# Runki2018/litehandnet

Hardware: AMD Instinct MI355X
Metric: images/sec fwd+bwd @256x256 bs64 litehandnet (higher is better)
Workload: dtype f32; 1 GPU; litehandnet variant B (MSRB hourglass litehourglass.py) C=128, 256x256x3 -> 21x64x64, per-GPU batch 64, train-mode BN, fwd + TopdownHeatmapLoss + bwd + fused Adam; global_batch=64, parallelism=dp1

## Files before the change

litehandnet_amd/csrc/k_misc.hip:

```cpp
#include "lhn_common.h"

static inline int grid_cap(int64_t blocks, int cap_per_cu) {
  const int64_t cap = (int64_t)lhn_num_cus() * cap_per_cu;
  if (blocks > cap) blocks = cap;
  if (blocks < 1) blocks = 1;
  return (int)blocks;
}
static inline bool pow2i(int v) { return v > 0 && (v & (v - 1)) == 0; }

#define LHN_FIN_THREADS 1024
__global__ void __launch_bounds__(LHN_FIN_THREADS) k_bn_finalize(const double* __restrict__ stats, const float* __restrict__ gamma,
                              const float* __restrict__ beta, float* __restrict__ rmean, float* __restrict__ rvar,
                              int64_t* __restrict__ nbt, float* __restrict__ table, int cs, int coff, int C,
                              float* __restrict__ save, double count, float eps, float momentum, float slope, int training,
                              const float* __restrict__ cbias, int SC) {
  __shared__ double part[2 * LHN_FIN_THREADS];
  const int nt = blockDim.x;
  int G = nt / C;
  G = G < 1 ? 1 : (G > LHN_STAT_REPLICAS ? LHN_STAT_REPLICAS : G);
  for (int c0 = 0; c0 < C; c0 += nt) {
    const int g = threadIdx.x / C, c = c0 + (G > 1 ? threadIdx.x - g * C : threadIdx.x);
    if (c0) __syncthreads();
    if (training && g < G && c < C) {
      double s1 = 0, s2 = 0;
#pragma unroll 4
      for (int r = g; r < LHN_STAT_REPLICAS; r += G) {
        s1 += stats[(size_t)r * 2 * SC + c];
        s2 += stats[(size_t)r * 2 * SC + SC + c];
      }
      part[2 * threadIdx.x] = s1;
      part[2 * threadIdx.x + 1] = s2;
    }
    __syncthreads();
    if (g != 0 || c >= C) continue;
    double mean, var;
    const double cb = cbias ? (double)cbias[c] : 0.0;
    if (training) {
      double s1 = 0, s2 = 0;
      for (int k = 0; k < G; ++k) {
        s1 += part[2 * (k * C + threadIdx.x)];
        s2 += part[2 * (k * C + threadIdx.x) + 1];
      }
      mean = s1 / count;
      var = s2 / count - mean * mean;
      if (var < 0) var = 0;
      if (rmean) {
        rmean[c] = (float)((1.0 - (double)momentum) * (double)rmean[c] + (double)momentum * (mean + cb));
        const double unb = count > 1 ? var * count / (count - 1.0) : var;
        rvar[c] = (float)((1.0 - (double)momentum) * (double)rvar[c] + (double)momentum * unb);
      }
    } else {
      mean = (double)rmean[c] - cb;
      var = rvar[c];
    }
    const float invstd = (float)(1.0 / sqrt(var + (double)eps));
    const float gm = gamma ? gamma[c] : 1.f, b = beta ? beta[c] : 0.f;
    const float sc = gm * invstd;
    table[coff + c] = sc;
    table[cs + coff + c] = b - (float)mean * sc;
    table[2 * cs + coff + c] = slope;
    if (save) {
      save[c] = (float)mean;
      save[SC + c] = invstd;
    }
  }
  if (training && nbt && threadIdx.x == 0) nbt[0] += 1;
}

__global__ void k_table_fill(float* __restrict__ table, int cs, int coff, int C, float sc, float sh, float sl) {
  for (int c = threadIdx.x; c < C; c += blockDim.x) {
    table[coff + c] = sc;
    table[cs + coff + c] = sh;
    table[2 * cs + coff + c] = sl;
  }
}

__global__ void k_table_bias(float* __restrict__ table, int cs, int coff, int C, const float* __restrict__ bias, float sl) {
  for (int c = threadIdx.x; c < C; c += blockDim.x) {
    table[coff + c] = 1.f;
    table[cs + coff + c] = bias ? bias[c] : 0.f;
    table[2 * cs + coff + c] = sl;
  }
}

struct EwSrcs {
  lhn_view v[3];
  float coef[3];
  int mode;
};
__device__ __forceinline__ void bil_taps(int d, int in, int out, int& i0, int& i1, float& w1) {
  if (in == out || out == 1) {
    i0 = i1 = (in == out) ? d : 0;
    w1 = 0.f;
    return;
  }
  const float pos = (float)d * ((float)(in - 1) / (float)(out - 1));
  i0 = (int)floorf(pos);
  if (i0 > in - 1) i0 = in - 1;
  i1 = i0 + 1 < in ? i0 + 1 : in - 1;
  w1 = pos - (float)i0;
}
__device__ __forceinline__ float lhn_relu_sigmoid(float v) { return 1.f / (1.f + expf(-fmaxf(v, 0.f))); }
__device__ __forceinline__ float lhn_relu_sigmoid_grad(float v) {
  if (!(v > 0.f)) return 0.f;
  const float s = 1.f / (1.f + expf(-v));
  return s * (1.f - s);
}
__device__ __forceinline__ int nearest_src(int d, int in, int out) {
  if (in == out) return d;
  const float sc = (float)in / (float)out;
  const int s = (int)floorf((float)d * sc);
  return s < in - 1 ? s : in - 1;
}
template <bool BIL>
__global__ void __launch_bounds__(256, BIL ? 1 : 3) k_ew_fwd(EwSrcs S, int nsrc, lhn_view dst, float out_slope) {
  const int C4 = dst.C >> 2, c4 = threadIdx.x % C4, pl = threadIdx.x / C4, PL = 256 / C4;
  const int rows = dst.N * dst.H;
  Xf4 xf[3];
  int ca[3];
#pragma unroll
  for (int k = 0; k < 3; ++k)
    if (k < nsrc) {
      ca[k] = S.v[k].coff + 4 * c4;
      xf[k] = lhn_load_xf(S.v[k], ca[k]);
    }
  for (int row = blockIdx.x; row < rows; row += gridDim.x) {
    const int n = row / dst.H, h = row - n * dst.H;
    const float* base[3];
    f4 gate[3];
#pragma unroll
    for (int k = 0; k < 3; ++k)
      if (k < nsrc) {
        const lhn_view& v = S.v[k];
        const int hs = nearest_src(h, v.H, dst.H);
        base[k] = v.data + ((size_t)(n * v.H + hs) * v.W) * v.cstride + ca[k];
        gate[k] = v.gate ? *reinterpret_cast<const f4*>(v.gate + (size_t)n * v.cstride + ca[k]) : (f4){1.f, 1.f, 1.f, 1.f};
      }
    float* out = dst.data + (size_t)row * dst.W * dst.cstride + dst.coff + 4 * c4;
    const bool mul = (S.mode & 1) != 0;
    constexpr bool bil = BIL;
    if (!bil) {
      for (int w0 = LHN_LANE0(pl, PL); w0 < dst.W; w0 += 4 * PL) {
        f4 raw[3][4];
#pragma unroll
        for (int k = 0; k < 3; ++k)
          if (k < nsrc) {
            const lhn_view& v = S.v[k];
#pragma unroll
            for (int j = 0; j < 4; ++j) {
              const int w = min(w0 + j * PL, dst.W - 1);
              const int ws = (v.W == dst.W) ? w : nearest_src(w, v.W, dst.W);
              raw[k][j] = *reinterpret_cast<const f4*>(base[k] + (size_t)ws * v.cstride);
            }
          }
#pragma unroll
        for (int j = 0; j < 4; ++j) {
          const int w = w0 + j * PL;
          if (w < dst.W) {
            f4 acc = mul ? (f4){1.f, 1.f, 1.f, 1.f} : (f4){0.f, 0.f, 0.f, 0.f};
#pragma unroll
            for (int k = 0; k < 3; ++k)
              if (k < nsrc) {
                const f4 val = lhn_apply_xf(raw[k][j], xf[k]) * (gate[k] * S.coef[k]);
                if (mul) acc *= val; else acc += val;
              }
            if (out_slope == LHN_SLOPE_RELU_SIGMOID) {
              acc.x = lhn_relu_sigmoid(acc.x); acc.y = lhn_relu_sigmoid(acc.y); acc.z = lhn_relu_sigmoid(acc.z); acc.w = lhn_relu_sigmoid(acc.w);
            } else if (out_slope == LHN_SLOPE_SILU) {
              acc.x = lhn_silu(acc.x); acc.y = lhn_silu(acc.y); acc.z = lhn_silu(acc.z); acc.w = lhn_silu(acc.w);
            } else {
              acc.x = lhn_lrelu(acc.x, out_slope); acc.y = lhn_lrelu(acc.y, out_slope); acc.z = lhn_lrelu(acc.z, out_slope); acc.w = lhn_lrelu(acc.w, out_slope);
            }
            *reinterpret_cast<f4*>(out + (size_t)w * dst.cstride) = acc;
          }
        }
      }
      continue;
    }
    for (int w = LHN_LANE0(pl, PL); w < dst.W; w += PL) {
      f4 acc = mul ? (f4){1.f, 1.f, 1.f, 1.f} : (f4){0.f, 0.f, 0.f, 0.f};
#pragma unroll
      for (int k = 0; k < 3; ++k)
        if (k < nsrc) {
          const lhn_view& v = S.v[k];
          f4 val;
          if (bil && (v.H != dst.H || v.W != dst.W)) {
            int h0, h1, w0, w1;
            float ah, aw;
            bil_taps(h, v.H, dst.H, h0, h1, ah);
            bil_taps(w, v.W, dst.W, w0, w1, aw);
            const float* b0 = v.data + ((size_t)(n * v.H + h0) * v.W) * v.cstride + ca[k];
            const float* b1 = v.data + ((size_t)(n * v.H + h1) * v.W) * v.cstride + ca[k];
            const f4 v00 = lhn_apply_xf(*reinterpret_cast<const f4*>(b0 + (size_t)w0 * v.cstride), xf[k]);
            const f4 v01 = lhn_apply_xf(*reinterpret_cast<const f4*>(b0 + (size_t)w1 * v.cstride), xf[k]);
            const f4 v10 = lhn_apply_xf(*reinterpret_cast<const f4*>(b1 + (size_t)w0 * v.cstride), xf[k]);
            const f4 v11 = lhn_apply_xf(*reinterpret_cast<const f4*>(b1 + (size_t)w1 * v.cstride), xf[k]);
            val = ((v00 * (1.f - aw) + v01 * aw) * (1.f - ah) + (v10 * (1.f - aw) + v11 * aw) * ah) * (gate[k] * S.coef[k]);
          } else {
            const int ws = nearest_src(w, v.W, dst.W);
            val = lhn_apply_xf(*reinterpret_cast<const f4*>(base[k] + (size_t)ws * v.cstride), xf[k]) * (gate[k] * S.coef[k]);
          }
          if (mul) acc *= val; else acc += val;
        }
      if (out_slope == LHN_SLOPE_RELU_SIGMOID) {
        acc.x = lhn_relu_sigmoid(acc.x);
        acc.y = lhn_relu_sigmoid(acc.y);
        acc.z = lhn_relu_sigmoid(acc.z);
        acc.w = lhn_relu_sigmoid(acc.w);
      } else if (out_slope == LHN_SLOPE_SILU) {
        acc.x = lhn_silu(acc.x);
        acc.y = lhn_silu(acc.y);
        acc.z = lhn_silu(acc.z);
        acc.w = lhn_silu(acc.w);
      } else {
        acc.x = lhn_lrelu(acc.x, out_slope);
        acc.y = lhn_lrelu(acc.y, out_slope);
        acc.z = lhn_lrelu(acc.z, out_slope);
        acc.w = lhn_lrelu(acc.w, out_slope);
      }
      *reinterpret_cast<f4*>(out + (size_t)w * dst.cstride) = acc;
    }
  }
}

__global__ void __launch_bounds__(256) k_ew_bwd_src(lhn_view src, lhn_view dst, const float* __restrict__ ddst,
                                                    const float* __restrict__ dst_dpool, float out_slope,
                                                    float* __restrict__ dsrc, int accumulate, lhn_bnsum bs) {
  __shared__ f4 bred[512];
  const int C4 = src.C >> 2, c4 = threadIdx.x % C4, pl = threadIdx.x / C4, PL = 256 / C4;
  f4 bsum = (f4){0.f, 0.f, 0.f, 0.f}, bsq = bsum, bmean = bsum, binv = bsum;
  Xf4 bxf;
  if (bs.sums) {
    bxf = lhn_load_xf(src, src.coff + 4 * c4);
    bmean = *reinterpret_cast<const f4*>(bs.save + bs.coff + 4 * c4);
    binv = *reinterpret_cast<const f4*>(bs.save + bs.C + bs.coff + 4 * c4);
  }
  const int fh = dst.H / src.H, fw = dst.W / src.W;
  const int cd = dst.coff + 4 * c4;
  const int rows = src.N * src.H;
  for (int row = blockIdx.x; row < rows; row += gridDim.x) {
    const int n = row / src.H, h = row - n * src.H;
    const f4 gate = dst.gate ? *reinterpret_cast<const f4*>(dst.gate + (size_t)n * dst.cstride + cd) : (f4){1.f, 1.f, 1.f, 1.f};
    for (int w = LHN_LANE0(pl, PL); w < src.W; w += PL) {
      f4 g = (f4){0.f, 0.f, 0.f, 0.f};
      for (int a = 0; a < fh; ++a)
        for (int b = 0; b < fw; ++b) {
          const int hd = h * fh + a, wd = w * fw + b;
          const size_t pd = ((size_t)(n * dst.H + hd) * dst.W + wd) * dst.cstride + cd;
          f4 e = *reinterpret_cast<const f4*>(ddst + pd) * gate;
          if (dst_dpool) {
            lhn_gradview gv{nullptr, dst_dpool, nullptr};
            e += lhn_dpool_sum(gv, dst, n, hd, wd, cd);
          }
          if (out_slope == LHN_SLOPE_SILU || out_slope == LHN_SLOPE_RELU_SIGMOID) {
            const Xf4 sxf = lhn_load_xf(src, src.coff + 4 * c4);
            const f4 v = lhn_load_val(src, sxf, (int64_t)(n * src.H + h) * src.W + w, n, src.coff + 4 * c4);
            if (out_slope == LHN_SLOPE_SILU) {
              e.x *= lhn_silu_grad(v.x);
              e.y *= lhn_silu_grad(v.y);
              e.z *= lhn_silu_grad(v.z);
              e.w *= lhn_silu_grad(v.w);
            } else {
              e.x *= lhn_relu_sigmoid_grad(v.x);
              e.y *= lhn_relu_sigmoid_grad(v.y);
              e.z *= lhn_relu_sigmoid_grad(v.z);
              e.w *= lhn_relu_sigmoid_grad(v.w);
            }
          } else if (out_slope != 1.f) {
            const f4 o = *reinterpret_cast<const f4*>(dst.data + pd);
            e.x *= o.x > 0.f ? 1.f : out_slope;
            e.y *= o.y > 0.f ? 1.f : out_slope;
            e.z *= o.z > 0.f ? 1.f : out_slope;
            e.w *= o.w > 0.f ? 1.f : out_slope;
          }
          g += e;
        }
      float* o = dsrc + ((size_t)row * src.W + w) * src.cstride + src.coff + 4 * c4;
      if (bs.sums) {
        const f4 raw = *reinterpret_cast<const f4*>(src.data + ((size_t)row * src.W + w) * src.cstride + src.coff + 4 * c4);
        const f4 du = g * lhn_dact_xf(raw, bxf);
        bsum += du;
        bsq += du * ((raw - bmean) * binv);
      }
      if (accumulate) g += *reinterpret_cast<const f4*>(o);
      *reinterpret_cast<f4*>(o) = g;
    }
  }
  if (bs.sums) lhn_bns_flush(bs, bsum, bsq, C4, bred);
}

struct EwBwdMulti {
  int n;
  lhn_view src[3];
  float* dsrc[3];
  int acc[3];
  lhn_bnsum bs[3];
};
__global__ void __launch_bounds__(256) k_ew_bwd_multi(EwBwdMulti m, lhn_view dst, const float* __restrict__ ddst,
                                                      const float* __restrict__ dst_dpool, float out_slope) {
  __shared__ f4 bred[512];
  const int C4 = dst.C >> 2, c4 = threadIdx.x % C4, pl = threadIdx.x / C4, PL = 256 / C4;
  f4 bsum[3], bsq[3], bmean[3], binv[3];
  Xf4 bxf[3];
#pragma unroll
  for (int k = 0; k < 3; ++k) {
    bsum[k] = bsq[k] = bmean[k] = binv[k] = (f4){0.f, 0.f, 0.f, 0.f};
    if (k < m.n && m.bs[k].sums) {
      bxf[k] = lhn_load_xf(m.src[k], m.src[k].coff + 4 * c4);
      bmean[k] = *reinterpret_cast<const f4*>(m.bs[k].save + m.bs[k].coff + 4 * c4);
      binv[k] = *reinterpret_cast<const f4*>(m.bs[k].save + m.bs[k].C + m.bs[k].coff + 4 * c4);
    }
  }
  const int cd = dst.coff + 4 * c4;
  const int rows = dst.N * dst.H;
  for (int row = blockIdx.x; row < rows; row += gridDim.x) {
    const int n = row / dst.H, h = row - n * dst.H;
    const f4 gate = dst.gate ? *reinterpret_cast<const f4*>(dst.gate + (size_t)n * dst.cstride + cd) : (f4){1.f, 1.f, 1.f, 1.f};
    for (int w = LHN_LANE0(pl, PL); w < dst.W; w += PL) {
      const size_t pix = (size_t)row * dst.W + w, pd = pix * dst.cstride + cd;
      f4 e = *reinterpret_cast<const f4*>(ddst + pd) * gate;
      if (dst_dpool) {
        lhn_gradview gv{nullptr, dst_dpool, nullptr};
        e += lhn_dpool_sum(gv, dst, n, h, w, cd);
      }
      if (out_slope != 1.f) {
        const f4 o = *reinterpret_cast<const f4*>(dst.data + pd);
        e.x *= o.x > 0.f ? 1.f : out_slope;
        e.y *= o.y > 0.f ? 1.f : out_slope;
        e.z *= o.z > 0.f ? 1.f : out_slope;
        e.w *= o.w > 0.f ? 1.f : out_slope;
      }
#pragma unroll
      for (int k = 0; k < 3; ++k) {
        if (k < m.n) {
          const size_t ps = pix * m.src[k].cstride + m.src[k].coff + 4 * c4;
          f4 g = e;
          if (m.bs[k].sums) {
            const f4 raw = *reinterpret_cast<const f4*>(m.src[k].data + ps);
            const f4 du = g * lhn_dact_xf(raw, bxf[k]);
            bsum[k] += du;
            bsq[k] += du * ((raw - bmean[k]) * binv[k]);
          }
          float* o = m.dsrc[k] + ps;
          if (m.acc[k]) g += *reinterpret_cast<const f4*>(o);
          *reinterpret_cast<f4*>(o) = g;
        }
      }
    }
  }
#pragma unroll
  for (int k = 0; k < 3; ++k)
    if (k < m.n && m.bs[k].sums) {
      lhn_bns_flush(m.bs[k], bsum[k], bsq[k], C4, bred);
      __syncthreads();
    }
}

__global__ void __launch_bounds__(256) k_maxpool2_fwd(lhn_view x, lhn_view y) {
  const int C4 = y.C >> 2, c4 = threadIdx.x % C4, pl = threadIdx.x / C4, PL = 256 / C4;
  const int ca = x.coff + 4 * c4;
  const Xf4 xf = lhn_load_xf(x, ca);
  const int rows = y.N * y.H;
  for (int row = blockIdx.x; row < rows; row += gridDim.x) {
    const int n = row / y.H, ho = row - n * y.H;
    const f4 gate = x.gate ? *reinterpret_cast<const f4*>(x.gate + (size_t)n * x.cstride + ca) : (f4){1.f, 1.f, 1.f, 1.f};
    for (int wo = LHN_LANE0(pl, PL); wo < y.W; wo += PL) {
      f4 m = (f4){-INFINITY, -INFINITY, -INFINITY, -INFINITY};
#pragma unroll
      for (int o = 0; o < 4; ++o) {
        const int ih = 2 * ho + (o >> 1), iw = 2 * wo + (o & 1);
        if (ih < x.H && iw < x.W) {
          const f4 v = lhn_apply_xf(*reinterpret_cast<const f4*>(x.data + ((size_t)(n * x.H + ih) * x.W + iw) * x.cstride + ca), xf) * gate;
          m.x = v.x > m.x || v.x != v.x ? v.x : m.x;
          m.y = v.y > m.y || v.y != v.y ? v.y : m.y;
          m.z = v.z > m.z || v.z != v.z ? v.z : m.z;
          m.w = v.w > m.w || v.w != v.w ? v.w : m.w;
        }
      }
      *reinterpret_cast<f4*>(y.data + ((size_t)row * y.W + wo) * y.cstride + y.coff + 4 * c4) = m;
    }
  }
}
template <bool ADD>
__global__ void __launch_bounds__(256) k_maxpool2_bwd(lhn_view x, lhn_view y, const float* __restrict__ dy,
                                                      float* __restrict__ dx, int accumulate, lhn_bnsum bs, lhn_grad_adds ad) {
  __shared__ f4 bred[512];
  const int C4 = y.C >> 2, c4 = threadIdx.x % C4, pl = threadIdx.x / C4, PL = 256 / C4;
  const int ca = x.coff + 4 * c4;
  const Xf4 xf = lhn_load_xf(x, ca);
  f4 bsum = (f4){0.f, 0.f, 0.f, 0.f}, bsq = bsum, bmean = bsum, binv = bsum;
  if (bs.sums) {
    bmean = *reinterpret_cast<const f4*>(bs.save + bs.coff + 4 * c4);
    binv = *reinterpret_cast<const f4*>(bs.save + bs.C + bs.coff + 4 * c4);
  }
  const int rows = y.N * y.H;
  for (int row = blockIdx.x; row < rows; row += gridDim.x) {
    const int n = row / y.H, ho = row - n * y.H;
    const f4 gate = x.gate ? *reinterpret_cast<const f4*>(x.gate + (size_t)n * x.cstride + ca) : (f4){1.f, 1.f, 1.f, 1.f};
    for (int wo = LHN_LANE0(pl, PL); wo < y.W; wo += PL) {
      const f4 g = *reinterpret_cast<const f4*>(dy + ((size_t)row * y.W + wo) * y.cstride + y.coff + 4 * c4);
      f4 m = (f4){-INFINITY, -INFINITY, -INFINITY, -INFINITY};
      int arg[4] = {-1, -1, -1, -1};
      f4 raws[4];
#pragma unroll
      for (int o = 0; o < 4; ++o) {
        const int ih = 2 * ho + (o >> 1), iw = 2 * wo + (o & 1);
        if (ih < x.H && iw < x.W) {
          raws[o] = *reinterpret_cast<const f4*>(x.data + ((size_t)(n * x.H + ih) * x.W + iw) * x.cstride + ca);
          const f4 v = lhn_apply_xf(raws[o], xf) * gate;
          if (v.x > m.x || v.x != v.x || arg[0] < 0) { if (!(m.x != m.x)) { m.x = v.x; arg[0] = o; } }
          if (v.y > m.y || v.y != v.y || arg[1] < 0) { if (!(m.y != m.y)) { m.y = v.y; arg[1] = o; } }
          if (v.z > m.z || v.z != v.z || arg[2] < 0) { if (!(m.z != m.z)) { m.z = v.z; arg[2] = o; } }
          if (v.w > m.w || v.w != v.w || arg[3] < 0) { if (!(m.w != m.w)) { m.w = v.w; arg[3] = o; } }
        }
      }
#pragma unroll
      for (int o = 0; o < 4; ++o) {
        const int ih = 2 * ho + (o >> 1), iw = 2 * wo + (o & 1);
        if (ih < x.H && iw < x.W) {
          f4 r = (f4){arg[0] == o ? g.x : 0.f, arg[1] == o ? g.y : 0.f, arg[2] == o ? g.z : 0.f, arg[3] == o ? g.w : 0.f};
          if (ADD) {
            if (ad.same) r += *reinterpret_cast<const f4*>(ad.same + ((size_t)(n * x.H + ih) * x.W + iw) * ad.same_cstride + ad.same_coff + 4 * c4);
            if (ad.pooled) {
              const int OH = ad.OH, OW = ad.OW, ohc = (ih * OH) / x.H, owc = (iw * OW) / x.W;
              for (int oh = max(ohc - 1, 0); oh <= min(ohc + 1, OH - 1); ++oh) {
                const int h0 = (oh * x.H) / OH, h1 = ((oh + 1) * x.H + OH - 1) / OH;
                if (ih < h0 || ih >= h1) continue;
                for (int ow = max(owc - 1, 0); ow <= min(owc + 1, OW - 1); ++ow) {
                  const int w0 = (ow * x.W) / OW, w1 = ((ow + 1) * x.W + OW - 1) / OW;
                  if (iw < w0 || iw >= w1) continue;
                  const float inv = 1.f / (float)((h1 - h0) * (w1 - w0));
                  r += *reinterpret_cast<const f4*>(ad.pooled + ((size_t)(n * OH + oh) * OW + ow) * ad.pooled_cstride + ad.pooled_coff + 4 * c4) * inv;
                }
              }
            }
          }
          float* q = dx + ((size_t)(n * x.H + ih) * x.W + iw) * x.cstride + ca;
          if (bs.sums) {
            const f4 du = r * lhn_dact_xf(raws[o], xf);
            bsum += du;
            bsq += du * ((raws[o] - bmean) * binv);
          }
          if (accumulate) r += *reinterpret_cast<const f4*>(q);
          *reinterpret_cast<f4*>(q) = r;
        }
      }
    }
  }
  if (bs.sums) lhn_bns_flush(bs, bsum, bsq, C4, bred);
}

struct BnSlices {
  const float* save[2];
  double* sums[2];
  int lo[2], C[2], n;
};
__device__ __forceinline__ void lhn_slice_mi4(const BnSlices& sl, int c, f4& mean, f4& inv) {
  mean = (f4){0.f, 0.f, 0.f, 0.f};
  inv = (f4){1.f, 1.f, 1.f, 1.f};
#pragma unroll
  for (int k = 0; k < 2; ++k)
    if (k < sl.n && c >= sl.lo[k] && c < sl.lo[k] + sl.C[k]) {
      mean = *reinterpret_cast<const f4*>(sl.save[k] + (c - sl.lo[k]));
      inv = *reinterpret_cast<const f4*>(sl.save[k] + sl.C[k] + (c - sl.lo[k]));
    }
}
__device__ __forceinline__ f4 lhn_dact4(f4 raw, const Xf4& t) {
  const f4 u = raw * t.sc + t.sh;
  return (f4){u.x > 0.f ? 1.f : t.sl.x, u.y > 0.f ? 1.f : t.sl.y, u.z > 0.f ? 1.f : t.sl.z, u.w > 0.f ? 1.f : t.sl.w};
}

template <bool STAT, bool COPY>
__global__ void __launch_bounds__(256) k_avgpool_fwd(lhn_view x, float* __restrict__ out, int OH, int OW, int ostride,
                                                     int ocoff, float* __restrict__ pstat, BnSlices sl, lhn_view src) {
  __shared__ f4 red[STAT ? 768 : 256];
  const int C4 = x.C >> 2, PL = 256 / C4;
  const int b = blockIdx.x;
  const int ow = b % OW, oh = (b / OW) % OH, n = b / (OW * OH);
  const int h0 = (oh * x.H) / OH, h1 = ((oh + 1) * x.H + OH - 1) / OH;
  const int w0 = (ow * x.W) / OW, w1 = ((ow + 1) * x.W + OW - 1) / OW;
  const int bw = w1 - w0, cnt = (h1 - h0) * bw;
  const int c4 = threadIdx.x % C4, pl = threadIdx.x / C4;
  const int ca = x.coff + 4 * c4;
  const bool cp = COPY && 4 * c4 < src.C;
  const int sca = src.coff + 4 * c4;
  Xf4 xf = lhn_load_xf(x, ca);
  f4 sgate = (f4){1.f, 1.f, 1.f, 1.f};
  if (cp) {
    xf = lhn_load_xf(src, sca);
    if (src.gate) sgate = *reinterpret_cast<const f4*>(src.gate + (int64_t)n * src.cstride + sca);
  }
  f4 mean, inv;
  if (STAT) lhn_slice_mi4(sl, ca, mean, inv);
  const float* base = cp ? src.data + (int64_t)n * x.H * x.W * src.cstride + sca : x.data + (int64_t)n * x.H * x.W * x.cstride + ca;
  const int64_t pstr = cp ? src.cstride : x.cstride;
  auto at = [&](int p) { return *reinterpret_cast<const f4*>(base + (int64_t)((h0 + p / bw) * x.W + w0 + p % bw) * pstr); };
  const int hown = ((oh + 1) * x.H) / OH, wown = ((ow + 1) * x.W) / OW;
  float* xout = x.data + (int64_t)n * x.H * x.W * x.cstride + ca;
  auto put = [&](int p, f4 v) {
    const int h = h0 + p / bw, w = w0 + p % bw;
    if (h < hown && w < wown) *reinterpret_cast<f4*>(xout + (int64_t)(h * x.W + w) * x.cstride) = v;
  };
  f4 s0 = (f4){0.f, 0.f, 0.f, 0.f}, s1 = s0, s2 = s0, s3 = s0, m0 = s0, m1 = s0;
  int p = LHN_LANE0(pl, PL);
  for (; p + 3 * PL < cnt; p += 4 * PL) {
    const f4 a = at(p), b2 = at(p + PL), c2 = at(p + 2 * PL), d2 = at(p + 3 * PL);
    const f4 va = lhn_apply_xf(a, xf) * sgate, vb = lhn_apply_xf(b2, xf) * sgate, vc = lhn_apply_xf(c2, xf) * sgate, vd = lhn_apply_xf(d2, xf) * sgate;
    s0 += va;
    s1 += vb;
    s2 += vc;
    s3 += vd;
    if (cp) {
      put(p, va);
      put(p + PL, vb);
      put(p + 2 * PL, vc);
      put(p + 3 * PL, vd);
    }
    if (STAT) {
      const f4 da = lhn_dact4(a, xf), db = lhn_dact4(b2, xf), dc = lhn_dact4(c2, xf), dd = lhn_dact4(d2, xf);
      m0 += (da + db) + (dc + dd);
      m1 += (da * ((a - mean) * inv) + db * ((b2 - mean) * inv)) + (dc * ((c2 - mean) * inv) + dd * ((d2 - mean) * inv));
    }
  }
  for (; p < cnt; p += PL) {
    const f4 a = at(p);
    const f4 va = lhn_apply_xf(a, xf) * sgate;
    s0 += va;
    if (cp) put(p, va);
    if (STAT) {
      const f4 da = lhn_dact4(a, xf);
      m0 += da;
      m1 += da * ((a - mean) * inv);
    }
  }
  f4 s = (s0 + s1) + (s2 + s3);
  if (x.gate) s *= *reinterpret_cast<const f4*>(x.gate + (int64_t)n * x.cstride + ca);
  const bool shuf = C4 <= 64 && (C4 & (C4 - 1)) == 0;
  if (shuf)
    for (int o = C4; o < 64; o <<= 1) {
      s.x += __shfl_xor(s.x, o, 64); s.y += __shfl_xor(s.y, o, 64); s.z += __shfl_xor(s.z, o, 64); s.w += __shfl_xor(s.w, o, 64);
      if (STAT) {
        m0.x += __shfl_xor(m0.x, o, 64); m0.y += __shfl_xor(m0.y, o, 64); m0.z += __shfl_xor(m0.z, o, 64); m0.w += __shfl_xor(m0.w, o, 64);
        m1.x += __shfl_xor(m1.x, o, 64); m1.y += __shfl_xor(m1.y, o, 64); m1.z += __shfl_xor(m1.z, o, 64); m1.w += __shfl_xor(m1.w, o, 64);
      }
    }
  const int lane = threadIdx.x & 63, wave = threadIdx.x >> 6;
  if (shuf && lane < C4) {
    red[wave * C4 + lane] = s;
    if (STAT) {
      red[256 + wave * C4 + lane] = m0;
      red[512 + wave * C4 + lane] = m1;
    }
  }
  if (!shuf) {
    red[threadIdx.x] = s;
    if (STAT) {
      red[256 + threadIdx.x] = m0;
      red[512 + threadIdx.x] = m1;
    }
  }
  __syncthreads();
  if (threadIdx.x < C4) {
    const int nj = shuf ? 4 : PL;
    f4 t = (f4){0.f, 0.f, 0.f, 0.f}, t0 = t, t1 = t;
    for (int j = 0; j < nj; ++j) {
      t += red[j * C4 + threadIdx.x];
      if (STAT) {
        t0 += red[256 + j * C4 + threadIdx.x];
        t1 += red[512 + j * C4 + threadIdx.x];
      }
    }
    const float invc = 1.f / (float)cnt;
    *reinterpret_cast<f4*>(out + (int64_t)b * ostride + ocoff + 4 * threadIdx.x) = t * invc;
    if (STAT) {
      *reinterpret_cast<f4*>(pstat + ((int64_t)b * 2 + 0) * x.C + 4 * threadIdx.x) = t0;
      *reinterpret_cast<f4*>(pstat + ((int64_t)b * 2 + 1) * x.C + 4 * threadIdx.x) = t1;
    }
  }
}
__global__ void __launch_bounds__(256) k_avgpool_small(lhn_view x, float* __restrict__ out, int OH, int OW, int ostride, int ocoff) {
  const int C4 = x.C >> 2;
  const int64_t total = (int64_t)x.N * OH * OW * C4;
  for (int64_t i = (int64_t)blockIdx.x * 256 + threadIdx.x; i < total; i += (int64_t)gridDim.x * 256) {
    const int c4 = (int)(i % C4);
    const int64_t b = i / C4;
    const int ow = (int)(b % OW), oh = (int)((b / OW) % OH), n = (int)(b / ((int64_t)OW * OH));
    const int h0 = (oh * x.H) / OH, h1 = ((oh + 1) * x.H + OH - 1) / OH;
    const int w0 = (ow * x.W) / OW, w1 = ((ow + 1) * x.W + OW - 1) / OW;
    const int ca = x.coff + 4 * c4;
    const Xf4 xf = lhn_load_xf(x, ca);
    f4 s = (f4){0.f, 0.f, 0.f, 0.f};
    for (int h = h0; h < h1; ++h)
      for (int w = w0; w < w1; ++w)
        s += lhn_apply_xf(*reinterpret_cast<const f4*>(x.data + ((int64_t)(n * x.H + h) * x.W + w) * x.cstride + ca), xf);
    if (x.gate) s *= *reinterpret_cast<const f4*>(x.gate + (int64_t)n * x.cstride + ca);
    *reinterpret_cast<f4*>(out + b * ostride + ocoff + 4 * c4) = s * (1.f / (float)((h1 - h0) * (w1 - w0)));
  }
}
__global__ void __launch_bounds__(256) k_avgpool_bwd(lhn_view x, const float* __restrict__ dout, int OH, int OW,
                                                     float* __restrict__ dx, int accumulate, int ostride, int ocoff, lhn_bnsum bs) {
  __shared__ f4 bred[512];
  const int C4 = x.C >> 2, c4 = threadIdx.x % C4, pl = threadIdx.x / C4, PL = 256 / C4;
  f4 bsum = (f4){0.f, 0.f, 0.f, 0.f}, bsq = bsum, bmean = bsum, binv = bsum;
  Xf4 bxf;
  if (bs.sums) {
    bxf = lhn_load_xf(x, x.coff + 4 * c4);
    bmean = *reinterpret_cast<const f4*>(bs.save + bs.coff + 4 * c4);
    binv = *reinterpret_cast<const f4*>(bs.save + bs.C + bs.coff + 4 * c4);
  }
  const int rows = x.N * x.H;
  for (int row = blockIdx.x; row < rows; row += gridDim.x) {
    const int n = row / x.H, h = row - n * x.H;
    for (int w = LHN_LANE0(pl, PL); w < x.W; w += PL) {
      f4 g = (f4){0.f, 0.f, 0.f, 0.f};
      const int ohc = (h * OH) / x.H, owc = (w * OW) / x.W;
      for (int oh = max(ohc - 1, 0); oh <= min(ohc + 1, OH - 1); ++oh) {
        const int h0 = (oh * x.H) / OH, h1 = ((oh + 1) * x.H + OH - 1) / OH;
        if (h < h0 || h >= h1) continue;
        for (int ow = max(owc - 1, 0); ow <= min(owc + 1, OW - 1); ++ow) {
          const int w0 = (ow * x.W) / OW, w1 = ((ow + 1) * x.W + OW - 1) / OW;
          if (w < w0 || w >= w1) continue;
          const float inv = 1.f / (float)((h1 - h0) * (w1 - w0));
          g += *reinterpret_cast<const f4*>(dout + ((size_t)(n * OH + oh) * OW + ow) * ostride + ocoff + 4 * c4) * inv;
        }
      }
      float* o = dx + ((size_t)row * x.W + w) * x.cstride + x.coff + 4 * c4;
      if (bs.sums) {
        const f4 raw = *reinterpret_cast<const f4*>(x.data + ((size_t)row * x.W + w) * x.cstride + x.coff + 4 * c4);
        const f4 du = g * lhn_dact_xf(raw, bxf);
        bsum += du;
        bsq += du * ((raw - bmean) * binv);
      }
      if (accumulate) g += *reinterpret_cast<const f4*>(o);
      *reinterpret_cast<f4*>(o) = g;
    }
  }
  if (bs.sums) lhn_bns_flush(bs, bsum, bsq, C4, bred);
}

__global__ void __launch_bounds__(1024) k_ca1(const float* __restrict__ pooled, const float* __restrict__ w3,
                                             const float* __restrict__ gamma, const float* __restrict__ beta,
                                             float* __restrict__ rmean, float* __restrict__ rvar, int64_t* __restrict__ nbt,
                                             const float* __restrict__ mask, float* __restrict__ save, int N, int C,
                                             float eps, float momentum, int training, int stage, double* __restrict__ gsum,
                                             double count_scale) {
  __shared__ double rs[32][32], rq[32][32];
  const int NL = blockDim.x >> 5;
  __shared__ float s_sc[32], s_sh[32];
  float* a = save;
  float* ahat = save + (int64_t)N * C;
  float* smean = save + (int64_t)N * C * 3 + (int64_t)N * (C / 2);
  float* sinv = smean + C;
  const int cl = threadIdx.x & 31, nl = threadIdx.x >> 5, c = blockIdx.x * 32 + cl;
  const bool ok = c < C;
  float wt[9];
#pragma unroll
  for (int t = 0; t < 9; ++t) wt[t] = ok ? w3[c * 9 + t] : 0.f;
  double s = 0, q = 0;
  if (ok && stage != 2)
    for (int n = nl; n < N; n += NL) {
      float v = 0.f;
#pragma unroll
      for (int t = 0; t < 9; ++t) v += pooled[((int64_t)n * 9 + t) * C + c] * wt[t];
      a[(int64_t)n * C + c] = v;
      s += v;
      q += (double)v * v;
    }
  rs[nl][cl] = s;
  rq[nl][cl] = q;
  __syncthreads();
  if (nl == 0 && ok) {
    for (int j = 1; j < NL; ++j) {
      s += rs[j][cl];
      q += rq[j][cl];
    }
    if (stage == 1) {
      gsum[c] = s;
      gsum[C + c] = q;
    } else if (stage == 2) {
      s = gsum[c];
      q = gsum[C + c];
    }
  }
  if (stage == 1) return;
  const double NT = (double)N * count_scale;
  if (nl == 0 && ok) {
    double mean, var;
    if (!gamma) {
      smean[c] = 0.f;
      sinv[c] = 1.f;
      s_sc[cl] = 1.f;
      s_sh[cl] = beta ? beta[c] : 0.f;
    } else {
    if (training) {
      mean = s / NT;
      var = q / NT - mean * mean;
      if (var < 0) var = 0;
      rmean[c] = (float)((1.0 - (double)momentum) * rmean[c] + (double)momentum * mean);
      rvar[c] = (float)((1.0 - (double)momentum) * rvar[c] + (double)momentum * (NT > 1 ? var * NT / (NT - 1.0) : var));
    } else {
      mean = rmean[c];
      var = rvar[c];
    }
    const float invstd = (float)(1.0 / sqrt(var + (double)eps));
    smean[c] = (float)mean;
    sinv[c] = invstd;
    s_sc[cl] = gamma[c] * invstd;
    s_sh[cl] = beta[c] - (float)mean * (gamma[c] * invstd);
    }
  }
  __syncthreads();
  if (ok) {
    const float sc = s_sc[cl], sh = s_sh[cl];
    for (int n = nl; n < N; n += NL) {
      float v = a[(int64_t)n * C + c] * sc + sh;
      if (mask) v *= mask[(int64_t)n * C + c];
      ahat[(int64_t)n * C + c] = v;
    }
  }
  if (training && nbt && blockIdx.x == 0 && threadIdx.x == 0) nbt[0] += 1;
}
__global__ void __launch_bounds__(256) k_ca2(const float* __restrict__ w1, const float* __restrict__ b1,
                                             const float* __restrict__ w2, const float* __restrict__ b2,
                                             float* __restrict__ save, float* __restrict__ gate, int gs, int gcoff, int N,
                                             int C) {
  __shared__ float sa[256], shh[128];
  const int n = blockIdx.x, Ch = C / 2;
  const float* ahat = save + (int64_t)N * C + (int64_t)n * C;
  float* h = save + (int64_t)N * C * 2 + (int64_t)n * Ch;
  float* g = save + (int64_t)N * C * 2 + (int64_t)N * Ch + (int64_t)n * C;
  for (int c = threadIdx.x; c < C; c += blockDim.x) sa[c] = ahat[c];
  __syncthreads();
  for (int j = threadIdx.x; j < Ch; j += blockDim.x) {
    float v = b1[j];
    for (int c = 0; c < C; ++c) v += w1[j * C + c] * sa[c];
    v = lhn_lrelu(v, 0.01f);
    h[j] = v;
    shh[j] = v;
  }
  __syncthreads();
  for (int c = threadIdx.x; c < C; c += blockDim.x) {
    float v = b2[c];
    for (int j = 0; j < Ch; ++j) v += w2[c * Ch + j] * shh[j];
    const float sg = 1.f / (1.f + expf(-v));
    g[c] = sg;
    gate[(int64_t)n * gs + gcoff + c] = sg;
  }
}

__global__ void __launch_bounds__(256) k_gate_bwd_reduce(lhn_view y, const float* __restrict__ dz,
                                                         float* __restrict__ dgate, float* __restrict__ tsum, BnSlices sl) {
  __shared__ f4 red[768];
  const int C4 = y.C >> 2, PL = 256 / C4, n = blockIdx.x;
  const int c4 = threadIdx.x % C4, pl = threadIdx.x / C4;
  const int ca = y.coff + 4 * c4;
  const Xf4 xf = lhn_load_xf(y, ca);
  f4 mean, inv;
  lhn_slice_mi4(sl, ca, mean, inv);
  const int HW = y.H * y.W;
  const int chunk = (HW + gridDim.y - 1) / gridDim.y;
  const int p0 = blockIdx.y * chunk, p1 = min(HW, p0 + chunk);
  f4 s = (f4){0.f, 0.f, 0.f, 0.f}, t0 = s, t1 = s;
  for (int p = p0 + LHN_LANE0(pl, PL); p < p1; p += 2 * PL) {
    const int64_t pixa = (int64_t)n * HW + p, pixb = (int64_t)n * HW + min(p + PL, p1 - 1);
    const f4 rawa = *reinterpret_cast<const f4*>(y.data + pixa * y.cstride + ca);
    const f4 rawb = *reinterpret_cast<const f4*>(y.data + pixb * y.cstride + ca);
    const f4 dza = *reinterpret_cast<const f4*>(dz + pixa * y.cstride + ca);
    f4 dzb = *reinterpret_cast<const f4*>(dz + pixb * y.cstride + ca);
    if (p + PL >= p1) dzb = (f4){0.f, 0.f, 0.f, 0.f};
    s += lhn_apply_xf(rawa, xf) * dza + lhn_apply_xf(rawb, xf) * dzb;
    if (tsum) {
      const f4 da = lhn_dact4(rawa, xf) * dza, db = lhn_dact4(rawb, xf) * dzb;
      t0 += da + db;
      t1 += da * ((rawa - mean) * inv) + db * ((rawb - mean) * inv);
    }
  }
  red[threadIdx.x] = s;
  red[256 + threadIdx.x] = t0;
  red[512 + threadIdx.x] = t1;
  __syncthreads();
  if (threadIdx.x < C4) {
    f4 t = (f4){0.f, 0.f, 0.f, 0.f}, u0 = t, u1 = t;
    for (int j = 0; j < PL; ++j) {
      t += red[j * C4 + threadIdx.x];
      u0 += red[256 + j * C4 + threadIdx.x];
      u1 += red[512 + j * C4 + threadIdx.x];
    }
    float* o = dgate + (int64_t)n * y.C + 4 * threadIdx.x;
    atomicAdd(o + 0, t.x);
    atomicAdd(o + 1, t.y);
    atomicAdd(o + 2, t.z);
    atomicAdd(o + 3, t.w);
    if (tsum) {
      float* o0 = tsum + ((int64_t)n * 2 + 0) * y.C + 4 * threadIdx.x;
      float* o1 = tsum + ((int64_t)n * 2 + 1) * y.C + 4 * threadIdx.x;
      atomicAdd(o0 + 0, u0.x); atomicAdd(o0 + 1, u0.y); atomicAdd(o0 + 2, u0.z); atomicAdd(o0 + 3, u0.w);
      atomicAdd(o1 + 0, u1.x); atomicAdd(o1 + 1, u1.y); atomicAdd(o1 + 2, u1.z); atomicAdd(o1 + 3, u1.w);
    }
  }
}

__global__ void __launch_bounds__(256) k_ca_bwd2(const float* __restrict__ w1, const float* __restrict__ w2,
                                                 const float* __restrict__ save, const float* __restrict__ dgate,
                                                 float* __restrict__ dahat , float* __restrict__ dvbuf ,
                                                 float* __restrict__ dhbuf , int N, int C) {
  __shared__ float sdv[256], sdh[128], shh[128];
  const int Ch = C / 2, n = blockIdx.x;
  const float* h = save + (int64_t)N * C * 2 + (int64_t)n * Ch;
  const float* g = save + (int64_t)N * C * 2 + (int64_t)N * Ch + (int64_t)n * C;
  for (int c = threadIdx.x; c < C; c += blockDim.x) {
    const float gg = g[c];
    const float dv = dgate[(int64_t)n * C + c] * gg * (1.f - gg);
    sdv[c] = dv;
    dvbuf[(int64_t)n * C + c] = dv;
  }
  for (int j = threadIdx.x; j < Ch; j += blockDim.x) shh[j] = h[j];
  __syncthreads();
  for (int j = threadIdx.x; j < Ch; j += blockDim.x) {
    float d = 0.f;
#pragma unroll 8
    for (int c = 0; c < C; ++c) d += w2[c * Ch + j] * sdv[c];
    d *= shh[j] > 0.f ? 1.f : 0.01f;
    sdh[j] = d;
    dhbuf[(int64_t)n * Ch + j] = d;
  }
  __syncthreads();
  for (int c = threadIdx.x; c < C; c += blockDim.x) {
    float d = 0.f;
#pragma unroll 8
    for (int j = 0; j < Ch; ++j) d += w1[j * C + c] * sdh[j];
    dahat[(int64_t)n * C + c] = d;
  }
}
__global__ void __launch_bounds__(1024) k_ca_bwd1(const float* __restrict__ pooled, const float* __restrict__ w3,
                                                 const float* __restrict__ gamma, const float* __restrict__ mask,
                                                 const float* __restrict__ save, const float* __restrict__ dahat,
                                                 float* __restrict__ dpool, int cs, int coff, int H, int W,
                                                 float* __restrict__ dw3, float* __restrict__ dgamma,
                                                 float* __restrict__ dbeta, int N, int C, int training, int stage,
                                                 double* __restrict__ gsum, double count_scale, float pgrad_scale,
                                                 const float* __restrict__ tsum, const float* __restrict__ pstat, BnSlices sl,
                                                 const float* __restrict__ dvbuf, const float* __restrict__ dhbuf,
                                                 float* __restrict__ dw1, float* __restrict__ db1, float* __restrict__ dw2,
                                                 float* __restrict__ db2) {
  const int nmain = (C + 31) / 32;
  if ((int)blockIdx.x >= nmain) {
    if (stage == 1) return;
    const int Ch = C / 2, o = ((int)blockIdx.x - nmain) * blockDim.x + threadIdx.x, nw = C * Ch;
    const float* ahat = save + (int64_t)N * C;
    const float* hh = save + (int64_t)N * C * 2;
    if (o < nw) {
      const int cc = o / Ch, j = o - cc * Ch;
      float v = 0.f;
#pragma unroll 8
      for (int n = 0; n < N; ++n) v += dvbuf[(int64_t)n * C + cc] * hh[(int64_t)n * Ch + j];
      dw2[o] += v;
    } else if (o < 2 * nw) {
      const int q = o - nw, j = q / C, cc = q - j * C;
      float v = 0.f;
#pragma unroll 8
      for (int n = 0; n < N; ++n) v += dhbuf[(int64_t)n * Ch + j] * ahat[(int64_t)n * C + cc];
      dw1[q] += v;
    } else if (o < 2 * nw + C) {
      const int cc = o - 2 * nw;
      float v = 0.f;
#pragma unroll 8
      for (int n = 0; n < N; ++n) v += dvbuf[(int64_t)n * C + cc];
      db2[cc] += v;
    } else if (o < 2 * nw + C + Ch) {
      const int j = o - 2 * nw - C;
      float v = 0.f;
#pragma unroll 8
      for (int n = 0; n < N; ++n) v += dhbuf[(int64_t)n * Ch + j];
      db1[j] += v;
    }
    return;
  }
  __shared__ double rs[32][32], rq[32][32];
  __shared__ float rw[32][32][9];
  const int NL = blockDim.x >> 5;
  const float* a = save;
  const float* smean = save + (int64_t)N * C * 3 + (int64_t)N * (C / 2);
  const float* sinv = smean + C;
  const int cl = threadIdx.x & 31, nl = threadIdx.x >> 5, c = blockIdx.x * 32 + cl;
  const bool ok = c < C;
  const float mean = ok ? smean[c] : 0.f, invstd = ok ? sinv[c] : 0.f, gm = ok ? gamma[c] : 0.f;
  double sd = 0, sdx = 0;
  if (ok && stage != 2)
    for (int n = nl; n < N; n += NL) {
      float d = dahat[(int64_t)n * C + c];
      if (mask) d *= mask[(int64_t)n * C + c];
      const float xh = (a[(int64_t)n * C + c] - mean) * invstd;
      sd += d;
      sdx += (double)d * xh;
    }
  rs[nl][cl] = sd;
  rq[nl][cl] = sdx;
  __syncthreads();
  sd = 0;
  sdx = 0;
  for (int j = 0; j < NL; ++j) {
    sd += rs[j][cl];
    sdx += rq[j][cl];
  }
  if (stage == 1) {
    if (nl == 0 && ok) {
      gsum[c] = sd;
      gsum[C + c] = sdx;
    }
    return;
  }
  if (stage == 2 && ok) {
    sd = gsum[c];
    sdx = gsum[C + c];
  }
  const double NT = (double)N * count_scale;
  if (nl == 0 && ok) {
    dgamma[c] += (float)sdx * pgrad_scale;
    dbeta[c] += (float)sd * pgrad_scale;
  }
  const float* gsave = save + (int64_t)N * C * 2 + (int64_t)N * (C / 2);
  double bs0 = 0, bs1 = 0;
  float wt[9], dwt[9], binv[9];
#pragma unroll
  for (int t = 0; t < 9; ++t) {
    wt[t] = ok ? w3[c * 9 + t] : 0.f;
    dwt[t] = 0.f;
    const int bi = t / 3, bj = t % 3;
    binv[t] = 1.f / (float)((lhn_bin_hi(bi, H) - lhn_bin_lo(bi, H)) * (lhn_bin_hi(bj, W) - lhn_bin_lo(bj, W)));
  }
  if (ok)
    for (int n = nl; n < N; n += NL) {
      float d = dahat[(int64_t)n * C + c];
      if (mask) d *= mask[(int64_t)n * C + c];
      const float xh = (a[(int64_t)n * C + c] - mean) * invstd;
      float da = gm * invstd * d;
      if (training) da = gm * invstd * (d - (float)(sd / NT) - xh * (float)(sdx / NT));
      float dseg[9];
#pragma unroll
      for (int t = 0; t < 9; ++t) {
        dwt[t] += da * pooled[((int64_t)n * 9 + t) * C + c];
        dseg[t] = da * wt[t] * binv[t];
      }
      lhn_dpool_store(dpool, n, cs, coff + c, dseg);
      if (tsum) {
        const float g = gsave[(int64_t)n * C + c];
        float a0 = g * tsum[((int64_t)n * 2 + 0) * C + c], a1 = g * tsum[((int64_t)n * 2 + 1) * C + c];
#pragma unroll
        for (int t = 0; t < 9; ++t) {
          a0 += dseg[t] * pstat[(((int64_t)n * 9 + t) * 2 + 0) * C + c];
          a1 += dseg[t] * pstat[(((int64_t)n * 9 + t) * 2 + 1) * C + c];
        }
        bs0 += a0;
        bs1 += a1;
      }
    }
  if (tsum) {
    __syncthreads();
    rs[nl][cl] = bs0;
    rq[nl][cl] = bs1;
    __syncthreads();
    if (nl == 0 && ok) {
      double t0 = 0, t1 = 0;
      for (int j = 0; j < NL; ++j) {
        t0 += rs[j][cl];
        t1 += rq[j][cl];
      }
      const int cb = coff + c;
#pragma unroll
      for (int k = 0; k < 2; ++k)
        if (k < sl.n && sl.sums[k] && cb >= sl.lo[k] && cb < sl.lo[k] + sl.C[k]) {
          sl.sums[k][cb - sl.lo[k]] = t0;
          sl.sums[k][sl.C[k] + cb - sl.lo[k]] = t1;
        }
    }
  }
#pragma unroll
  for (int t = 0; t < 9; ++t) rw[nl][cl][t] = dwt[t];
  __syncthreads();
  if (nl == 0 && ok) {
#pragma unroll
    for (int t = 0; t < 9; ++t) {
      float v = 0.f;
      for (int j = 0; j < NL; ++j) v += rw[j][cl][t];
      dw3[c * 9 + t] += v;
    }
  }
}

__global__ void __launch_bounds__(256) k_bn_bwd_reduce(lhn_view y, lhn_gradview g, const float* __restrict__ save,
                                                       double* __restrict__ sums, lhn_bnbwdfin fin) {
  __shared__ f4 red[512];
  const int C4 = y.C >> 2, PL = 256 / C4;
  const int c4 = threadIdx.x % C4, pl = threadIdx.x / C4;
  const int ca = y.coff + 4 * c4;
  const Xf4 xf = lhn_load_xf(y, ca);
  const f4 mean = *reinterpret_cast<const f4*>(save + 4 * c4);
  const f4 inv = *reinterpret_cast<const f4*>(save + y.C + 4 * c4);
  const int rows = y.N * y.H;
  f4 s = (f4){0.f, 0.f, 0.f, 0.f}, q = s;
  for (int row = blockIdx.x; row < rows; row += gridDim.x) {
    const int n = row / y.H, h = row - n * y.H;
    const f4 gate = y.gate ? *reinterpret_cast<const f4*>(y.gate + (size_t)n * y.cstride + ca) : (f4){1.f, 1.f, 1.f, 1.f};
    const size_t rbase = (size_t)row * y.W * y.cstride + ca;
    for (int w0 = LHN_LANE0(pl, PL); w0 < y.W; w0 += 4 * PL) {
      f4 raw4[4], dz4[4];
#pragma unroll
      for (int j = 0; j < 4; ++j) {
        const size_t off = rbase + (size_t)min(w0 + j * PL, y.W - 1) * y.cstride;
        raw4[j] = *reinterpret_cast<const f4*>(y.data + off);
        dz4[j] = *reinterpret_cast<const f4*>(g.dz + off);
      }
#pragma unroll
      for (int j = 0; j < 4; ++j) {
        const int w = w0 + j * PL;
        if (w < y.W) {
          const f4 raw = raw4[j];
          f4 e = dz4[j] * gate;
          if (g.dpool) e += lhn_dpool_sum(g, y, n, h, w, ca);
          const f4 u = raw * xf.sc + xf.sh;
          const f4 du = e * (f4){u.x > 0.f ? 1.f : xf.sl.x, u.y > 0.f ? 1.f : xf.sl.y, u.z > 0.f ? 1.f : xf.sl.z, u.w > 0.f ? 1.f : xf.sl.w};
          s += du;
          q += du * ((raw - mean) * inv);
        }
      }
    }
  }
  double* st = sums + (size_t)(blockIdx.x % LHN_STAT_REPLICAS) * 2 * y.C;
  if (C4 <= 32 && (C4 & (C4 - 1)) == 0) {
    lhn_block_stat_atomics(s, q, C4, red, st, st + y.C);
  } else {
    red[threadIdx.x * 2] = s;
    red[threadIdx.x * 2 + 1] = q;
    __syncthreads();
    if (threadIdx.x < C4) {
      double sd[4] = {0, 0, 0, 0}, qd[4] = {0, 0, 0, 0};
      for (int j = 0; j < PL; ++j) {
        const f4 a = red[(j * C4 + threadIdx.x) * 2], b = red[(j * C4 + threadIdx.x) * 2 + 1];
        sd[0] += a.x; sd[1] += a.y; sd[2] += a.z; sd[3] += a.w;
        qd[0] += b.x; qd[1] += b.y; qd[2] += b.z; qd[3] += b.w;
      }
#pragma unroll
      for (int j = 0; j < 4; ++j) {
        atomicAdd(st + 4 * threadIdx.x + j, sd[j]);
        atomicAdd(st + y.C + 4 * threadIdx.x + j, qd[j]);
      }
    }
  }
  if (fin.counter && lhn_last_block(fin.counter)) lhn_bn_bwd_finalize_block(fin, sums, save);
}
__global__ void __launch_bounds__(LHN_FIN_THREADS) k_bn_bwd_finalize(const double* __restrict__ sums, const float* __restrict__ gamma,
                                  const float* __restrict__ save, float* __restrict__ coef, int cs, int coff, int C,
                                  double count, float* __restrict__ dgamma, float* __restrict__ dbeta, float pgrad_scale, int SC) {
  __shared__ double part[2 * LHN_FIN_THREADS];
  const int nt = blockDim.x;
  int G = nt / C;
  G = G < 1 ? 1 : (G > LHN_STAT_REPLICAS ? LHN_STAT_REPLICAS : G);
  for (int c0 = 0; c0 < C; c0 += nt) {
    const int g = threadIdx.x / C, c = c0 + (G > 1 ? threadIdx.x - g * C : threadIdx.x);
    if (c0) __syncthreads();
    if (g < G && c < C) {
      double s1 = 0, s2 = 0;
#pragma unroll 4
      for (int r = g; r < LHN_STAT_REPLICAS; r += G) {
        s1 += sums[(size_t)r * 2 * SC + c];
        s2 += sums[(size_t)r * 2 * SC + SC + c];
      }
      part[2 * threadIdx.x] = s1;
      part[2 * threadIdx.x + 1] = s2;
    }
    __syncthreads();
    if (g != 0 || c >= C) continue;
    double db = 0, dg = 0;
    for (int k = 0; k < G; ++k) {
      db += part[2 * (k * C + threadIdx.x)];
      dg += part[2 * (k * C + threadIdx.x) + 1];
    }
    const double mean = save[c], inv = save[SC + c], s = (double)(gamma ? gamma[c] : 1.f) * inv;
    coef[coff + c] = (float)s;
    coef[cs + coff + c] = (float)(-s * inv * dg / count);
    coef[2 * cs + coff + c] = (float)(-s * db / count + s * inv * mean * dg / count);
    if (dgamma) dgamma[c] += (float)dg * pgrad_scale;
    if (dbeta) dbeta[c] += (float)db * pgrad_scale;
  }
}

__global__ void __launch_bounds__(256) k_reduce_replicas(float* __restrict__ out, const float* __restrict__ part, int64_t n4,
                                                         int nrep, int64_t rep_stride) {
  for (int64_t i = (int64_t)blockIdx.x * blockDim.x + threadIdx.x; i < n4; i += (int64_t)gridDim.x * blockDim.x) {
    f4 s = *reinterpret_cast<const f4*>(part + 4 * i);
    for (int r = 1; r < nrep; ++r) s += *reinterpret_cast<const f4*>(part + (size_t)r * rep_stride + 4 * i);
    *reinterpret_cast<f4*>(out + 4 * i) = s;
  }
}

__global__ void __launch_bounds__(256) k_fold_stat_replicas(double* __restrict__ st, int64_t n, int nrep) {
  for (int64_t i = (int64_t)blockIdx.x * 256 + threadIdx.x; i < n; i += (int64_t)gridDim.x * 256) {
    double s = st[i];
    for (int r = 1; r < nrep; ++r) {
      s += st[(int64_t)r * n + i];
      st[(int64_t)r * n + i] = 0.0;
    }
    st[i] = s;
  }
}

extern "C" {

int lhn_fold_stat_replicas(double* stats, int64_t n, int nrep, void* stream) {
  LHN_CHECK_ARG(stats && n > 0 && nrep >= 1, "lhn_fold_stat_replicas: bad argument");
  hipLaunchKernelGGL(k_fold_stat_replicas, dim3((unsigned)((n + 255) / 256 > 64 ? 64 : (n + 255) / 256)), dim3(256), 0, (hipStream_t)stream, stats, n, nrep);
  LHN_CHECK_LAUNCH("lhn_fold_stat_replicas");
  return 0;
}

int lhn_reduce_replicas(float* out, const float* part, int64_t n, int nrep, int64_t rep_stride, void* stream) {
  LHN_CHECK_ARG(out && part && n > 0 && n % 4 == 0 && nrep >= 1 && rep_stride % 4 == 0, "lhn_reduce_replicas: bad args (n and stride multiples of 4)");
  hipLaunchKernelGGL(k_reduce_replicas, dim3(grid_cap((n / 4 + 255) / 256, 8)), dim3(256), 0, (hipStream_t)stream, out, part, n / 4, nrep, rep_stride);
  LHN_CHECK_LAUNCH("lhn_reduce_replicas");
  return 0;
}

int lhn_bn_finalize(const double* stats, const float* gamma, const float* beta, float* running_mean, float* running_var,
                    int64_t* nbt, float* table, int cstride, int coff, int C, float* save, double count, float eps,
                    float momentum, float slope, int training, const float* conv_bias, void* stream) {
  return lhn_bn_finalize2(stats, gamma, beta, running_mean, running_var, nbt, table, cstride, coff, C, C, save, count, eps, momentum,
                          slope, training, conv_bias, stream);
}
int lhn_bn_finalize2(const double* stats, const float* gamma, const float* beta, float* running_mean, float* running_var,
                     int64_t* nbt, float* table, int cstride, int coff, int C, int stat_channels, float* save, double count,
                     float eps, float momentum, float slope, int training, const float* conv_bias, void* stream) {
  LHN_CHECK_ARG(table && C > 0 && coff >= 0 && coff + C <= cstride && stat_channels >= C, "lhn_bn_finalize: bad table slice");
  LHN_CHECK_ARG(training ? (stats != nullptr) : (running_mean && running_var), "lhn_bn_finalize: missing statistics");
  LHN_CHECK_ARG(!training || count >= 1, "lhn_bn_finalize: count");
  int nt = training ? (C >= LHN_FIN_THREADS ? LHN_FIN_THREADS : (LHN_FIN_THREADS / C > LHN_STAT_REPLICAS ? LHN_STAT_REPLICAS : LHN_FIN_THREADS / C) * C)
                    : (C <= 64 ? 64 : (C <= 128 ? 128 : 256));
  nt = (nt + 63) / 64 * 64;
  hipLaunchKernelGGL(k_bn_finalize, dim3(1), dim3(nt), 0, (hipStream_t)stream, stats,
                     gamma, beta, running_mean, running_var, nbt, table, cstride, coff, C, save, count, eps, momentum,
                     slope, training, conv_bias, stat_channels);
  LHN_CHECK_LAUNCH("lhn_bn_finalize");
  return 0;
}

int lhn_table_fill(float* table, int cstride, int coff, int C, float scale, float shift, float slope, void* stream) {
  LHN_CHECK_ARG(table && C > 0 && coff >= 0 && coff + C <= cstride, "lhn_table_fill: bad table slice");
  hipLaunchKernelGGL(k_table_fill, dim3(1), dim3(128), 0, (hipStream_t)stream, table, cstride, coff, C, scale, shift, slope);
  LHN_CHECK_LAUNCH("lhn_table_fill");
  return 0;
}

int lhn_table_bias(float* table, int cstride, int coff, int C, const float* bias, float slope, void* stream) {
  LHN_CHECK_ARG(table && C > 0 && coff >= 0 && coff + C <= cstride, "lhn_table_bias: bad slice");
  hipLaunchKernelGGL(k_table_bias, dim3(1), dim3(128), 0, (hipStream_t)stream, table, cstride, coff, C, bias, slope);
  LHN_CHECK_LAUNCH("lhn_table_bias");
  return 0;
}

int lhn_ew_fwd(const lhn_view* srcs, int nsrc, const lhn_view* dst, float out_slope, void* stream) {
  return lhn_ew_fwd2(srcs, nsrc, nullptr, dst, out_slope, stream);
}
int lhn_ew_fwd2(const lhn_view* srcs, int nsrc, const float* coef, const lhn_view* dst, float out_slope, void* stream) {
  return lhn_ew_fwd3(srcs, nsrc, coef, dst, out_slope, 0, stream);
}
int lhn_ew_fwd3(const lhn_view* srcs, int nsrc, const float* coef, const lhn_view* dst, float out_slope, int mode, void* stream) {
  LHN_CHECK_ARG(srcs && nsrc >= 1 && nsrc <= 3 && lhn_view_ok(dst) && mode >= 0 && mode <= 3, "lhn_ew_fwd: 1..3 sources, valid dst");
  EwSrcs S;
  memset(&S, 0, sizeof(S));
  S.mode = mode;
  for (int i = 0; i < nsrc; ++i) {
    LHN_CHECK_ARG(lhn_view_ok(&srcs[i]) && srcs[i].C == dst->C && srcs[i].N == dst->N && lhn_no_pend(&srcs[i]), "lhn_ew_fwd: source %d mismatch", i);
    S.v[i] = srcs[i];
    S.coef[i] = coef ? coef[i] : 1.f;
  }
  LHN_CHECK_ARG(dst->C % 4 == 0 && dst->C <= 1024, "lhn_ew_fwd: C=%d", dst->C);
  if (S.mode & 2)
    hipLaunchKernelGGL(k_ew_fwd<true>, dim3(grid_cap((int64_t)dst->N * dst->H, 8)), dim3(256), 0, (hipStream_t)stream, S, nsrc, *dst, out_slope);
  else
    hipLaunchKernelGGL(k_ew_fwd<false>, dim3(grid_cap((int64_t)dst->N * dst->H, 8)), dim3(256), 0, (hipStream_t)stream, S, nsrc, *dst, out_slope);
  LHN_CHECK_LAUNCH("lhn_ew_fwd");
  return 0;
}

int lhn_ew_bwd(const lhn_view* srcs, int nsrc, const lhn_view* dst, const float* ddst, float out_slope,
               float* const* dsrcs, const int* accumulate, void* stream) {
  LHN_CHECK_ARG(srcs && nsrc >= 1 && nsrc <= 3 && lhn_view_ok(dst) && ddst && dsrcs && accumulate, "lhn_ew_bwd: bad args");
  for (int i = 0; i < nsrc; ++i) {
    if (!dsrcs[i]) continue;
    const lhn_view* s = &srcs[i];
    LHN_CHECK_ARG(lhn_view_ok(s) && s->C == dst->C, "lhn_ew_bwd: source %d mismatch", i);
    LHN_CHECK_ARG(dst->H % s->H == 0 && dst->W % s->W == 0, "lhn_ew_bwd: non-integer upsample %dx%d -> %dx%d", s->H, s->W, dst->H, dst->W);
    LHN_CHECK_ARG(s->C % 4 == 0 && s->C <= 1024, "lhn_ew_bwd: C=%d", s->C);
    lhn_bnsum nob;
    memset(&nob, 0, sizeof(nob));
    hipLaunchKernelGGL(k_ew_bwd_src, dim3(grid_cap((int64_t)s->N * s->H, 8)), dim3(256), 0, (hipStream_t)stream, *s, *dst, ddst,
                       (const float*)nullptr, out_slope, dsrcs[i], accumulate[i], nob);
  }
  LHN_CHECK_LAUNCH("lhn_ew_bwd");
  return 0;
}
static int bns_of(const lhn_bnsum* in, const lhn_view* v, lhn_bnsum* out, const char* who) {
  memset(out, 0, sizeof(*out));
  if (!in || !in->sums) return 0;
  LHN_CHECK_ARG(in->save && in->C > 0 && in->coff >= 0 && in->coff % 4 == 0 && in->coff + v->C <= in->C && !v->gate && v->table,
                "%s: BatchNorm sums need an ungated input view with a table, inside the producer's %d channels (offset %d, view %d)", who,
                in->C, in->coff, v->C);
  *out = *in;
  return 0;
}
int lhn_ew_bwd2(const lhn_view* src, const lhn_view* dst, const float* ddst, const float* dst_dpool, float out_slope,
                float* dsrc, int accumulate, void* stream) {
  return lhn_ew_bwd3(src, dst, ddst, dst_dpool, out_slope, dsrc, accumulate, nullptr, stream);
}
int lhn_ew_bwd3(const lhn_view* src, const lhn_view* dst, const float* ddst, const float* dst_dpool, float out_slope,
                float* dsrc, int accumulate, const lhn_bnsum* bns, void* stream) {
  LHN_CHECK_ARG(lhn_view_ok(src) && lhn_view_ok(dst) && ddst && dsrc && src->C == dst->C && lhn_no_pend(src) && lhn_no_pend(dst), "lhn_ew_bwd2: bad args");
  LHN_CHECK_ARG(dst->H % src->H == 0 && dst->W % src->W == 0, "lhn_ew_bwd2: non-integer upsample");
  LHN_CHECK_ARG((out_slope != LHN_SLOPE_SILU && out_slope != LHN_SLOPE_RELU_SIGMOID) || (dst->H == src->H && dst->W == src->W), "lhn_ew_bwd2: SiLU / ReLU-sigmoid need a single same-size source");
  LHN_CHECK_ARG(src->C % 4 == 0 && src->C <= 1024, "lhn_ew_bwd2: C=%d", src->C);
  lhn_bnsum bs;
  if (bns_of(bns, src, &bs, "lhn_ew_bwd3")) return 1;
  hipLaunchKernelGGL(k_ew_bwd_src, dim3(grid_cap((int64_t)src->N * src->H, 8)), dim3(256), 0, (hipStream_t)stream, *src, *dst, ddst,
                     dst_dpool, out_slope, dsrc, accumulate, bs);
  LHN_CHECK_LAUNCH("lhn_ew_bwd2");
  return 0;
}

int lhn_ew_bwd_multi(const lhn_view* srcs, int nsrc, const lhn_view* dst, const float* ddst, const float* dst_dpool, float out_slope,
                     float* const* dsrcs, const int* accumulate, const lhn_bnsum* const* bns, void* stream) {
  LHN_CHECK_ARG(srcs && nsrc >= 1 && nsrc <= 3 && lhn_view_ok(dst) && ddst && dsrcs && accumulate && lhn_no_pend(dst), "lhn_ew_bwd_multi: bad args");
  LHN_CHECK_ARG(out_slope != LHN_SLOPE_SILU && out_slope != LHN_SLOPE_RELU_SIGMOID, "lhn_ew_bwd_multi: SiLU / ReLU-sigmoid take lhn_ew_bwd3");
  LHN_CHECK_ARG(dst->C % 4 == 0 && dst->C <= 1024, "lhn_ew_bwd_multi: C=%d", dst->C);
  EwBwdMulti m;
  memset(&m, 0, sizeof(m));
  m.n = nsrc;
  for (int k = 0; k < nsrc; ++k) {
    const lhn_view* v = &srcs[k];
    LHN_CHECK_ARG(lhn_view_ok(v) && lhn_no_pend(v) && dsrcs[k] && v->C == dst->C && v->N == dst->N && v->H == dst->H && v->W == dst->W,
                  "lhn_ew_bwd_multi: source %d must have the destination's geometry", k);
    m.src[k] = *v;
    m.dsrc[k] = dsrcs[k];
    m.acc[k] = accumulate[k];
    if (bns_of(bns ? bns[k] : nullptr, v, &m.bs[k], "lhn_ew_bwd_multi")) return 1;
  }
  hipLaunchKernelGGL(k_ew_bwd_multi, dim3(grid_cap((int64_t)dst->N * dst->H, 8)), dim3(256), 0, (hipStream_t)stream, m, *dst, ddst, dst_dpool, out_slope);
  LHN_CHECK_LAUNCH("lhn_ew_bwd_multi");
  return 0;
}

int lhn_maxpool2_fwd(const lhn_view* x, const lhn_view* y, void* stream) {
  LHN_CHECK_ARG(lhn_view_ok(x) && lhn_view_ok(y) && x->C == y->C, "lhn_maxpool2_fwd: bad views");
  LHN_CHECK_ARG(y->H == (x->H + 1) / 2 && y->W == (x->W + 1) / 2 && y->N == x->N, "lhn_maxpool2_fwd: geometry");
  LHN_CHECK_ARG(y->C % 4 == 0 && y->C <= 1024, "lhn_maxpool2_fwd: C=%d", y->C);
  LHN_CHECK_ARG(lhn_no_pend(x), "lhn_maxpool2_fwd: lhn_view.pend is reserved (NULL)");
  hipLaunchKernelGGL(k_maxpool2_fwd, dim3(grid_cap((int64_t)y->N * y->H, 8)), dim3(256), 0, (hipStream_t)stream, *x, *y);
  LHN_CHECK_LAUNCH("lhn_maxpool2_fwd");
  return 0;
}
int lhn_maxpool2_bwd(const lhn_view* x, const lhn_view* y, const float* dy, float* dx, int dx_accumulate, void* stream) {
  return lhn_maxpool2_bwd2(x, y, dy, dx, dx_accumulate, nullptr, stream);
}
int lhn_maxpool2_bwd2(const lhn_view* x, const lhn_view* y, const float* dy, float* dx, int dx_accumulate, const lhn_bnsum* bns,
                      void* stream) {
  return lhn_maxpool2_bwd3(x, y, dy, dx, dx_accumulate, bns, nullptr, stream);
}
int lhn_maxpool2_bwd3(const lhn_view* x, const lhn_view* y, const float* dy, float* dx, int dx_accumulate, const lhn_bnsum* bns,
                      const lhn_grad_adds* adds, void* stream) {
  LHN_CHECK_ARG(lhn_view_ok(x) && lhn_view_ok(y) && dy && dx && x->C == y->C && lhn_no_pend(x), "lhn_maxpool2_bwd: bad args");
  LHN_CHECK_ARG(y->C % 4 == 0 && y->C <= 1024, "lhn_maxpool2_bwd: C=%d", y->C);
  lhn_bnsum bs;
  if (bns_of(bns, x, &bs, "lhn_maxpool2_bwd2")) return 1;
  lhn_grad_adds ad;
  memset(&ad, 0, sizeof(ad));
  if (adds && (adds->same || adds->pooled)) {
    ad = *adds;
    LHN_CHECK_ARG(x->H % 2 == 0 && x->W % 2 == 0 && y->H == x->H / 2 && y->W == x->W / 2, "lhn_maxpool2_bwd3: gradient addends need even H, W (%dx%d)", x->H, x->W);
    LHN_CHECK_ARG(!ad.same || (ad.same_cstride % 4 == 0 && ad.same_coff % 4 == 0 && ad.same_coff >= 0 && ad.same_coff + x->C <= ad.same_cstride),
                  "lhn_maxpool2_bwd3: same-resolution addend layout");
    LHN_CHECK_ARG(!ad.pooled || (ad.OH > 0 && ad.OW > 0 && ad.OH <= x->H && ad.OW <= x->W && ad.pooled_cstride % 4 == 0 && ad.pooled_coff % 4 == 0 &&
                                 ad.pooled_coff >= 0 && ad.pooled_coff + x->C <= ad.pooled_cstride),
                  "lhn_maxpool2_bwd3: pooled addend layout");
    hipLaunchKernelGGL(k_maxpool2_bwd<true>, dim3(grid_cap((int64_t)y->N * y->H, 8)), dim3(256), 0, (hipStream_t)stream, *x, *y, dy, dx, dx_accumulate, bs, ad);
  } else {
    hipLaunchKernelGGL(k_maxpool2_bwd<false>, dim3(grid_cap((int64_t)y->N * y->H, 8)), dim3(256), 0, (hipStream_t)stream, *x, *y, dy, dx, dx_accumulate, bs, ad);
  }
  LHN_CHECK_LAUNCH("lhn_maxpool2_bwd");
  return 0;
}

int lhn_avgpool_fwd(const lhn_view* x, float* out, int OH, int OW, void* stream) {
  return lhn_avgpool_fwd2(x, out, OH, OW, x ? x->C : 0, 0, stream);
}
int lhn_avgpool_fwd2(const lhn_view* x, float* out, int OH, int OW, int out_cstride, int out_coff, void* stream) {
  LHN_CHECK_ARG(lhn_view_ok(x) && out && OH > 0 && OW > 0 && out_coff >= 0 && out_coff % 4 == 0 && out_cstride % 4 == 0 &&
                    out_coff + x->C <= out_cstride,
                "lhn_avgpool_fwd: bad args");
  LHN_CHECK_ARG(x->C % 4 == 0 && x->C <= 1024, "lhn_avgpool_fwd: C=%d", x->C);
  LHN_CHECK_ARG(lhn_no_pend(x), "lhn_avgpool_fwd: lhn_view.pend is reserved (NULL)");
  const int binmax = ((x->H + OH - 1) / OH + 1) * ((x->W + OW - 1) / OW + 1);
  if (binmax <= 25) {
    const int64_t total = (int64_t)x->N * OH * OW * (x->C / 4);
    hipLaunchKernelGGL(k_avgpool_small, dim3(grid_cap((total + 255) / 256, 16)), dim3(256), 0, (hipStream_t)stream, *x, out, OH, OW, out_cstride, out_coff);
  } else
  {
    BnSlices sl;
    memset(&sl, 0, sizeof(sl));
    lhn_view nosrc;
    memset(&nosrc, 0, sizeof(nosrc));
    hipLaunchKernelGGL((k_avgpool_fwd<false, false>), dim3(x->N * OH * OW), dim3(256), 0, (hipStream_t)stream, *x, out, OH, OW, out_cstride, out_coff,
                       (float*)nullptr, sl, nosrc);
  }
  LHN_CHECK_LAUNCH("lhn_avgpool_fwd");
  return 0;
}
static int mk_slices(const lhn_bn_slices* in, int C, BnSlices* sl, const char* who) {
  memset(sl, 0, sizeof(*sl));
  if (!in) return 0;
  LHN_CHECK_ARG(in->n >= 0 && in->n <= 2, "%s: 0..2 BatchNorm slices", who);
  sl->n = in->n;
  for (int k = 0; k < in->n; ++k) {
    LHN_CHECK_ARG(in->save[k] && in->lo[k] >= 0 && in->C[k] > 0 && in->lo[k] % 4 == 0 && in->C[k] % 4 == 0 && in->lo[k] + in->C[k] <= C,
                  "%s: BatchNorm slice %d = channels [%d, %d) of %d", who, k, in->lo[k], in->lo[k] + in->C[k], C);
    sl->save[k] = in->save[k];
    sl->sums[k] = in->sums[k];
    sl->lo[k] = in->lo[k];
    sl->C[k] = in->C[k];
  }
  return 0;
}
int lhn_avgpool_fwd3(const lhn_view* x, float* out, int OH, int OW, float* pstat, const lhn_bn_slices* slices, void* stream) {
  return lhn_avgpool_fwd4(x, out, OH, OW, pstat, slices, nullptr, stream);
}
int lhn_avgpool_fwd4(const lhn_view* x, float* out, int OH, int OW, float* pstat, const lhn_bn_slices* slices, const lhn_view* copy_src,
                     void* stream) {
  if (!pstat && !copy_src) return lhn_avgpool_fwd2(x, out, OH, OW, x ? x->C : 0, 0, stream);
  LHN_CHECK_ARG(lhn_view_ok(x) && out && OH > 0 && OW > 0 && x->C % 4 == 0 && x->C <= 1024 && x->coff == 0 && x->C == x->cstride && lhn_no_pend(x),
                "lhn_avgpool_fwd4: the statistics / copy forms pool a whole buffer");
  LHN_CHECK_ARG(!copy_src || (lhn_view_ok(copy_src) && lhn_no_pend(copy_src) && copy_src->N == x->N && copy_src->H == x->H && copy_src->W == x->W &&
                              copy_src->C < x->C && copy_src->data != x->data),
                "lhn_avgpool_fwd4: copy_src = the first channels of the pooled tensor, same pixels, another buffer");
  BnSlices sl;
  if (mk_slices(pstat ? slices : nullptr, x->C, &sl, "lhn_avgpool_fwd4")) return 1;
  lhn_view src;
  memset(&src, 0, sizeof(src));
  if (copy_src) src = *copy_src;
  const dim3 g(x->N * OH * OW), bk(256);
  hipStream_t s = (hipStream_t)stream;
  if (pstat && copy_src) hipLaunchKernelGGL((k_avgpool_fwd<true, true>), g, bk, 0, s, *x, out, OH, OW, x->C, 0, pstat, sl, src);
  else if (pstat) hipLaunchKernelGGL((k_avgpool_fwd<true, false>), g, bk, 0, s, *x, out, OH, OW, x->C, 0, pstat, sl, src);
  else hipLaunchKernelGGL((k_avgpool_fwd<false, true>), g, bk, 0, s, *x, out, OH, OW, x->C, 0, pstat, sl, src);
  LHN_CHECK_LAUNCH("lhn_avgpool_fwd4");
  return 0;
}
int lhn_avgpool_bwd(const lhn_view* x, const float* dout, int OH, int OW, float* dx, int dx_accumulate, void* stream) {
  return lhn_avgpool_bwd2(x, dout, OH, OW, x ? x->C : 0, 0, dx, dx_accumulate, stream);
}
int lhn_avgpool_bwd2(const lhn_view* x, const float* dout, int OH, int OW, int out_cstride, int out_coff, float* dx,
                     int dx_accumulate, void* stream) {
  return lhn_avgpool_bwd3(x, dout, OH, OW, out_cstride, out_coff, dx, dx_accumulate, nullptr, stream);
}
int lhn_avgpool_bwd3(const lhn_view* x, const float* dout, int OH, int OW, int out_cstride, int out_coff, float* dx,
                     int dx_accumulate, const lhn_bnsum* bns, void* stream) {
  LHN_CHECK_ARG(lhn_view_ok(x) && dout && dx && out_coff >= 0 && out_coff + x->C <= out_cstride, "lhn_avgpool_bwd: bad args");
  LHN_CHECK_ARG(x->C % 4 == 0 && x->C <= 1024, "lhn_avgpool_bwd: C=%d", x->C);
  lhn_bnsum bs;
  if (bns_of(bns, x, &bs, "lhn_avgpool_bwd3")) return 1;
  hipLaunchKernelGGL(k_avgpool_bwd, dim3(grid_cap((int64_t)x->N * x->H, 8)), dim3(256), 0, (hipStream_t)stream, *x, dout, OH, OW, dx, dx_accumulate, out_cstride, out_coff, bs);
  LHN_CHECK_LAUNCH("lhn_avgpool_bwd");
  return 0;
}

int lhn_ca_mlp_fwd(const float* pooled, const float* w3, const float* gamma, const float* beta, float* rmean, float* rvar,
                   int64_t* nbt, const float* w1, const float* b1, const float* w2, const float* b2, const float* dropmask,
                   float* gate, int gate_stride, int gate_coff, float* save, int N, int C, float eps, float momentum,
                   int training, int stage, double* gsum, double count_scale, void* stream) {
  LHN_CHECK_ARG(pooled && w3 && w1 && b1 && w2 && b2 && gate && save, "lhn_ca_mlp_fwd: null pointer");
  LHN_CHECK_ARG(gamma ? (beta && rmean && rvar) : !training, "lhn_ca_mlp_fwd: BatchNorm tensors missing (gamma NULL = deployed form, eval only)");
  LHN_CHECK_ARG(C > 0 && C <= 256 && C % 2 == 0 && N > 0, "lhn_ca_mlp_fwd: C=%d (<=256)", C);
  hipStream_t s = (hipStream_t)stream;
  LHN_CHECK_ARG(stage == 0 || (gsum && stage >= 1 && stage <= 2 && count_scale >= 1), "lhn_ca_mlp_fwd: stage %d needs gsum", stage);
  hipLaunchKernelGGL(k_ca1, dim3((C + 31) / 32), dim3(1024), 0, s, pooled, w3, gamma, beta, rmean, rvar, nbt, dropmask, save, N, C, eps, momentum, training, stage, gsum, stage ? count_scale : 1.0);
  if (stage != 1) hipLaunchKernelGGL(k_ca2, dim3(N), dim3(128), 0, s, w1, b1, w2, b2, save, gate, gate_stride, gate_coff, N, C);
  LHN_CHECK_LAUNCH("lhn_ca_mlp_fwd");
  return 0;
}

int lhn_gate_bwd_reduce(const lhn_view* y, const float* dz, float* dgate, void* stream) {
  return lhn_gate_bwd_reduce2(y, dz, dgate, nullptr, nullptr, stream);
}
int lhn_gate_bwd_reduce2(const lhn_view* y, const float* dz, float* dgate, float* tsum, const lhn_bn_slices* slices, void* stream) {
  return lhn_gate_bwd_reduce3(y, dz, dgate, tsum, slices, 0, stream);
}
int lhn_gate_bwd_reduce3(const lhn_view* y, const float* dz, float* dgate, float* tsum, const lhn_bn_slices* slices, int prezeroed,
                         void* stream) {
  LHN_CHECK_ARG(lhn_view_ok(y) && dz && dgate && y->C % 4 == 0 && y->C <= 1024 && lhn_no_pend(y), "lhn_gate_bwd_reduce: bad args");
  LHN_CHECK_ARG(!tsum || (y->coff == 0 && y->C == y->cstride && tsum == dgate + (size_t)y->N * y->C),
                "lhn_gate_bwd_reduce2: tsum = the 2*N*C floats behind dgate, whole-buffer view");
  hipStream_t s = (hipStream_t)stream;
  BnSlices sl;
  if (mk_slices(tsum ? slices : nullptr, y->C, &sl, "lhn_gate_bwd_reduce2")) return 1;
  if (!prezeroed && hipMemsetAsync(dgate, 0, (size_t)y->N * y->C * 4 * (tsum ? 3 : 1), s) != hipSuccess) {
    lhn_set_error("lhn_gate_bwd_reduce: memset failed");
    return 2;
  }
  int split = (y->H * y->W + 127) / 128;
  if (split < 1) split = 1;
  if (split > 32) split = 32;
  if (lhn_deterministic_mode()) split = 1;
  hipLaunchKernelGGL(k_gate_bwd_reduce, dim3(y->N, split), dim3(256), 0, s, *y, dz, dgate, tsum, sl);
  LHN_CHECK_LAUNCH("lhn_gate_bwd_reduce");
  return 0;
}

int lhn_ca_mlp_bwd(const float* pooled, const float* w3, const float* gamma, const float* w1, const float* w2,
                   const float* dropmask, const float* save, const float* dgate, float* dpool, int cstride, int coff, int H,
                   int W, float* dw3, float* dgamma, float* dbeta, float* dw1, float* db1, float* dw2, float* db2, int N,
                   int C, int stage, double* gsum, double count_scale, float pgrad_scale, void* stream) {
  return lhn_ca_mlp_bwd2(pooled, w3, gamma, w1, w2, dropmask, save, dgate, dpool, cstride, coff, H, W, dw3, dgamma, dbeta, dw1, db1, dw2,
                         db2, N, C, stage, gsum, count_scale, pgrad_scale, nullptr, nullptr, nullptr, stream);
}
int lhn_ca_mlp_bwd2(const float* pooled, const float* w3, const float* gamma, const float* w1, const float* w2,
                    const float* dropmask, const float* save, const float* dgate, float* dpool, int cstride, int coff, int H,
                    int W, float* dw3, float* dgamma, float* dbeta, float* dw1, float* db1, float* dw2, float* db2, int N,
                    int C, int stage, double* gsum, double count_scale, float pgrad_scale, const float* tsum, const float* pstat,
                    const lhn_bn_slices* slices, void* stream) {
  LHN_CHECK_ARG(!tsum == !pstat && (!tsum || (slices && coff == 0 && C == cstride)), "lhn_ca_mlp_bwd2: tsum, pstat and slices come together (whole buffer)");
  BnSlices sl;
  if (mk_slices(tsum ? slices : nullptr, cstride, &sl, "lhn_ca_mlp_bwd2")) return 1;
  LHN_CHECK_ARG(pooled && w3 && gamma && w1 && w2 && save && dgate && dpool && dw3 && dgamma && dbeta && dw1 && db1 && dw2 && db2,
                "lhn_ca_mlp_bwd: null pointer");
  LHN_CHECK_ARG(C > 0 && C <= 256 && C % 2 == 0, "lhn_ca_mlp_bwd: C=%d", C);
  hipStream_t s = (hipStream_t)stream;
  float* dahat = const_cast<float*>(save) + (int64_t)N * C * 3 + (int64_t)N * (C / 2) + 2 * C;
  float* dvbuf = dahat + (int64_t)N * C;
  float* dhbuf = dvbuf + (int64_t)N * C;
  LHN_CHECK_ARG(stage == 0 || (gsum && stage >= 1 && stage <= 2 && count_scale >= 1), "lhn_ca_mlp_bwd: stage %d needs gsum", stage);
  if (stage != 2) hipLaunchKernelGGL(k_ca_bwd2, dim3(N), dim3(256), 0, s, w1, w2, save, dgate, dahat, dvbuf, dhbuf, N, C);
  hipLaunchKernelGGL(k_ca_bwd1, dim3((C + 31) / 32 + (C * C + C + C / 2 + 1023) / 1024), dim3(1024), 0, s, pooled, w3, gamma, dropmask, save, dahat, dpool, cstride, coff, H, W, dw3, dgamma, dbeta, N, C, 1, stage, gsum, stage ? count_scale : 1.0, stage ? pgrad_scale : 1.f, tsum, pstat, sl, dvbuf, dhbuf, dw1, db1, dw2, db2);
  LHN_CHECK_LAUNCH("lhn_ca_mlp_bwd");
  return 0;
}

int lhn_bn_bwd_reduce(const lhn_view* y, const lhn_gradview* g, const float* save, double* sums, const lhn_bnbwdfin* finp,
                      void* stream) {
  lhn_bnbwdfin fin;
  if (finp) fin = *finp; else fin.counter = nullptr;
  LHN_CHECK_ARG(lhn_view_ok(y) && g && g->dz && save && sums && y->C % 4 == 0 && y->C <= 1024 && lhn_no_pend(y), "lhn_bn_bwd_reduce: bad args");
  hipLaunchKernelGGL(k_bn_bwd_reduce, dim3(grid_cap((int64_t)y->N * y->H, 8)), dim3(256), 0, (hipStream_t)stream, *y, *g, save, sums, fin);
  LHN_CHECK_LAUNCH("lhn_bn_bwd_reduce");
  return 0;
}
int lhn_bn_bwd_finalize(const double* sums, const float* gamma, const float* save, float* coef, int cstride, int coff, int C,
                        double count, float* dgamma, float* dbeta, float pgrad_scale, void* stream) {
  return lhn_bn_bwd_finalize2(sums, gamma, save, coef, cstride, coff, C, C, count, dgamma, dbeta, pgrad_scale, stream);
}
int lhn_bn_bwd_finalize2(const double* sums, const float* gamma, const float* save, float* coef, int cstride, int coff, int C,
                         int stat_channels, double count, float* dgamma, float* dbeta, float pgrad_scale, void* stream) {
  LHN_CHECK_ARG(sums && save && coef && C > 0 && coff + C <= cstride && stat_channels >= C, "lhn_bn_bwd_finalize: bad args");
  int nt = C >= LHN_FIN_THREADS ? LHN_FIN_THREADS : (LHN_FIN_THREADS / C > LHN_STAT_REPLICAS ? LHN_STAT_REPLICAS : LHN_FIN_THREADS / C) * C;
  nt = (nt + 63) / 64 * 64;
  hipLaunchKernelGGL(k_bn_bwd_finalize, dim3(1), dim3(nt), 0, (hipStream_t)stream, sums, gamma, save, coef, cstride, coff, C, count, dgamma, dbeta, pgrad_scale, stat_channels);
  LHN_CHECK_LAUNCH("lhn_bn_bwd_finalize");
  return 0;
}
}

__global__ void __launch_bounds__(256) k_adam_flat(float* __restrict__ p, const float* __restrict__ g, float* __restrict__ m,
                                                   float* __restrict__ v, int64_t n4, int64_t n, float omb1, float b2, float omb2,
                                                   float eps, float wd, float step_size, float bc2_sqrt) {
  for (int64_t i = (int64_t)blockIdx.x * 256 + threadIdx.x; i < n4; i += (int64_t)gridDim.x * 256) {
    f4 pp = *reinterpret_cast<const f4*>(p + 4 * i), gg = *reinterpret_cast<const f4*>(g + 4 * i);
    f4 mm = *reinterpret_cast<const f4*>(m + 4 * i), vv = *reinterpret_cast<const f4*>(v + 4 * i);
    if (wd != 0.f) gg += pp * wd;
    mm += (gg - mm) * omb1;
    vv = vv * b2 + gg * gg * omb2;
    const f4 den = (f4){sqrtf(vv.x) / bc2_sqrt + eps, sqrtf(vv.y) / bc2_sqrt + eps, sqrtf(vv.z) / bc2_sqrt + eps, sqrtf(vv.w) / bc2_sqrt + eps};
    pp -= (f4){mm.x / den.x, mm.y / den.y, mm.z / den.z, mm.w / den.w} * step_size;
    *reinterpret_cast<f4*>(p + 4 * i) = pp;
    *reinterpret_cast<f4*>(m + 4 * i) = mm;
    *reinterpret_cast<f4*>(v + 4 * i) = vv;
  }
  if (blockIdx.x == 0 && threadIdx.x < (n & 3)) {
    const int64_t i = 4 * n4 + threadIdx.x;
    float gg = g[i];
    if (wd != 0.f) gg += p[i] * wd;
    const float mm = m[i] + (gg - m[i]) * omb1, vv = v[i] * b2 + gg * gg * omb2;
    p[i] -= mm / (sqrtf(vv) / bc2_sqrt + eps) * step_size;
    m[i] = mm;
    v[i] = vv;
  }
}

extern "C" int lhn_adam_step(float* param, const float* grad, float* exp_avg, float* exp_avg_sq, int64_t n, double lr, double beta1,
                             double beta2, double eps, double weight_decay, int64_t step, void* stream) {
  LHN_CHECK_ARG(param && grad && exp_avg && exp_avg_sq && n > 0 && step >= 1, "lhn_adam_step: null pointer / n / step");
  LHN_CHECK_ARG(((reinterpret_cast<uintptr_t>(param) | reinterpret_cast<uintptr_t>(grad) | reinterpret_cast<uintptr_t>(exp_avg) |
                  reinterpret_cast<uintptr_t>(exp_avg_sq)) & 15) == 0, "lhn_adam_step: buffers must be 16-byte aligned");
  const double bc1 = 1.0 - pow(beta1, (double)step), bc2 = 1.0 - pow(beta2, (double)step);
  const int64_t n4 = n / 4;
  int64_t grid = (n4 + 255) / 256;
  const int64_t cap = (int64_t)lhn_num_cus() * 8;
  if (grid > cap) grid = cap;
  if (grid < 1) grid = 1;
  hipLaunchKernelGGL(k_adam_flat, dim3((unsigned)grid), dim3(256), 0, (hipStream_t)stream, param, grad, exp_avg, exp_avg_sq, n4, n, (float)(1.0 - beta1),
                     (float)beta2, (float)(1.0 - beta2), (float)eps, (float)weight_decay, (float)(lr / bc1), (float)sqrt(bc2));
  LHN_CHECK_LAUNCH("lhn_adam_step");
  return 0;
}
```

litehandnet_amd/csrc/lhn_common.h:

```cpp
#pragma once
#include <hip/hip_runtime.h>
#include <stdint.h>
#include <stdio.h>
#include <string.h>
#include <mutex>
#include "../../include/lhn.h"

#define LHN_WAVE 64
#define LHN_DEAD (1 << 30)
#define LHN_LANE0(pl, PL) ((pl) < (PL) ? (pl) : LHN_DEAD)

void lhn_set_error(const char* fmt, ...);

#define LHN_CHECK_ARG(cond, ...)                 \
  do {                                           \
    if (!(cond)) {                               \
      lhn_set_error(__VA_ARGS__);                \
      return 1;                                  \
    }                                            \
  } while (0)

#define LHN_CHECK_LAUNCH(name)                                                    \
  do {                                                                            \
    hipError_t e__ = hipGetLastError();                                           \
    if (e__ != hipSuccess) {                                                      \
      lhn_set_error("%s: launch failed: %s", name, hipGetErrorString(e__));       \
      return 2;                                                                   \
    }                                                                             \
  } while (0)

static inline int lhn_no_pend(const lhn_view* v) { return !v || !v->pend; }

static inline int lhn_view_ok(const lhn_view* v) {
  return v && v->data && v->N > 0 && v->H > 0 && v->W > 0 && v->C > 0 && v->coff >= 0 &&
         v->coff + v->C <= v->cstride && (v->cstride % 4) == 0 && (v->coff % 4) == 0 && (v->C % 4) == 0;
}

#define LHN_MAX_DEVICES 16
static inline int lhn_device_slot() {
  int d = 0;
  if (hipGetDevice(&d) != hipSuccess || d < 0) d = 0;
  return d % LHN_MAX_DEVICES;
}
int lhn_num_cus();
bool lhn_deterministic_mode();

#ifdef __HIPCC__
template <typename F>
static inline int lhn_resident_per_cu(F kernel, size_t dyn_lds, int cap) {
  int n = 0;
  if (hipOccupancyMaxActiveBlocksPerMultiprocessor(&n, kernel, 256, dyn_lds) != hipSuccess || n < 1) n = 1;
  hipFuncAttributes a;
  if (hipFuncGetAttributes(&a, reinterpret_cast<const void*>(kernel)) == hipSuccess) {
    size_t per = (dyn_lds + a.sharedSizeBytes + 1023) / 1024 * 1024;
    const int by_lds = per ? (int)((160 * 1024) / per) : n;
    if (by_lds < n) n = by_lds;
  }
  if (n > cap) n = cap;
  return n < 1 ? 1 : n;
}

struct LhnKernelCfg {
  std::once_flag once[LHN_MAX_DEVICES];
  int per_cu[LHN_MAX_DEVICES];
  bool ok[LHN_MAX_DEVICES];
};
template <typename F>
static inline bool lhn_kernel_cfg(LhnKernelCfg& c, F kernel, size_t dyn_lds, int cap, int* per_cu) {
  const int d = lhn_device_slot();
  std::call_once(c.once[d], [&] {
    c.ok[d] = hipFuncSetAttribute(reinterpret_cast<const void*>(kernel), hipFuncAttributeMaxDynamicSharedMemorySize,
                                  (int)dyn_lds) == hipSuccess;
    c.per_cu[d] = lhn_resident_per_cu(kernel, dyn_lds, cap);
  });
  if (per_cu) *per_cu = c.per_cu[d];
  return c.ok[d];
}

typedef float f4 __attribute__((ext_vector_type(4)));
typedef float f16v __attribute__((ext_vector_type(16)));

__device__ __forceinline__ float lhn_lrelu(float v, float slope) { return v > 0.f ? v : v * slope; }
__device__ __forceinline__ float lhn_silu(float v) { return v / (1.f + expf(-v)); }
__device__ __forceinline__ float lhn_silu_grad(float v) {
  const float s = 1.f / (1.f + expf(-v));
  return s * (1.f + v * (1.f - s));
}

struct Xf4 {
  f4 sc, sh, sl;
};
__device__ __forceinline__ Xf4 lhn_load_xf(const lhn_view& v, int c_abs) {
  Xf4 t;
  if (v.table) {
    t.sc = *reinterpret_cast<const f4*>(v.table + c_abs);
    t.sh = *reinterpret_cast<const f4*>(v.table + v.cstride + c_abs);
    t.sl = *reinterpret_cast<const f4*>(v.table + 2 * v.cstride + c_abs);
  } else {
    t.sc = (f4){1.f, 1.f, 1.f, 1.f};
    t.sh = (f4){0.f, 0.f, 0.f, 0.f};
    t.sl = (f4){1.f, 1.f, 1.f, 1.f};
  }
  return t;
}
__device__ __forceinline__ f4 lhn_apply_xf(f4 raw, const Xf4& t) {
  f4 u = raw * t.sc + t.sh;
  f4 r;
  r.x = lhn_lrelu(u.x, t.sl.x);
  r.y = lhn_lrelu(u.y, t.sl.y);
  r.z = lhn_lrelu(u.z, t.sl.z);
  r.w = lhn_lrelu(u.w, t.sl.w);
  return r;
}
__device__ __forceinline__ f4 lhn_load_val(const lhn_view& v, const Xf4& t, int64_t pix, int n, int c_abs) {
  f4 raw = *reinterpret_cast<const f4*>(v.data + pix * v.cstride + c_abs);
  f4 r = lhn_apply_xf(raw, t);
  if (v.gate) r *= *reinterpret_cast<const f4*>(v.gate + (int64_t)n * v.cstride + c_abs);
  return r;
}

struct Gr4 {
  f4 A, B, Cc;
};
__device__ __forceinline__ Gr4 lhn_load_coef(const lhn_gradview& g, int cstride, int c_abs) {
  Gr4 r;
  if (g.coef) {
    r.A = *reinterpret_cast<const f4*>(g.coef + c_abs);
    r.B = *reinterpret_cast<const f4*>(g.coef + cstride + c_abs);
    r.Cc = *reinterpret_cast<const f4*>(g.coef + 2 * cstride + c_abs);
  } else {
    r.A = (f4){1.f, 1.f, 1.f, 1.f};
    r.B = (f4){0.f, 0.f, 0.f, 0.f};
    r.Cc = (f4){0.f, 0.f, 0.f, 0.f};
  }
  return r;
}
__device__ __forceinline__ int lhn_bin_lo(int i, int S) { return (i * S) / 3; }
__device__ __forceinline__ int lhn_bin_hi(int i, int S) { return ((i + 1) * S + 2) / 3; }

#define LHN_DPOOL_SLOTS 25
__device__ __forceinline__ int lhn_pool_seg(int h, int S) {
  return (h >= lhn_bin_lo(1, S)) + (h >= lhn_bin_hi(0, S)) + (h >= lhn_bin_lo(2, S)) + (h >= lhn_bin_hi(1, S));
}
__device__ __forceinline__ f4 lhn_dpool_sum(const lhn_gradview& g, const lhn_view& v, int n, int h, int w, int c_abs) {
  const int slot = lhn_pool_seg(h, v.H) * 5 + lhn_pool_seg(w, v.W);
  return *reinterpret_cast<const f4*>(g.dpool + ((int64_t)n * LHN_DPOOL_SLOTS + slot) * v.cstride + c_abs);
}
__device__ __forceinline__ void lhn_dpool_store(float* dpool, int64_t n, int cs, int c_abs, const float (&d)[9]) {
#pragma unroll
  for (int sh = 0; sh < 5; ++sh)
#pragma unroll
    for (int sw = 0; sw < 5; ++sw) {
      float v = 0.f;
#pragma unroll
      for (int bi = 0; bi < 3; ++bi)
#pragma unroll
        for (int bj = 0; bj < 3; ++bj) {
          const bool rin = (sh == 2 * bi) || (sh == 2 * bi - 1) || (sh == 2 * bi + 1);
          const bool cin = (sw == 2 * bj) || (sw == 2 * bj - 1) || (sw == 2 * bj + 1);
          if (rin && cin) v += d[bi * 3 + bj];
        }
      dpool[(n * LHN_DPOOL_SLOTS + sh * 5 + sw) * cs + c_abs] = v;
    }
}
__device__ __forceinline__ f4 lhn_grad_du(const lhn_view& v, const lhn_gradview& g, const Xf4& t, f4 raw, f4 dz,
                                          int n, int h, int w, int c_abs) {
  f4 e = dz;
  if (v.gate) e *= *reinterpret_cast<const f4*>(v.gate + (int64_t)n * v.cstride + c_abs);
  f4 u = raw * t.sc + t.sh;
  f4 du;
  du.x = e.x * (u.x > 0.f ? 1.f : t.sl.x);
  du.y = e.y * (u.y > 0.f ? 1.f : t.sl.y);
  du.z = e.z * (u.z > 0.f ? 1.f : t.sl.z);
  du.w = e.w * (u.w > 0.f ? 1.f : t.sl.w);
  if (g.dpool) {
    f4 dp = lhn_dpool_sum(g, v, n, h, w, c_abs);
    du.x += dp.x * (u.x > 0.f ? 1.f : t.sl.x);
    du.y += dp.y * (u.y > 0.f ? 1.f : t.sl.y);
    du.z += dp.z * (u.z > 0.f ? 1.f : t.sl.z);
    du.w += dp.w * (u.w > 0.f ? 1.f : t.sl.w);
  }
  return du;
}

__device__ __forceinline__ f4 lhn_dy_fast(const Xf4& t, const Gr4& gr, f4 raw, f4 dz, f4 gate) {
  const f4 u = raw * t.sc + t.sh;
  const f4 dl = (f4){u.x > 0.f ? 1.f : t.sl.x, u.y > 0.f ? 1.f : t.sl.y, u.z > 0.f ? 1.f : t.sl.z, u.w > 0.f ? 1.f : t.sl.w};
  return gr.A * (dz * gate * dl) + gr.B * raw + gr.Cc;
}

#define LHN_TICKET_WORDS 33
__device__ __forceinline__ bool lhn_last_block(unsigned* counter) {
  __shared__ int s_last;
  asm volatile("s_waitcnt vmcnt(0)" ::: "memory");
  __syncthreads();
  if (threadIdx.x == 0) {
    const unsigned nb = gridDim.x * gridDim.y, b = blockIdx.x + blockIdx.y * gridDim.x;
    const unsigned g = b & 31u, ng = nb < 32u ? nb : 32u, gsize = (nb - g + 31u) >> 5;
    int last = 0;
    if (__hip_atomic_fetch_add(counter + 1 + g, 1u, __ATOMIC_RELAXED, __HIP_MEMORY_SCOPE_AGENT) == gsize - 1u)
      last = __hip_atomic_fetch_add(counter, 1u, __ATOMIC_RELAXED, __HIP_MEMORY_SCOPE_AGENT) == ng - 1u;
    s_last = last;
  }
  __syncthreads();
  return s_last != 0;
}
__device__ __forceinline__ double lhn_ld_agent(const double* p) {
  return __hip_atomic_load(p, __ATOMIC_RELAXED, __HIP_MEMORY_SCOPE_AGENT);
}
__device__ __forceinline__ void lhn_bn_finalize_block(const lhn_bnfin& f, const double* stats) {
  const int C = f.C;
  for (int c = threadIdx.x; c < C; c += blockDim.x) {
    double s1 = 0, s2 = 0;
    for (int r = 0; r < LHN_STAT_REPLICAS; ++r) {
      s1 += lhn_ld_agent(stats + (size_t)r * 2 * C + c);
      s2 += lhn_ld_agent(stats + (size_t)r * 2 * C + C + c);
    }
    const double mean = s1 / f.count;
    double var = s2 / f.count - mean * mean;
    if (var < 0) var = 0;
    if (f.running_mean) {
      const double bm = mean + (f.conv_bias ? (double)f.conv_bias[c] : 0.0);
      f.running_mean[c] = (float)((1.0 - (double)f.momentum) * (double)f.running_mean[c] + (double)f.momentum * bm);
      const double unb = f.count > 1 ? var * f.count / (f.count - 1.0) : var;
      f.running_var[c] = (float)((1.0 - (double)f.momentum) * (double)f.running_var[c] + (double)f.momentum * unb);
    }
    const float invstd = (float)(1.0 / sqrt(var + (double)f.eps));
    const float g = f.gamma ? f.gamma[c] : 1.f, b = f.beta ? f.beta[c] : 0.f;
    const float sc = g * invstd;
    f.table[f.coff + c] = sc;
    f.table[f.cstride + f.coff + c] = b - (float)mean * sc;
    f.table[2 * f.cstride + f.coff + c] = f.slope;
    if (f.save_mean_invstd) {
      f.save_mean_invstd[c] = (float)mean;
      f.save_mean_invstd[C + c] = invstd;
    }
  }
  if (f.num_batches_tracked && threadIdx.x == 0) f.num_batches_tracked[0] += 1;
}
__device__ __forceinline__ void lhn_bn_finalize_block_par(const lhn_bnfin& f, const double* stats, double* part) {
  const int C = f.C, nt = blockDim.x, tid = threadIdx.x;
  int G = nt / C;
  G = G < 1 ? 1 : (G > LHN_STAT_REPLICAS ? LHN_STAT_REPLICAS : G);
  __syncthreads();
  for (int c0 = 0; c0 < C; c0 += nt) {
    const int g = G > 1 ? tid / C : 0, c = c0 + (G > 1 ? tid - g * C : tid);
    if (c0) __syncthreads();
    if (g < G && c < C) {
      double s1 = 0, s2 = 0;
#pragma unroll 4
      for (int r = g; r < LHN_STAT_REPLICAS; r += G) {
        s1 += lhn_ld_agent(stats + (size_t)r * 2 * C + c);
        s2 += lhn_ld_agent(stats + (size_t)r * 2 * C + C + c);
      }
      part[2 * tid] = s1;
      part[2 * tid + 1] = s2;
    }
    __syncthreads();
    if (g != 0 || c >= C) continue;
    double s1 = 0, s2 = 0;
    for (int k = 0; k < G; ++k) {
      s1 += part[2 * (k * C + tid)];
      s2 += part[2 * (k * C + tid) + 1];
    }
    const double mean = s1 / f.count;
    double var = s2 / f.count - mean * mean;
    if (var < 0) var = 0;
    if (f.running_mean) {
      const double bm = mean + (f.conv_bias ? (double)f.conv_bias[c] : 0.0);
      f.running_mean[c] = (float)((1.0 - (double)f.momentum) * (double)f.running_mean[c] + (double)f.momentum * bm);
      const double unb = f.count > 1 ? var * f.count / (f.count - 1.0) : var;
      f.running_var[c] = (float)((1.0 - (double)f.momentum) * (double)f.running_var[c] + (double)f.momentum * unb);
    }
    const float invstd = (float)(1.0 / sqrt(var + (double)f.eps));
    const float gm = f.gamma ? f.gamma[c] : 1.f, b = f.beta ? f.beta[c] : 0.f;
    const float sc = gm * invstd;
    f.table[f.coff + c] = sc;
    f.table[f.cstride + f.coff + c] = b - (float)mean * sc;
    f.table[2 * f.cstride + f.coff + c] = f.slope;
    if (f.save_mean_invstd) {
      f.save_mean_invstd[c] = (float)mean;
      f.save_mean_invstd[C + c] = invstd;
    }
  }
  if (f.num_batches_tracked && tid == 0) f.num_batches_tracked[0] += 1;
}
__device__ __forceinline__ void lhn_bn_bwd_finalize_block(const lhn_bnbwdfin& f, const double* sums, const float* save) {
  const int C = f.C;
  for (int c = threadIdx.x; c < C; c += blockDim.x) {
    double db = 0, dg = 0;
    for (int r = 0; r < LHN_STAT_REPLICAS; ++r) {
      db += lhn_ld_agent(sums + (size_t)r * 2 * C + c);
      dg += lhn_ld_agent(sums + (size_t)r * 2 * C + C + c);
    }
    const double mean = save[c], inv = save[C + c], s = (double)(f.gamma ? f.gamma[c] : 1.f) * inv;
    f.coef[f.coff + c] = (float)s;
    f.coef[f.cstride + f.coff + c] = (float)(-s * inv * dg / f.count);
    f.coef[2 * f.cstride + f.coff + c] = (float)(-s * db / f.count + s * inv * mean * dg / f.count);
    if (f.dgamma) f.dgamma[c] += (float)dg;
    if (f.dbeta) f.dbeta[c] += (float)db;
  }
}
static __device__ __forceinline__ lhn_bnfin lhn_nofin() {
  lhn_bnfin f;
  f.counter = nullptr;
  return f;
}

__device__ __forceinline__ void lhn_block_stat_atomics(f4 s, f4 q, int C4, f4* red, double* st0, double* st1, int nvalid = 64) {
  for (int o = C4; o < 64; o <<= 1) {
    s.x += __shfl_xor(s.x, o, 64); s.y += __shfl_xor(s.y, o, 64); s.z += __shfl_xor(s.z, o, 64); s.w += __shfl_xor(s.w, o, 64);
    q.x += __shfl_xor(q.x, o, 64); q.y += __shfl_xor(q.y, o, 64); q.z += __shfl_xor(q.z, o, 64); q.w += __shfl_xor(q.w, o, 64);
  }
  const int tid = threadIdx.x, lane = tid & 63, wave = tid >> 6;
  __syncthreads();
  if (lane < C4) {
    red[(wave * C4 + lane) * 2] = s;
    red[(wave * C4 + lane) * 2 + 1] = q;
  }
  __syncthreads();
  if (tid < 8 * C4) {
    const int kind = tid / (4 * C4), r = tid - kind * 4 * C4, cc = r >> 2, jj = r & 3;
    double v = 0;
#pragma unroll
    for (int wv = 0; wv < 4; ++wv) {
      const f4 a = red[(wv * C4 + cc) * 2 + kind];
      v += (double)(jj == 0 ? a.x : jj == 1 ? a.y : jj == 2 ? a.z : a.w);
    }
    if (cc < nvalid) atomicAdd((kind ? st1 : st0) + 4 * cc + jj, v);
  }
}

__device__ __forceinline__ Xf4 lhn_load_xf_t(const float* tab, int cstride, int c_abs) {
  Xf4 t;
  if (tab) {
    t.sc = *reinterpret_cast<const f4*>(tab + c_abs);
    t.sh = *reinterpret_cast<const f4*>(tab + cstride + c_abs);
    t.sl = *reinterpret_cast<const f4*>(tab + 2 * cstride + c_abs);
  } else {
    t.sc = (f4){1.f, 1.f, 1.f, 1.f};
    t.sh = (f4){0.f, 0.f, 0.f, 0.f};
    t.sl = (f4){1.f, 1.f, 1.f, 1.f};
  }
  return t;
}

struct TileStat {
  float k, s, q;
  int n;
  __device__ __forceinline__ void reset() { n = 0; k = s = q = 0.f; }
  __device__ __forceinline__ void add(float v) {
    if (n == 0) k = v;
    const float d = v - k;
    s += d;
    q += d * d;
    ++n;
  }
  __device__ __forceinline__ void flush(double& sum, double& sq) const {
    const double K = (double)k, S = (double)s;
    sum += S + (double)n * K;
    sq += (double)q + 2.0 * K * S + (double)n * K * K;
  }
};

__device__ __forceinline__ void lhn_unshift4(double (&sd)[4], double (&qd)[4], f4 s, f4 q, f4 k, int n) {
  const float sv[4] = {s.x, s.y, s.z, s.w}, qv[4] = {q.x, q.y, q.z, q.w}, kv[4] = {k.x, k.y, k.z, k.w};
#pragma unroll
  for (int j = 0; j < 4; ++j) {
    const double K = (double)kv[j], S = (double)sv[j];
    sd[j] += S + (double)n * K;
    qd[j] += (double)qv[j] + 2.0 * K * S + (double)n * K * K;
  }
}

__device__ __forceinline__ void lhn_block_stat_atomics_d(const double (&s)[4], const double (&q)[4], int C4, double* red,
                                                         double* st0, double* st1, int nvalid = 64) {
  double v[8] = {s[0], s[1], s[2], s[3], q[0], q[1], q[2], q[3]};
  for (int o = C4; o < 64; o <<= 1) {
#pragma unroll
    for (int i = 0; i < 8; ++i) v[i] += __shfl_xor(v[i], o, 64);
  }
  const int tid = threadIdx.x, lane = tid & 63, wave = tid >> 6;
  __syncthreads();
  if (lane < C4) {
#pragma unroll
    for (int i = 0; i < 8; ++i) red[(wave * C4 + lane) * 8 + i] = v[i];
  }
  __syncthreads();
  if (tid < 8 * C4) {
    const int kind = tid / (4 * C4), r = tid - kind * 4 * C4, cc = r >> 2, jj = r & 3;
    double t = 0;
#pragma unroll
    for (int wv = 0; wv < 4; ++wv) t += red[(wv * C4 + cc) * 8 + kind * 4 + jj];
    if (cc < nvalid) atomicAdd((kind ? st1 : st0) + 4 * cc + jj, t);
  }
}

__device__ __forceinline__ void lhn_bns_flush(const lhn_bnsum& b, f4 s, f4 q, int C4, f4* red) {
  double* st = b.sums + (size_t)(blockIdx.x % LHN_STAT_REPLICAS) * 2 * b.C + b.coff;
  if (C4 <= 32 && (C4 & (C4 - 1)) == 0) {
    lhn_block_stat_atomics(s, q, C4, red, st, st + b.C);
  } else {
    const int PL = 256 / C4;
    __syncthreads();
    red[threadIdx.x * 2] = s;
    red[threadIdx.x * 2 + 1] = q;
    __syncthreads();
    if ((int)threadIdx.x < C4) {
      double sd[4] = {0, 0, 0, 0}, qd[4] = {0, 0, 0, 0};
      for (int j = 0; j < PL; ++j) {
        const f4 a = red[(j * C4 + threadIdx.x) * 2], c = red[(j * C4 + threadIdx.x) * 2 + 1];
        sd[0] += a.x; sd[1] += a.y; sd[2] += a.z; sd[3] += a.w;
        qd[0] += c.x; qd[1] += c.y; qd[2] += c.z; qd[3] += c.w;
      }
#pragma unroll
      for (int j = 0; j < 4; ++j) {
        atomicAdd(st + 4 * threadIdx.x + j, sd[j]);
        atomicAdd(st + b.C + 4 * threadIdx.x + j, qd[j]);
      }
    }
  }
}
__device__ __forceinline__ f4 lhn_dact_xf(f4 raw, const Xf4& t) {
  const f4 u = raw * t.sc + t.sh;
  return (f4){u.x > 0.f ? 1.f : t.sl.x, u.y > 0.f ? 1.f : t.sl.y, u.z > 0.f ? 1.f : t.sl.z, u.w > 0.f ? 1.f : t.sl.w};
}

__device__ __forceinline__ float lhn_wave_sum(float v) {
#pragma unroll
  for (int o = 32; o > 0; o >>= 1) v += __shfl_xor(v, o, 64);
  return v;
}
__device__ __forceinline__ double lhn_wave_sum_d(double v) {
#pragma unroll
  for (int o = 32; o > 0; o >>= 1) v += __shfl_xor(v, o, 64);
  return v;
}
#endif
```

litehandnet_amd/csrc/lhn_plan.cpp:

```cpp
#include <stdint.h>
#include <stdlib.h>
#include <string.h>
#include <vector>
#include "lhn_common.h"

static lhn_bnsum mkbns(void* ws, int64_t sums_off, int64_t save_off, int C, int coff) {
  lhn_bnsum b;
  memset(&b, 0, sizeof(b));
  if (sums_off >= 0 && save_off >= 0 && C > 0) {
    b.sums = reinterpret_cast<double*>(static_cast<char*>(ws) + sums_off);
    b.save = reinterpret_cast<const float*>(static_cast<char*>(ws) + save_off);
    b.C = C;
    b.coff = coff;
  }
  return b;
}

enum {
  OP_STEM = 1, OP_PW = 2, OP_DW = 3, OP_KXK = 4, OP_FINALIZE = 5, OP_EW = 6, OP_MAXPOOL = 7, OP_AVGPOOL = 8,
  OP_CA_MLP = 9, OP_TABLE_FILL = 10, OP_MEMSET = 11, OP_ATT_MLP = 12, OP_SE_MLP = 13, OP_SHUFFLE = 14,
  OP_PWDW = 15,
  OP_STEM_BWD = 101, OP_PW_BWD = 102, OP_DW_BWD = 103, OP_KXK_BWD = 104, OP_BN_BWD = 105, OP_EW_BWD = 106,
  OP_MAXPOOL_BWD = 107, OP_AVGPOOL_BWD = 108, OP_GATE_REDUCE = 109, OP_CA_MLP_BWD = 110, OP_ATT_MLP_BWD = 111, OP_SE_MLP_BWD = 112,
  OP_SHUFFLE_BWD = 113,
};

struct GraphEntry {
  int phase, training, nrep, seen;
  int64_t rstr;
  void *ws, *io0, *io1;
  uint64_t phash, ghash;
  hipGraphExec_t exec;
  uint64_t last_use;
};

struct Plan {
  std::vector<lhn_buf> bufs;
  std::vector<lhn_op> fwd, bwd;
  std::vector<GraphEntry> graphs;
  uint64_t tick = 0;
  int graph_misses = 0;
};

static inline char* at(void* ws, int64_t off) { return off < 0 ? nullptr : static_cast<char*>(ws) + off; }

static lhn_view mkview(const Plan* P, void* ws, int buf, int coff, int C, bool with_gate = true) {
  const lhn_buf& b = P->bufs[buf];
  lhn_view v;
  v.pend = nullptr;
  v.data = reinterpret_cast<float*>(at(ws, b.data_off));
  v.table = reinterpret_cast<const float*>(at(ws, b.table_off));
  v.gate = with_gate ? reinterpret_cast<const float*>(at(ws, b.gate_off)) : nullptr;
  v.N = b.N; v.H = b.H; v.W = b.W;
  v.cstride = b.C; v.coff = coff; v.C = C;
  return v;
}
static lhn_gradview mkgrad(const Plan* P, void* ws, int buf, bool use_coef) {
  const lhn_buf& b = P->bufs[buf];
  lhn_gradview g;
  g.dz = reinterpret_cast<const float*>(at(ws, b.grad_off));
  g.dpool = reinterpret_cast<const float*>(at(ws, b.dpool_off));
  g.coef = use_coef ? reinterpret_cast<const float*>(at(ws, b.coef_off)) : nullptr;
  return g;
}
template <typename T>
static inline T* prm(void* const* arr, int idx) { return idx < 0 ? nullptr : static_cast<T*>(arr[idx]); }
static lhn_bn_slices mkslices(void* ws, const int32_t* pk, const int64_t* sv, const int64_t* sm) {
  lhn_bn_slices s;
  memset(&s, 0, sizeof(s));
  for (int k = 0; k < 2; ++k)
    if (pk[k] > 0 && sv[k] >= 0) {
      const int j = s.n++;
      s.lo[j] = pk[k] >> 16;
      s.C[j] = pk[k] & 0xffff;
      s.save[j] = reinterpret_cast<const float*>(at(ws, sv[k]));
      s.sums[j] = (sm && sm[k] >= 0) ? reinterpret_cast<double*>(at(ws, sm[k])) : nullptr;
    }
  return s;
}

static bool conv_has_bn(const lhn_op& o) { return o.p[2] >= 0 || o.p[3] >= 0 || o.ws[1] >= 0; }
static lhn_bnfin mkfin(const Plan* P, void* ws, const lhn_op& o, void* const* params) {
  const lhn_buf& b = P->bufs[o.out_buf];
  lhn_bnfin f;
  f.counter = reinterpret_cast<uint32_t*>(at(ws, o.ws[2]));
  f.gamma = prm<const float>(params, o.p[2]);
  f.beta = prm<const float>(params, o.p[3]);
  f.running_mean = prm<float>(params, o.p[4]);
  f.running_var = prm<float>(params, o.p[5]);
  f.num_batches_tracked = prm<int64_t>(params, o.p[6]);
  f.table = reinterpret_cast<float*>(at(ws, b.table_off));
  f.save_mean_invstd = reinterpret_cast<float*>(at(ws, o.ws[1]));
  f.count = (double)b.N * b.H * b.W;
  f.cstride = b.C; f.coff = o.out_coff; f.C = o.out_C;
  f.eps = o.f[0]; f.momentum = o.f[1]; f.slope = o.f[2];
  f.conv_bias = prm<const float>(params, o.p[1]);
  return f;
}
static bool fuse_finalize() {
  static int v = -1;
  if (v < 0) {
    const char* e = getenv("LHN_FUSE_FINALIZE");
    v = (e && e[0] == '1') ? 1 : 0;
  }
  return v == 1;
}
static int sep_finalize(const lhn_bnfin& f, const double* stats, int training, void* stream, int creal = 0, int repeat = 1) {
  int rc = 0;
  for (int r = 0; r < (training ? (repeat < 1 ? 1 : repeat) : 1) && !rc; ++r)
    rc = lhn_bn_finalize2(training ? stats : nullptr, f.gamma, f.beta, f.running_mean, f.running_var,
                          training ? f.num_batches_tracked : nullptr, f.table, f.cstride, f.coff, creal > 0 ? creal : f.C, f.C,
                          training ? f.save_mean_invstd : nullptr, f.count, f.eps, f.momentum, f.slope, training, f.conv_bias, stream);
  return rc;
}

extern "C" {

void* lhn_plan_create(const lhn_buf* bufs, int nbufs, const lhn_op* fwd, int nfwd, const lhn_op* bwd, int nbwd) {
  if (!bufs || nbufs <= 0 || !fwd || nfwd <= 0) {
    lhn_set_error("lhn_plan_create: empty plan");
    return nullptr;
  }
  Plan* p = new Plan();
  p->bufs.assign(bufs, bufs + nbufs);
  p->fwd.assign(fwd, fwd + nfwd);
  if (bwd && nbwd > 0) p->bwd.assign(bwd, bwd + nbwd);
  for (const auto* lst : {&p->fwd, &p->bwd})
    for (const lhn_op& o : *lst) {
      bool ok = o.out_buf < nbufs;
      for (int k = 0; k < 3; ++k) ok = ok && o.in_buf[k] < nbufs;
      if (!ok) {
        lhn_set_error("lhn_plan_create: op kind %d references buffer out of range", o.kind);
        delete p;
        return nullptr;
      }
    }
  return p;
}

void lhn_plan_destroy(void* plan) {
  Plan* p = static_cast<Plan*>(plan);
  if (!p) return;
  for (GraphEntry& g : p->graphs)
    if (g.exec) (void)hipGraphExecDestroy(g.exec);
  delete p;
}

static int run_ops(const Plan* P, int phase, void* ws, void* const* params, void* const* grads, void* const* io, int mode,
                   int nrep, int64_t rstr, void* stream, size_t sb = 0, size_t se = (size_t)-1, double cscale = 1.0,
                   float pscale = 1.f) {
  const int training = mode & 1;
  const bool skip_tables = (mode & 2) != 0 && !training;
  const std::vector<lhn_op>& ops = phase == 0 ? P->fwd : P->bwd;
  hipStream_t s = static_cast<hipStream_t>(stream);
  int rc = 0;
  const bool whole = (sb == 0 && se >= 2 * ops.size());
  for (size_t oi = 0; oi < ops.size() && rc == 0; ++oi) {
    const lhn_op& o = ops[oi];
    const bool deferred = false;
    const bool is_conv = o.kind == OP_STEM || o.kind == OP_PW || o.kind == OP_DW || o.kind == OP_KXK;
    const bool fz = is_conv && training && fuse_finalize() && whole && !(o.kind == OP_PW && o.i[2] > 0) &&
                    !((o.kind == OP_PW || o.kind == OP_DW) && (int)o.f[3] > 1);
    const bool h0 = 2 * oi >= sb && 2 * oi < se, h1 = 2 * oi + 1 >= sb && 2 * oi + 1 < se;
    if (!h0 && !h1) continue;
    const bool two_half = o.kind == OP_STEM || o.kind == OP_PW || o.kind == OP_DW || o.kind == OP_KXK || o.kind == OP_CA_MLP ||
                          o.kind == OP_ATT_MLP || o.kind == OP_BN_BWD || o.kind == OP_CA_MLP_BWD || o.kind == OP_ATT_MLP_BWD;
    if (!two_half && !h0) continue;
    const int stage = (h0 && h1) ? 0 : (h0 ? 1 : 2);
    switch (o.kind) {
      case OP_MEMSET: {
        if (hipMemsetAsync(at(ws, o.ws[0]), 0, (size_t)o.ws[1], s) != hipSuccess) {
          lhn_set_error("lhn_plan_run: memset failed");
          rc = 2;
        }
        break;
      }
      case OP_TABLE_FILL: {
        if (skip_tables) break;
        const lhn_buf& b = P->bufs[o.out_buf];
        if (o.i[0])
          rc = lhn_table_bias(reinterpret_cast<float*>(at(ws, b.table_off)), b.C, o.out_coff, o.out_C, prm<const float>(params, o.p[0]), o.f[2], stream);
        else
          rc = lhn_table_fill(reinterpret_cast<float*>(at(ws, b.table_off)), b.C, o.out_coff, o.out_C, o.f[0], o.f[1], o.f[2], stream);
        break;
      }
      case OP_STEM: {
        lhn_view y = mkview(P, ws, o.out_buf, o.out_coff, o.out_C);
        const bool bn = conv_has_bn(o);
        lhn_bnfin fin;
        if (bn) {
          fin = mkfin(P, ws, o, params);
          fin.count *= cscale;
        }
        if (h0) rc = lhn_conv_stem_fwd(static_cast<const float*>(io[0]), prm<const float>(params, o.p[0]), &y,
                               (training && o.ws[0] >= 0) ? reinterpret_cast<double*>(at(ws, o.ws[0])) : nullptr, o.i[3], o.i[4], o.i[0], o.i[1],
                               o.i[2], (bn && fz) ? &fin : nullptr, stream);
        if (!rc && bn && h1 && !skip_tables && !deferred && !fz) rc = sep_finalize(fin, reinterpret_cast<const double*>(at(ws, o.ws[0])), training, stream);
        break;
      }
      case OP_PW: {
        lhn_view x = mkview(P, ws, o.in_buf[0], o.in_coff[0], o.in_C[0]);
        lhn_view y;
        float* nchw = nullptr;
        if (o.i[1]) {
          y = x;
          y.data = nullptr; y.table = nullptr; y.gate = nullptr; y.pend = nullptr;
          y.cstride = o.out_C; y.coff = 0; y.C = o.out_C;
          nchw = static_cast<float*>(io[1]);
        } else {
          y = mkview(P, ws, o.out_buf, o.out_coff, o.out_C);
        }
        const bool bn = !o.i[1] && conv_has_bn(o);
        lhn_bnfin fin;
        if (bn) {
          fin = mkfin(P, ws, o, params);
          fin.count *= cscale;
        }
        lhn_pw_opts po;
        memset(&po, 0, sizeof(po));
        po.w_rows = o.i[2]; po.w_cols = o.i[3];
        lhn_view extra[2];
        if (o.i[6] > 1) {
          po.n_extra = o.i[6] - 1;
          for (int e = 0; e < po.n_extra; ++e) {
            extra[e] = mkview(P, ws, o.in_buf[e + 1], o.in_coff[e + 1], o.in_C[e + 1]);
          }
          po.extra = extra;
          for (int e = 0; e < 3; ++e) po.coef[e] = o.f[4 + e];
        }
        lhn_view sumv;
        if (o.i[6] > 1 && o.ws[4] >= 0) {
          sumv = x;
          sumv.data = reinterpret_cast<float*>(at(ws, o.ws[4]));
          sumv.table = nullptr; sumv.gate = nullptr; sumv.pend = nullptr;
          sumv.cstride = (int)(o.ws[5] >> 16); sumv.coff = (int)(o.ws[5] & 0xffff);
          po.sum_out = &sumv;
        }
        if (nchw && o.i[5] > 1) {
          const int64_t khw = (int64_t)o.out_C * y.H * y.W;
          nchw += (int64_t)o.i[4] * khw;
          po.nchw_batch_stride = (int64_t)o.i[5] * khw;
        }
        if (h0) rc = lhn_conv_pw_fwd2(&x, prm<const float>(params, o.p[0]), bn ? nullptr : prm<const float>(params, o.p[1]), &y,
                              (training && o.ws[0] >= 0) ? reinterpret_cast<double*>(at(ws, o.ws[0])) : nullptr, o.i[0], nchw,
                              (bn && fz) ? &fin : nullptr, &po, stream);
        if (!rc && bn && h1 && !skip_tables && !deferred && !fz)
          rc = sep_finalize(fin, reinterpret_cast<const double*>(at(ws, o.ws[0])), training, stream, o.i[2], (int)o.f[3]);
        break;
      }
      case OP_DW: {
        lhn_view x = mkview(P, ws, o.in_buf[0], o.in_coff[0], o.in_C[0]);
        lhn_view y = mkview(P, ws, o.out_buf, o.out_coff, o.out_C);
        const bool bn = conv_has_bn(o);
        lhn_bnfin fin;
        if (bn) {
          fin = mkfin(P, ws, o, params);
          fin.count *= cscale;
        }
        lhn_view extra;
        const float coef2[2] = {o.f[4], o.f[5]};
        if (o.i[6] > 1) {
          extra = mkview(P, ws, o.in_buf[1], o.in_coff[1], o.in_C[1]);
        }
        lhn_view sumv;
        const bool so = o.i[6] > 1 && o.ws[4] >= 0;
        if (so) {
          sumv = x;
          sumv.data = reinterpret_cast<float*>(at(ws, o.ws[4]));
          sumv.table = nullptr; sumv.gate = nullptr; sumv.pend = nullptr;
          sumv.cstride = (int)(o.ws[5] >> 16); sumv.coff = (int)(o.ws[5] & 0xffff);
        }
        if (h0) rc = lhn_conv_dw_fwd3(&x, prm<const float>(params, o.p[0]), &y,
                              (training && o.ws[0] >= 0) ? reinterpret_cast<double*>(at(ws, o.ws[0])) : nullptr, o.i[0], o.i[1], o.i[2], o.i[3],
                              (bn && fz) ? &fin : nullptr, o.i[6] > 1 ? &extra : nullptr, coef2,
                              so ? &sumv : nullptr, stream);
        if (!rc && bn && h1 && !skip_tables && !deferred && !fz)
          rc = sep_finalize(fin, reinterpret_cast<const double*>(at(ws, o.ws[0])), training, stream, 0, (int)o.f[3]);
        break;
      }
      case OP_KXK: {
        lhn_view x = mkview(P, ws, o.in_buf[0], o.in_coff[0], o.in_C[0]);
        lhn_view y = mkview(P, ws, o.out_buf, o.out_coff, o.out_C);
        const bool bn = conv_has_bn(o);
        lhn_bnfin fin;
        if (bn) {
          fin = mkfin(P, ws, o, params);
          fin.count *= cscale;
        }
        if (h0) rc = lhn_conv_kxk_fwd(&x, prm<const float>(params, o.p[0]), &y,
                              (training && o.ws[0] >= 0) ? reinterpret_cast<double*>(at(ws, o.ws[0])) : nullptr, o.i[0],
                              (bn && fz) ? &fin : nullptr,
                              o.ws[3] >= 0 ? reinterpret_cast<float*>(at(ws, o.ws[3])) : nullptr, stream);
        if (!rc && bn && h1 && !skip_tables && !deferred && !fz) rc = sep_finalize(fin, reinterpret_cast<const double*>(at(ws, o.ws[0])), training, stream);
        break;
      }
      case OP_PWDW: {
        if (training) {
          lhn_set_error("lhn_plan_run: a fused 1x1 -> depthwise launch has no batch statistics (inference plans only)");
          rc = 1;
          break;
        }
        lhn_view x = mkview(P, ws, o.in_buf[0], o.in_coff[0], o.in_C[0]);
        lhn_view y = mkview(P, ws, o.out_buf, o.out_coff, o.out_C);
        rc = lhn_conv_pw_dw3_fwd(&x, prm<const float>(params, o.p[0]), reinterpret_cast<const float*>(at(ws, P->bufs[o.in_buf[1]].table_off)),
                                 prm<const float>(params, o.p[1]), &y, stream);
        break;
      }
      case OP_FINALIZE: {
        if (skip_tables) break;
        const lhn_buf& b = P->bufs[o.out_buf];
        const int src = o.in_buf[0] >= 0 ? o.in_buf[0] : o.out_buf;
        const lhn_buf& sb = P->bufs[src];
        rc = lhn_bn_finalize(reinterpret_cast<const double*>(at(ws, o.ws[0])), prm<const float>(params, o.p[0]),
                             prm<const float>(params, o.p[1]), prm<float>(params, o.p[2]), prm<float>(params, o.p[3]),
                             prm<int64_t>(params, o.p[4]), reinterpret_cast<float*>(at(ws, b.table_off)), b.C, o.out_coff,
                             o.out_C, reinterpret_cast<float*>(at(ws, o.ws[1])), (double)sb.N * sb.H * sb.W, o.f[0], o.f[1],
                             o.f[2], training, nullptr, stream);
        break;
      }
      case OP_EW: {
        lhn_view srcs[3];
        for (int k = 0; k < o.i[0]; ++k) {
          srcs[k] = mkview(P, ws, o.in_buf[k], o.in_coff[k], o.in_C[k]);
        }
        lhn_view d = mkview(P, ws, o.out_buf, o.out_coff, o.out_C);
        const float coef[3] = {o.f[4], o.f[5], o.f[6]};
        rc = lhn_ew_fwd3(srcs, o.i[0], o.i[1] ? coef : nullptr, &d, o.f[0], o.i[2], stream);
        break;
      }
      case OP_MAXPOOL: {
        lhn_view x = mkview(P, ws, o.in_buf[0], o.in_coff[0], o.in_C[0]);
        lhn_view y = mkview(P, ws, o.out_buf, o.out_coff, o.out_C);
        rc = lhn_maxpool2_fwd(&x, &y, stream);
        break;
      }
      case OP_SHUFFLE: {
        lhn_view a = mkview(P, ws, o.in_buf[0], o.in_coff[0], o.in_C[0]);
        lhn_view b = mkview(P, ws, o.in_buf[1], o.in_coff[1], o.in_C[1]);
        lhn_view d = mkview(P, ws, o.out_buf, o.out_coff, o.out_C);
        rc = lhn_shuffle2_fwd(&a, &b, &d, stream);
        break;
      }
      case OP_AVGPOOL: {
        lhn_view x = mkview(P, ws, o.in_buf[0], o.in_coff[0], o.in_C[0], o.i[2] == 0);
        if (o.ws[1] >= 0 || o.in_buf[1] >= 0) {
          const lhn_bn_slices sl = mkslices(ws, &o.i[5], &o.ws[2], nullptr);
          lhn_view src;
          if (o.in_buf[1] >= 0) src = mkview(P, ws, o.in_buf[1], o.in_coff[1], o.in_C[1]);
          rc = lhn_avgpool_fwd4(&x, reinterpret_cast<float*>(at(ws, o.ws[0])), o.i[0], o.i[1],
                                o.ws[1] >= 0 ? reinterpret_cast<float*>(at(ws, o.ws[1])) : nullptr, &sl, o.in_buf[1] >= 0 ? &src : nullptr, stream);
          break;
        }
        rc = lhn_avgpool_fwd2(&x, reinterpret_cast<float*>(at(ws, o.ws[0])), o.i[0], o.i[1], o.i[3] > 0 ? o.i[3] : x.C, o.i[4], stream);
        break;
      }
      case OP_CA_MLP: {
        const lhn_buf& b = P->bufs[o.out_buf];
        if ((!training || o.ws[3] < 0) && !h0) break;
        rc = lhn_ca_mlp_fwd(reinterpret_cast<const float*>(at(ws, o.ws[0])), prm<const float>(params, o.p[0]),
                            prm<const float>(params, o.p[1]), prm<const float>(params, o.p[2]), prm<float>(params, o.p[3]),
                            prm<float>(params, o.p[4]), prm<int64_t>(params, o.p[5]), prm<const float>(params, o.p[6]),
                            prm<const float>(params, o.p[7]), prm<const float>(params, o.p[8]), prm<const float>(params, o.p[9]),
                            (training && o.ws[2] >= 0) ? reinterpret_cast<const float*>(at(ws, o.ws[2])) : nullptr,
                            reinterpret_cast<float*>(at(ws, b.gate_off)), b.C, o.out_coff,
                            reinterpret_cast<float*>(at(ws, o.ws[1])), b.N, o.out_C, o.f[0], o.f[1], training,
                            (training && o.ws[3] >= 0) ? stage : 0, o.ws[3] >= 0 ? reinterpret_cast<double*>(at(ws, o.ws[3])) : nullptr,
                            cscale, stream);
        break;
      }
      case OP_ATT_MLP: {
        const lhn_buf& b = P->bufs[o.out_buf];
        if ((!training || o.ws[3] < 0) && !h0) break;
        rc = lhn_att_mlp_fwd(reinterpret_cast<const float*>(at(ws, o.ws[0])), prm<const float>(params, o.p[0]),
                             prm<const float>(params, o.p[1]), prm<float>(params, o.p[2]), prm<float>(params, o.p[3]),
                             prm<int64_t>(params, o.p[4]), prm<const float>(params, o.p[5]), prm<const float>(params, o.p[6]),
                             prm<const float>(params, o.p[7]), prm<const float>(params, o.p[8]),
                             (training && o.ws[2] >= 0) ? reinterpret_cast<const float*>(at(ws, o.ws[2])) : nullptr,
                             reinterpret_cast<float*>(at(ws, b.gate_off)), b.C, o.out_coff,
                             reinterpret_cast<float*>(at(ws, o.ws[1])), b.N, o.out_C, o.f[0], o.f[1], training,
                             (training && o.ws[3] >= 0) ? stage : 0, o.ws[3] >= 0 ? reinterpret_cast<double*>(at(ws, o.ws[3])) : nullptr,
                             cscale, stream);
        break;
      }
      case OP_SE_MLP: {
        const lhn_buf& b = P->bufs[o.out_buf];
        rc = lhn_se_mlp_fwd2(reinterpret_cast<const float*>(at(ws, o.ws[0])), prm<const float>(params, o.p[0]),
                             prm<const float>(params, o.p[1]), prm<const float>(params, o.p[2]), prm<const float>(params, o.p[3]),
                             reinterpret_cast<float*>(at(ws, b.gate_off)), b.C, o.out_coff, reinterpret_cast<float*>(at(ws, o.ws[1])),
                             b.N, o.out_C, o.i[0], o.i[1], stream);
        break;
      }
      case OP_STEM_BWD: {
        lhn_view y = mkview(P, ws, o.out_buf, o.out_coff, o.out_C);
        lhn_gradview g = mkgrad(P, ws, o.out_buf, o.i[5] != 0);
        rc = lhn_conv_stem_bwd(static_cast<const float*>(io[0]), &y, &g, prm<float>(grads, o.p[1]), o.i[3], o.i[4], o.i[0],
                               o.i[1], o.i[2], nrep, rstr, stream);
        break;
      }
      case OP_PW_BWD: {
        lhn_view x = mkview(P, ws, o.in_buf[0], o.in_coff[0], o.in_C[0]);
        lhn_view y;
        lhn_gradview g;
        const float* nchw = nullptr;
        if (o.i[1]) {
          y = x;
          y.data = nullptr; y.table = nullptr; y.gate = nullptr;
          y.cstride = o.out_C; y.coff = 0; y.C = o.out_C;
          g.dz = nullptr; g.dpool = nullptr; g.coef = nullptr;
          nchw = static_cast<const float*>(io[1]);
        } else {
          y = mkview(P, ws, o.out_buf, o.out_coff, o.out_C);
          g = mkgrad(P, ws, o.out_buf, o.i[5] != 0);
        }
        float* dx = o.i[2] ? reinterpret_cast<float*>(at(ws, P->bufs[o.in_buf[0]].grad_off)) : nullptr;
        lhn_pw_opts po;
        memset(&po, 0, sizeof(po));
        po.w_rows = o.i[3]; po.w_cols = o.i[4];
        if (nchw && o.i[7] > 1) {
          const int64_t khw = (int64_t)o.out_C * y.H * y.W;
          nchw += (int64_t)o.i[6] * khw;
          po.nchw_batch_stride = (int64_t)o.i[7] * khw;
        }
        const lhn_bnsum bs = mkbns(ws, o.ws[0], o.ws[1], (int)o.f[6], (int)o.f[7]);
        rc = lhn_conv_pw_bwd3(&x, prm<const float>(params, o.p[0]), &y, &g, dx, o.i[2] == 2, prm<float>(grads, o.p[1]),
                              prm<float>(grads, o.p[2]), o.i[0], nchw, nrep, rstr, &po, bs.sums ? &bs : nullptr, stream);
        break;
      }
      case OP_DW_BWD: {
        lhn_view x = mkview(P, ws, o.in_buf[0], o.in_coff[0], o.in_C[0]);
        lhn_view y = mkview(P, ws, o.out_buf, o.out_coff, o.out_C);
        lhn_gradview g = mkgrad(P, ws, o.out_buf, o.i[5] != 0);
        float* dx = o.i[4] ? reinterpret_cast<float*>(at(ws, P->bufs[o.in_buf[0]].grad_off)) : nullptr;
        if (o.ws[2] >= 0 || o.ws[3] >= 0) {
          rc = lhn_conv_dw_bwd3(&x, prm<const float>(params, o.p[0]), &y, &g, dx, o.i[4] == 2, prm<float>(grads, o.p[1]), o.i[0], o.i[1],
                                o.i[2], o.i[3], nrep, rstr, o.ws[2] >= 0 ? reinterpret_cast<const float*>(at(ws, o.ws[2])) : nullptr,
                                o.ws[3] >= 0 ? reinterpret_cast<const float*>(at(ws, o.ws[3])) : nullptr, stream);
          break;
        }
        rc = lhn_conv_dw_bwd2(&x, prm<const float>(params, o.p[0]), &y, &g, dx, o.i[4] == 2, prm<float>(grads, o.p[1]), o.i[0],
                              o.i[1], o.i[2], o.i[3], nrep, rstr, o.ws[4] >= 0 ? reinterpret_cast<double*>(at(ws, o.ws[4])) : nullptr,
                              o.ws[5] >= 0 ? reinterpret_cast<const float*>(at(ws, o.ws[5])) : nullptr, o.i[6], o.i[7], stream);
        break;
      }
      case OP_KXK_BWD: {
        lhn_view x = mkview(P, ws, o.in_buf[0], o.in_coff[0], o.in_C[0]);
        lhn_view y = mkview(P, ws, o.out_buf, o.out_coff, o.out_C);
        lhn_gradview g = mkgrad(P, ws, o.out_buf, o.i[5] != 0);
        float* dx = o.i[2] ? reinterpret_cast<float*>(at(ws, P->bufs[o.in_buf[0]].grad_off)) : nullptr;
        rc = lhn_conv_kxk_bwd(&x, prm<const float>(params, o.p[0]), &y, &g, dx, o.i[2] == 2, prm<float>(grads, o.p[1]), o.i[0],
                              nrep, rstr, o.ws[3] >= 0 ? reinterpret_cast<float*>(at(ws, o.ws[3])) : nullptr, stream);
        break;
      }
      case OP_BN_BWD: {
        const lhn_buf& b = P->bufs[o.out_buf];
        lhn_view y = mkview(P, ws, o.out_buf, o.out_coff, o.out_C);
        lhn_gradview g = mkgrad(P, ws, o.out_buf, false);
        double* sums = reinterpret_cast<double*>(at(ws, o.ws[0]));
        const float* save = reinterpret_cast<const float*>(at(ws, o.ws[1]));
        lhn_bnbwdfin fin;
        fin.counter = reinterpret_cast<uint32_t*>(at(ws, o.ws[2]));
        fin.gamma = prm<const float>(params, o.p[0]);
        fin.coef = reinterpret_cast<float*>(at(ws, b.coef_off));
        fin.dgamma = prm<float>(grads, o.p[1]);
        fin.dbeta = prm<float>(grads, o.p[2]);
        fin.count = (double)b.N * b.H * b.W * cscale;
        fin.cstride = b.C; fin.coff = o.out_coff; fin.C = o.out_C;
        if (fin.counter && fuse_finalize() && whole && !o.i[1]) {
          rc = lhn_bn_bwd_reduce(&y, &g, save, sums, &fin, stream);
        } else {
          if (h0 && !o.i[1]) rc = lhn_bn_bwd_reduce(&y, &g, save, sums, nullptr, stream);
          if (!rc && h1)
            rc = lhn_bn_bwd_finalize2(sums, fin.gamma, save, fin.coef, b.C, o.out_coff, o.i[0] > 0 ? o.i[0] : o.out_C, o.out_C, fin.count,
                                      fin.dgamma, fin.dbeta, pscale, stream);
        }
        break;
      }
      case OP_EW_BWD: {
        lhn_view src = mkview(P, ws, o.in_buf[0], o.in_coff[0], o.in_C[0]);
        lhn_view d = mkview(P, ws, o.out_buf, o.out_coff, o.out_C);
        const lhn_buf& db = P->bufs[o.out_buf];
        if (o.i[1] == 1) {
          lhn_view other = mkview(P, ws, o.in_buf[1], o.in_coff[1], o.in_C[1]);
          rc = lhn_ew_mul_bwd(&src, &other, &d, reinterpret_cast<const float*>(at(ws, db.grad_off)),
                              reinterpret_cast<float*>(at(ws, P->bufs[o.in_buf[0]].grad_off)), o.i[0], stream);
        } else if (o.i[1] == 2) {
          rc = lhn_bilinear_bwd(&src, &d, reinterpret_cast<const float*>(at(ws, db.grad_off)),
                                reinterpret_cast<float*>(at(ws, P->bufs[o.in_buf[0]].grad_off)), o.i[0], o.f[0], stream);
        } else if (o.i[1] == 3) {
          lhn_view srcs[3];
          float* dsrcs[3];
          int acc[3] = {o.i[0], o.i[2], o.i[3]};
          lhn_bnsum bsv[3] = {mkbns(ws, o.ws[0], o.ws[1], o.i[4], o.i[5]), mkbns(ws, o.ws[2], o.ws[3], o.i[6], o.i[7]),
                              mkbns(ws, o.ws[4], o.ws[5], (int)o.f[4], (int)o.f[5])};
          const lhn_bnsum* bsp[3];
          int ns = 0;
          for (; ns < 3 && o.in_buf[ns] >= 0; ++ns) {
            srcs[ns] = mkview(P, ws, o.in_buf[ns], o.in_coff[ns], o.in_C[ns]);
            dsrcs[ns] = reinterpret_cast<float*>(at(ws, P->bufs[o.in_buf[ns]].grad_off));
            bsp[ns] = bsv[ns].sums ? &bsv[ns] : nullptr;
          }
          rc = lhn_ew_bwd_multi(srcs, ns, &d, reinterpret_cast<const float*>(at(ws, db.grad_off)),
                                reinterpret_cast<const float*>(at(ws, db.dpool_off)), o.f[0], dsrcs, acc, bsp, stream);
        } else {
          const lhn_bnsum bs = mkbns(ws, o.ws[0], o.ws[1], o.i[4], o.i[5]);
          rc = lhn_ew_bwd3(&src, &d, reinterpret_cast<const float*>(at(ws, db.grad_off)),
                           reinterpret_cast<const float*>(at(ws, db.dpool_off)), o.f[0],
                           reinterpret_cast<float*>(at(ws, P->bufs[o.in_buf[0]].grad_off)), o.i[0], bs.sums ? &bs : nullptr, stream);
        }
        break;
      }
      case OP_MAXPOOL_BWD: {
        lhn_view x = mkview(P, ws, o.in_buf[0], o.in_coff[0], o.in_C[0]);
        lhn_view y = mkview(P, ws, o.out_buf, o.out_coff, o.out_C);
        const lhn_bnsum bs = mkbns(ws, o.ws[0], o.ws[1], o.i[4], o.i[5]);
        lhn_grad_adds ad;
        memset(&ad, 0, sizeof(ad));
        if (o.ws[2] >= 0) {
          ad.same = reinterpret_cast<const float*>(at(ws, o.ws[2]));
          ad.same_cstride = o.i[1]; ad.same_coff = o.i[2];
        }
        if (o.ws[3] >= 0) {
          ad.pooled = reinterpret_cast<const float*>(at(ws, o.ws[3]));
          ad.pooled_cstride = o.i[3]; ad.pooled_coff = o.i[6];
          ad.OH = o.i[7] >> 16; ad.OW = o.i[7] & 0xffff;
        }
        rc = lhn_maxpool2_bwd3(&x, &y, reinterpret_cast<const float*>(at(ws, P->bufs[o.out_buf].grad_off)),
                               reinterpret_cast<float*>(at(ws, P->bufs[o.in_buf[0]].grad_off)), o.i[0], bs.sums ? &bs : nullptr,
                               (ad.same || ad.pooled) ? &ad : nullptr, stream);
        break;
      }
      case OP_AVGPOOL_BWD: {
        lhn_view x = mkview(P, ws, o.in_buf[0], o.in_coff[0], o.in_C[0]);
        const lhn_bnsum bs = mkbns(ws, o.ws[1], o.ws[2], o.i[5], o.i[6]);
        rc = lhn_avgpool_bwd3(&x, reinterpret_cast<const float*>(at(ws, o.ws[0])), o.i[0], o.i[1], o.i[3] > 0 ? o.i[3] : x.C, o.i[4],
                              reinterpret_cast<float*>(at(ws, P->bufs[o.in_buf[0]].grad_off)), o.i[2], bs.sums ? &bs : nullptr, stream);
        break;
      }
      case OP_SHUFFLE_BWD: {
        lhn_view a = mkview(P, ws, o.in_buf[0], o.in_coff[0], o.in_C[0]);
        lhn_view b = mkview(P, ws, o.in_buf[1], o.in_coff[1], o.in_C[1]);
        lhn_view d = mkview(P, ws, o.out_buf, o.out_coff, o.out_C);
        rc = lhn_shuffle2_bwd(&a, &b, &d, reinterpret_cast<const float*>(at(ws, P->bufs[o.out_buf].grad_off)),
                              o.i[0] ? reinterpret_cast<float*>(at(ws, P->bufs[o.in_buf[0]].grad_off)) : nullptr, o.i[0] == 2,
                              o.i[1] ? reinterpret_cast<float*>(at(ws, P->bufs[o.in_buf[1]].grad_off)) : nullptr, o.i[1] == 2, stream);
        break;
      }
      case OP_GATE_REDUCE: {
        lhn_view y = mkview(P, ws, o.out_buf, o.out_coff, o.out_C, false);
        float* dg = reinterpret_cast<float*>(at(ws, o.ws[3]));
        const lhn_bn_slices sl = mkslices(ws, &o.i[0], &o.ws[5], nullptr);
        rc = lhn_gate_bwd_reduce3(&y, reinterpret_cast<const float*>(at(ws, P->bufs[o.out_buf].grad_off)), dg,
                                  o.ws[4] >= 0 ? dg + (size_t)y.N * y.C : nullptr, &sl, 1, stream);
        break;
      }
      case OP_CA_MLP_BWD: {
        const lhn_buf& b = P->bufs[o.out_buf];
        if (o.ws[4] < 0 && !h0) break;
        const lhn_bn_slices sl = mkslices(ws, &o.i[0], &o.ws[6], &o.ws[8]);
        const float* dgp = reinterpret_cast<const float*>(at(ws, o.ws[3]));
        rc = lhn_ca_mlp_bwd2(reinterpret_cast<const float*>(at(ws, o.ws[0])), prm<const float>(params, o.p[0]),
                            prm<const float>(params, o.p[1]), prm<const float>(params, o.p[2]), prm<const float>(params, o.p[3]),
                            o.ws[2] >= 0 ? reinterpret_cast<const float*>(at(ws, o.ws[2])) : nullptr,
                            reinterpret_cast<const float*>(at(ws, o.ws[1])), reinterpret_cast<const float*>(at(ws, o.ws[3])),
                            reinterpret_cast<float*>(at(ws, b.dpool_off)), b.C, o.out_coff, b.H, b.W, prm<float>(grads, o.p[4]),
                            prm<float>(grads, o.p[5]), prm<float>(grads, o.p[6]), prm<float>(grads, o.p[7]),
                            prm<float>(grads, o.p[8]), prm<float>(grads, o.p[9]), prm<float>(grads, o.p[10]), b.N, o.out_C,
                            o.ws[4] >= 0 ? stage : 0, o.ws[4] >= 0 ? reinterpret_cast<double*>(at(ws, o.ws[4])) : nullptr, cscale, pscale,
                            o.ws[5] >= 0 ? dgp + (size_t)b.N * b.C : nullptr, o.ws[5] >= 0 ? reinterpret_cast<const float*>(at(ws, o.ws[5])) : nullptr,
                            &sl, stream);
        break;
      }
      case OP_ATT_MLP_BWD: {
        const lhn_buf& b = P->bufs[o.out_buf];
        if (o.ws[4] < 0 && !h0) break;
        rc = lhn_att_mlp_bwd(reinterpret_cast<const float*>(at(ws, o.ws[0])), prm<const float>(params, o.p[0]),
                             prm<const float>(params, o.p[1]), prm<const float>(params, o.p[2]), prm<const float>(params, o.p[3]),
                             o.ws[2] >= 0 ? reinterpret_cast<const float*>(at(ws, o.ws[2])) : nullptr,
                             reinterpret_cast<float*>(at(ws, o.ws[1])), reinterpret_cast<const float*>(at(ws, o.ws[3])),
                             reinterpret_cast<float*>(at(ws, b.dpool_off)), b.C, o.out_coff, b.H, b.W, prm<float>(grads, o.p[4]),
                             prm<float>(grads, o.p[5]), prm<float>(grads, o.p[6]), prm<float>(grads, o.p[7]),
                             prm<float>(grads, o.p[8]), prm<float>(grads, o.p[9]), b.N, o.out_C,
                             o.ws[4] >= 0 ? stage : 0, o.ws[4] >= 0 ? reinterpret_cast<double*>(at(ws, o.ws[4])) : nullptr, cscale, pscale,
                             stream);
        break;
      }
      case OP_SE_MLP_BWD: {
        const lhn_buf& b = P->bufs[o.out_buf];
        rc = lhn_se_mlp_bwd2(reinterpret_cast<const float*>(at(ws, o.ws[0])), prm<const float>(params, o.p[0]),
                             prm<const float>(params, o.p[1]), reinterpret_cast<const float*>(at(ws, o.ws[1])),
                             reinterpret_cast<const float*>(at(ws, o.ws[3])), reinterpret_cast<float*>(at(ws, b.dpool_off)), b.C,
                             o.out_coff, b.H, b.W, prm<float>(grads, o.p[2]), prm<float>(grads, o.p[3]), prm<float>(grads, o.p[4]),
                             prm<float>(grads, o.p[5]), b.N, o.out_C, o.i[0], o.i[1], stream);
        break;
      }
      default:
        lhn_set_error("lhn_plan_run: unknown op kind %d at index %zu", o.kind, oi);
        rc = 1;
    }
  }
  return rc;
}

int lhn_plan_run_range(void* plan, int phase, int64_t step_begin, int64_t step_end, void* ws, void* const* params,
                       void* const* grads, void* const* io, int training, int grad_replicas, int64_t grad_rep_stride,
                       double count_scale, float pgrad_scale, void* stream) {
  LHN_CHECK_ARG(plan && ws && params && io && step_begin >= 0 && step_end >= step_begin && count_scale >= 1, "lhn_plan_run_range: bad argument");
  LHN_CHECK_ARG(phase == 0 || (phase == 1 && grads), "lhn_plan_run_range: phase %d", phase);
  return run_ops(static_cast<const Plan*>(plan), phase, ws, params, grads, io, training, grad_replicas < 1 ? 1 : grad_replicas,
                 grad_rep_stride, stream, (size_t)step_begin, (size_t)step_end, count_scale, pgrad_scale);
}

static bool graphs_enabled() {
  static int v = -1;
  if (v < 0) {
    const char* e = getenv("LHN_GRAPH");
    v = (e && e[0] == '1') ? 1 : 0;
  }
  return v == 1;
}
static uint64_t hash_ptrs(void* const* a, const std::vector<lhn_op>& ops, bool grads) {
  uint64_t h = 1469598103934665603ull;
  if (!a) return h;
  for (const lhn_op& o : ops)
    for (int k = 0; k < 12; ++k)
      if (o.p[k] >= 0) {
        h ^= reinterpret_cast<uint64_t>(a[o.p[k]]);
        h *= 1099511628211ull;
      }
  (void)grads;
  return h;
}

int lhn_plan_run(void* plan, int phase, void* ws, void* const* params, void* const* grads, void* const* io, int training,
                 int grad_replicas, int64_t grad_rep_stride, void* stream) {
  const int nrep = grad_replicas < 1 ? 1 : grad_replicas;
  const int64_t rstr = grad_rep_stride;
  LHN_CHECK_ARG(plan && ws && params && io, "lhn_plan_run: null argument");
  LHN_CHECK_ARG(phase == 0 || (phase == 1 && grads), "lhn_plan_run: phase %d", phase);
  Plan* P = static_cast<Plan*>(plan);
  const bool want_graph = graphs_enabled() || (training & LHN_RUN_GRAPH) != 0;
  training &= ~LHN_RUN_GRAPH;
  if (!want_graph || stream == nullptr || P->graph_misses > 64) return run_ops(P, phase, ws, params, grads, io, training, nrep, rstr, stream);
  const std::vector<lhn_op>& ops = phase == 0 ? P->fwd : P->bwd;
  const uint64_t ph = hash_ptrs(params, ops, false), gh = phase == 1 ? hash_ptrs(grads, ops, true) : 0;
  hipStream_t s = static_cast<hipStream_t>(stream);
  GraphEntry* e = nullptr;
  for (GraphEntry& g : P->graphs)
    if (g.phase == phase && g.training == training && g.nrep == nrep && g.rstr == rstr && g.ws == ws && g.io0 == io[0] &&
        g.io1 == io[1] && g.phash == ph && g.ghash == gh) {
      e = &g;
      break;
    }
  ++P->tick;
  if (e && e->exec) {
    e->last_use = P->tick;
    if (hipGraphLaunch(e->exec, s) != hipSuccess) {
      lhn_set_error("lhn_plan_run: hipGraphLaunch failed");
      return 2;
    }
    return 0;
  }
  if (!e) {
    ++P->graph_misses;
    if (P->graphs.size() >= 8) {
      size_t victim = 0;
      for (size_t i = 1; i < P->graphs.size(); ++i)
        if (P->graphs[i].last_use < P->graphs[victim].last_use) victim = i;
      if (P->graphs[victim].exec) (void)hipGraphExecDestroy(P->graphs[victim].exec);
      P->graphs.erase(P->graphs.begin() + victim);
    }
    P->graphs.push_back(GraphEntry{phase, training, nrep, 1, rstr, ws, io[0], io[1], ph, gh, nullptr, P->tick});
    return run_ops(P, phase, ws, params, grads, io, training, nrep, rstr, stream);
  }
  e->last_use = P->tick;
  hipGraph_t graph = nullptr;
  if (hipStreamBeginCapture(s, hipStreamCaptureModeRelaxed) != hipSuccess)
    return run_ops(P, phase, ws, params, grads, io, training, nrep, rstr, stream);
  const int rc = run_ops(P, phase, ws, params, grads, io, training, nrep, rstr, stream);
  const hipError_t ec = hipStreamEndCapture(s, &graph);
  if (rc != 0 || ec != hipSuccess || !graph) {
    if (graph) (void)hipGraphDestroy(graph);
    (void)hipGetLastError();
    P->graph_misses = 1000;
    return rc != 0 ? rc : run_ops(P, phase, ws, params, grads, io, training, nrep, rstr, stream);
  }
  hipGraphExec_t exec = nullptr;
  const hipError_t ei = hipGraphInstantiate(&exec, graph, nullptr, nullptr, 0);
  (void)hipGraphDestroy(graph);
  if (ei != hipSuccess || !exec) {
    (void)hipGetLastError();
    P->graph_misses = 1000;
    return run_ops(P, phase, ws, params, grads, io, training, nrep, rstr, stream);
  }
  e->exec = exec;
  P->graph_misses = 0;
  if (hipGraphLaunch(exec, s) != hipSuccess) {
    lhn_set_error("lhn_plan_run: hipGraphLaunch failed");
    return 2;
  }
  return 0;
}
}
```

Before: 8210 images/s.

## Add latency-optimized channel-attention kernels and optional fused gate-reduce MLP backward tail

Adds LDS-staged variants of the channel-attention MLP forward and backward kernels that preload the weight matrices into shared memory with vector loads. It also adds a restructured bwd1 kernel that folds the weight-gradient blocks into the same launch. Separately, an env-gated path (LHN_CA_TAIL=1) uses per-sample atomic tickets so the last gate-reduce block runs the MLP backward for that sample, removing a separate launch. The aim is to cut small-kernel latency on the many tiny per-sample MLPs. The tail path adds a ticket buffer and relies on memory-ordering correctness; it is off by default, while the new lat kernels run when their guards pass.

```diff
diff --git a/litehandnet_amd/csrc/k_misc.hip b/litehandnet_amd/csrc/k_misc.hip
--- a/litehandnet_amd/csrc/k_misc.hip
+++ b/litehandnet_amd/csrc/k_misc.hip
@@ -748,8 +748,52 @@
   }
 }
 
+template <bool AGENT>
+__device__ __forceinline__ void ca_bwd2_sample(const float* __restrict__ w1, const float* __restrict__ w2, const float* save,
+                                               const float* dgate, float* dahat, float* dvbuf, float* dhbuf, int N, int C, int n,
+                                               float* sdv, float* sdh, float* shh) {
+  const int Ch = C / 2;
+  const float* h = save + (int64_t)N * C * 2 + (int64_t)n * Ch;
+  const float* g = save + (int64_t)N * C * 2 + (int64_t)N * Ch + (int64_t)n * C;
+  for (int c = threadIdx.x; c < C; c += blockDim.x) {
+    const float gg = g[c];
+    const float dgv = AGENT ? __hip_atomic_load(dgate + (int64_t)n * C + c, __ATOMIC_RELAXED, __HIP_MEMORY_SCOPE_AGENT) : dgate[(int64_t)n * C + c];
+    const float dv = dgv * gg * (1.f - gg);
+    sdv[c] = dv;
+    dvbuf[(int64_t)n * C + c] = dv;
+  }
+  for (int j = threadIdx.x; j < Ch; j += blockDim.x) shh[j] = h[j];
+  __syncthreads();
+  for (int j = threadIdx.x; j < Ch; j += blockDim.x) {
+    float d = 0.f;
+#pragma unroll 8
+    for (int c = 0; c < C; ++c) d += w2[c * Ch + j] * sdv[c];
+    d *= shh[j] > 0.f ? 1.f : 0.01f;
+    sdh[j] = d;
+    dhbuf[(int64_t)n * Ch + j] = d;
+  }
+  __syncthreads();
+  for (int c = threadIdx.x; c < C; c += blockDim.x) {
+    float d = 0.f;
+#pragma unroll 8
+    for (int j = 0; j < Ch; ++j) d += w1[j * C + c] * sdh[j];
+    dahat[(int64_t)n * C + c] = d;
+  }
+}
+struct CaTail {
+  unsigned* tickets;
+  const float* w1;
+  const float* w2;
+  const float* save;
+  float* dahat;
+  float* dvbuf;
+  float* dhbuf;
+  int N, C;
+};
+
 __global__ void __launch_bounds__(256) k_gate_bwd_reduce(lhn_view y, const float* __restrict__ dz,
-                                                         float* __restrict__ dgate, float* __restrict__ tsum, BnSlices sl) {
+                                                         float* __restrict__ dgate, float* __restrict__ tsum, BnSlices sl,
+                                                         CaTail tail) {
   __shared__ f4 red[768];
   const int C4 = y.C >> 2, PL = 256 / C4, n = blockIdx.x;
   const int c4 = threadIdx.x % C4, pl = threadIdx.x / C4;
@@ -798,6 +842,21 @@
       atomicAdd(o1 + 0, u1.x); atomicAdd(o1 + 1, u1.y); atomicAdd(o1 + 2, u1.z); atomicAdd(o1 + 3, u1.w);
     }
   }
+  if (tail.tickets) {
+    __shared__ int s_last;
+    asm volatile("s_waitcnt vmcnt(0)" ::: "memory");
+    __syncthreads();
+    if (threadIdx.x == 0) {
+      const int last = __hip_atomic_fetch_add(tail.tickets + n, 1u, __ATOMIC_RELAXED, __HIP_MEMORY_SCOPE_AGENT) == gridDim.y - 1u;
+      if (last) __hip_atomic_store(tail.tickets + n, 0u, __ATOMIC_RELAXED, __HIP_MEMORY_SCOPE_AGENT);
+      s_last = last;
+    }
+    __syncthreads();
+    if (s_last) {
+      float* sdv = reinterpret_cast<float*>(red);
+      ca_bwd2_sample<true>(tail.w1, tail.w2, tail.save, dgate, tail.dahat, tail.dvbuf, tail.dhbuf, tail.N, tail.C, n, sdv, sdv + 256, sdv + 384);
+    }
+  }
 }
 
 __global__ void __launch_bounds__(256) k_ca_bwd2(const float* __restrict__ w1, const float* __restrict__ w2,
@@ -805,32 +864,7 @@
                                                  float* __restrict__ dahat , float* __restrict__ dvbuf ,
                                                  float* __restrict__ dhbuf , int N, int C) {
   __shared__ float sdv[256], sdh[128], shh[128];
-  const int Ch = C / 2, n = blockIdx.x;
-  const float* h = save + (int64_t)N * C * 2 + (int64_t)n * Ch;
-  const float* g = save + (int64_t)N * C * 2 + (int64_t)N * Ch + (int64_t)n * C;
-  for (int c = threadIdx.x; c < C; c += blockDim.x) {
-    const float gg = g[c];
-    const float dv = dgate[(int64_t)n * C + c] * gg * (1.f - gg);
-    sdv[c] = dv;
-    dvbuf[(int64_t)n * C + c] = dv;
-  }
-  for (int j = threadIdx.x; j < Ch; j += blockDim.x) shh[j] = h[j];
-  __syncthreads();
-  for (int j = threadIdx.x; j < Ch; j += blockDim.x) {
-    float d = 0.f;
-#pragma unroll 8
-    for (int c = 0; c < C; ++c) d += w2[c * Ch + j] * sdv[c];
-    d *= shh[j] > 0.f ? 1.f : 0.01f;
-    sdh[j] = d;
-    dhbuf[(int64_t)n * Ch + j] = d;
-  }
-  __syncthreads();
-  for (int c = threadIdx.x; c < C; c += blockDim.x) {
-    float d = 0.f;
-#pragma unroll 8
-    for (int j = 0; j < Ch; ++j) d += w1[j * C + c] * sdh[j];
-    dahat[(int64_t)n * C + c] = d;
-  }
+  ca_bwd2_sample<false>(w1, w2, save, dgate, dahat, dvbuf, dhbuf, N, C, blockIdx.x, sdv, sdh, shh);
 }
 __global__ void __launch_bounds__(1024) k_ca_bwd1(const float* __restrict__ pooled, const float* __restrict__ w3,
                                                  const float* __restrict__ gamma, const float* __restrict__ mask,
@@ -988,6 +1022,422 @@
   }
 }
 
+#define CA_NS 2
+#define CA_W4 8
+#define CA_BWD1_LDS 53248
+
+template <bool MASK>
+__global__ void __launch_bounds__(1024) k_ca1_lat(const float* __restrict__ pooled, const float* __restrict__ w3,
+                                                 const float* __restrict__ gamma, const float* __restrict__ beta,
+                                                 float* __restrict__ rmean, float* __restrict__ rvar, int64_t* __restrict__ nbt,
+                                                 const float* __restrict__ mask, float* __restrict__ save, int N, int C,
+                                                 float eps, float momentum, int training) {
+  __shared__ double rs[32][32], rq[32][32];
+  __shared__ float s_sc[32], s_sh[32];
+  float* a = save;
+  float* ahat = save + (int64_t)N * C;
+  float* smean = save + (int64_t)N * C * 3 + (int64_t)N * (C / 2);
+  float* sinv = smean + C;
+  const int cl = threadIdx.x & 31, nl = threadIdx.x >> 5, c = blockIdx.x * 32 + cl;
+  const bool ok = c < C;
+  const int cc = ok ? c : C - 1;
+  float wt[9], pv[CA_NS][9], mk[CA_NS];
+#pragma unroll
+  for (int t = 0; t < 9; ++t) wt[t] = w3[cc * 9 + t];
+#pragma unroll
+  for (int i = 0; i < CA_NS; ++i) {
+    const int64_t nn = min(nl + 32 * i, N - 1);
+#pragma unroll
+    for (int t = 0; t < 9; ++t) pv[i][t] = pooled[(nn * 9 + t) * C + cc];
+    mk[i] = MASK ? mask[nn * C + cc] : 1.f;
+  }
+  float gm = 0.f, bt = 0.f, rm = 0.f, rv = 0.f;
+  if (gamma) {
+    gm = gamma[cc];
+    bt = beta[cc];
+    rm = rmean[cc];
+    rv = rvar[cc];
+  } else if (beta) {
+    bt = beta[cc];
+  }
+  if (!ok) {
+#pragma unroll
+    for (int t = 0; t < 9; ++t) wt[t] = 0.f;
+  }
+  float v[CA_NS];
+  double s = 0, q = 0;
+#pragma unroll
+  for (int i = 0; i < CA_NS; ++i) {
+    const int n = nl + 32 * i;
+    v[i] = 0.f;
+#pragma unroll
+    for (int t = 0; t < 9; ++t) v[i] += pv[i][t] * wt[t];
+    if (ok && n < N) {
+      a[(int64_t)n * C + c] = v[i];
+      s += v[i];
+      q += (double)v[i] * v[i];
+    }
+  }
+  rs[nl][cl] = s;
+  rq[nl][cl] = q;
+  __syncthreads();
+  if (nl == 0 && ok) {
+    for (int j = 1; j < 32; ++j) {
+      s += rs[j][cl];
+      q += rq[j][cl];
+    }
+    const double NT = (double)N;
+    double mean, var;
+    if (!gamma) {
+      smean[c] = 0.f;
+      sinv[c] = 1.f;
+      s_sc[cl] = 1.f;
+      s_sh[cl] = bt;
+    } else {
+      if (training) {
+        mean = s / NT;
+        var = q / NT - mean * mean;
+        if (var < 0) var = 0;
+        rmean[c] = (float)((1.0 - (double)momentum) * rm + (double)momentum * mean);
+        rvar[c] = (float)((1.0 - (double)momentum) * rv + (double)momentum * (NT > 1 ? var * NT / (NT - 1.0) : var));
+      } else {
+        mean = rm;
+        var = rv;
+      }
+      const float invstd = (float)(1.0 / sqrt(var + (double)eps));
+      smean[c] = (float)mean;
+      sinv[c] = invstd;
+      s_sc[cl] = gm * invstd;
+      s_sh[cl] = bt - (float)mean * (gm * invstd);
+    }
+  }
+  __syncthreads();
+  if (ok) {
+    const float sc = s_sc[cl], sh = s_sh[cl];
+#pragma unroll
+    for (int i = 0; i < CA_NS; ++i) {
+      const int n = nl + 32 * i;
+      float o = v[i] * sc + sh;
+      if (MASK) o *= mk[i];
+      if (n < N) ahat[(int64_t)n * C + c] = o;
+    }
+  }
+  if (training && nbt && blockIdx.x == 0 && threadIdx.x == 0) nbt[0] += 1;
+}
+
+__device__ __forceinline__ void ca_w_load(const float* __restrict__ w, int n4, f4 (&x)[CA_W4]) {
+#pragma unroll
+  for (int u = 0; u < CA_W4; ++u) x[u] = reinterpret_cast<const f4*>(w)[min((int)threadIdx.x + u * 256, n4 - 1)];
+}
+__device__ __forceinline__ void ca_w_store(float* lds, int n4, int L, int ls, const f4 (&x)[CA_W4]) {
+#pragma unroll
+  for (int u = 0; u < CA_W4; ++u) {
+    const int e = ((int)threadIdx.x + u * 256) * 4;
+    if (e < n4 * 4) *reinterpret_cast<f4*>(lds + (e / L) * ls + e % L) = x[u];
+  }
+}
+__global__ void __launch_bounds__(256) k_ca2_lat(const float* __restrict__ w1, const float* __restrict__ b1,
+                                                 const float* __restrict__ w2, const float* __restrict__ b2,
+                                                 float* __restrict__ save, float* __restrict__ gate, int gs, int gcoff, int N,
+                                                 int C) {
+  extern __shared__ __align__(16) float ca_lds[];
+  const int n = blockIdx.x, Ch = C / 2, S1 = C + 4, S2 = Ch + 4, n4 = C * Ch / 4, tid = threadIdx.x;
+  float* sw1 = ca_lds;
+  float* sw2 = sw1 + Ch * S1;
+  float* sa = sw2 + C * S2;
+  float* shh = sa + C;
+  const float* ahat = save + (int64_t)N * C + (int64_t)n * C;
+  float* h = save + (int64_t)N * C * 2 + (int64_t)n * Ch;
+  float* g = save + (int64_t)N * C * 2 + (int64_t)N * Ch + (int64_t)n * C;
+  f4 x1[CA_W4], x2[CA_W4];
+  ca_w_load(w1, n4, x1);
+  ca_w_load(w2, n4, x2);
+  const float av = ahat[min(tid, C - 1)], bj = b1[min(tid, Ch - 1)], bc = b2[min(tid, C - 1)];
+  ca_w_store(sw1, n4, C, S1, x1);
+  ca_w_store(sw2, n4, Ch, S2, x2);
+  if (tid < C) sa[tid] = av;
+  __syncthreads();
+  if (tid < Ch) {
+    float v = bj;
+    for (int c = 0; c < C; c += 4) {
+      const f4 w = *reinterpret_cast<const f4*>(sw1 + tid * S1 + c), x = *reinterpret_cast<const f4*>(sa + c);
+      v = fmaf(w.x, x.x, v);
+      v = fmaf(w.y, x.y, v);
+      v = fmaf(w.z, x.z, v);
+      v = fmaf(w.w, x.w, v);
+    }
+    v = lhn_lrelu(v, 0.01f);
+    h[tid] = v;
+    shh[tid] = v;
+  }
+  __syncthreads();
+  if (tid < C) {
+    float v = bc;
+    for (int j = 0; j < Ch; j += 4) {
+      const f4 w = *reinterpret_cast<const f4*>(sw2 + tid * S2 + j), x = *reinterpret_cast<const f4*>(shh + j);
+      v = fmaf(w.x, x.x, v);
+      v = fmaf(w.y, x.y, v);
+      v = fmaf(w.z, x.z, v);
+      v = fmaf(w.w, x.w, v);
+    }
+    const float sg = 1.f / (1.f + expf(-v));
+    g[tid] = sg;
+    gate[(int64_t)n * gs + gcoff + tid] = sg;
+  }
+}
+__global__ void __launch_bounds__(256) k_ca_bwd2_lat(const float* __restrict__ w1, const float* __restrict__ w2,
+                                                     const float* __restrict__ save, const float* __restrict__ dgate,
+                                                     float* __restrict__ dahat, float* __restrict__ dvbuf,
+                                                     float* __restrict__ dhbuf, int N, int C) {
+  extern __shared__ __align__(16) float ca_lds[];
+  const int n = blockIdx.x, Ch = C / 2, n4 = C * Ch / 4, tid = threadIdx.x;
+  float* sw2 = ca_lds;
+  float* sw1 = sw2 + C * Ch;
+  float* sdv = sw1 + C * Ch;
+  float* sdh = sdv + C;
+  float* shh = sdh + Ch;
+  const float* h = save + (int64_t)N * C * 2 + (int64_t)n * Ch;
+  const float* g = save + (int64_t)N * C * 2 + (int64_t)N * Ch + (int64_t)n * C;
+  f4 x1[CA_W4], x2[CA_W4];
+  ca_w_load(w2, n4, x2);
+  ca_w_load(w1, n4, x1);
+  const float gg = g[min(tid, C - 1)], dg = dgate[(int64_t)n * C + min(tid, C - 1)], hv = h[min(tid, Ch - 1)];
+  if (tid < C) {
+    const float dv = dg * gg * (1.f - gg);
+    sdv[tid] = dv;
+    dvbuf[(int64_t)n * C + tid] = dv;
+  }
+  if (tid < Ch) shh[tid] = hv;
+  ca_w_store(sw2, n4, Ch, Ch, x2);
+  ca_w_store(sw1, n4, C, C, x1);
+  __syncthreads();
+  if (tid < Ch) {
+    float d = 0.f;
+#pragma unroll 8
+    for (int c = 0; c < C; ++c) d += sw2[c * Ch + tid] * sdv[c];
+    d *= shh[tid] > 0.f ? 1.f : 0.01f;
+    sdh[tid] = d;
+    dhbuf[(int64_t)n * Ch + tid] = d;
+  }
+  __syncthreads();
+  if (tid < C) {
+    float d = 0.f;
+#pragma unroll 8
+    for (int j = 0; j < Ch; ++j) d += sw1[j * C + tid] * sdh[j];
+    dahat[(int64_t)n * C + tid] = d;
+  }
+}
+
+__device__ __forceinline__ void ca_pgrad_block(float* lds, int b, const float* __restrict__ save, const float* __restrict__ dvbuf,
+                                               const float* __restrict__ dhbuf, float* __restrict__ dw1, float* __restrict__ db1,
+                                               float* __restrict__ dw2, float* __restrict__ db2, int N, int C, int nb2, int nb1,
+                                               int nch) {
+  const int Ch = C / 2, nw = C * Ch, tid = threadIdx.x;
+  if (b >= nb2 + nb1) {
+    if (tid >= C + Ch) return;
+    const bool is2 = tid < C;
+    const float* src = is2 ? dvbuf + tid : dhbuf + (tid - C);
+    const int wd = is2 ? C : Ch;
+    float* dst = is2 ? db2 + tid : db1 + (tid - C);
+    float x[32 * CA_NS];
+    const float old = *dst;
+#pragma unroll
+    for (int u = 0; u < 32 * CA_NS; ++u) x[u] = src[(int64_t)min(u, N - 1) * wd];
+    float v = 0.f;
+#pragma unroll
+    for (int u = 0; u < 32 * CA_NS; ++u)
+      if (u < N) v += x[u];
+    *dst = old + v;
+    return;
+  }
+  const bool is2 = b < nb2;
+  const int L = is2 ? Ch : C, RW = is2 ? C : Ch;
+  const float* full = is2 ? save + (int64_t)N * C * 2 : save + (int64_t)N * C;
+  const float* cols = is2 ? dvbuf : dhbuf;
+  float* dst = is2 ? dw2 : dw1;
+  const int o0 = (is2 ? b : b - nb2) * 1024, o = o0 + tid;
+  const int r0 = o0 / L, nr = min(RW - 1, (o0 + 1023) / L) - r0 + 1;
+  const bool live = o < nw;
+  const int r = live ? o / L - r0 : 0, k = live ? o % L : 0;
+  const float old = dst[live ? o : 0];
+  float* sfull = lds;
+  float* scol = lds + nch * L;
+  float v = 0.f;
+  for (int n0 = 0; n0 < N; n0 += nch) {
+    const int nn = min(nch, N - n0), t4 = nn * L / 4, te = nn * nr;
+    f4 xf[2];
+    float xc[3];
+#pragma unroll
+    for (int u = 0; u < 2; ++u) xf[u] = reinterpret_cast<const f4*>(full + (int64_t)n0 * L)[min(tid + u * 1024, t4 - 1)];
+#pragma unroll
+    for (int u = 0; u < 3; ++u) {
+      const int e = min(tid + u * 1024, te - 1);
+      xc[u] = cols[(int64_t)(n0 + e / nr) * RW + r0 + e % nr];
+    }
+    if (n0) __syncthreads();
+#pragma unroll
+    for (int u = 0; u < 2; ++u)
+      if (tid + u * 1024 < t4) reinterpret_cast<f4*>(sfull)[tid + u * 1024] = xf[u];
+#pragma unroll
+    for (int u = 0; u < 3; ++u)
+      if (tid + u * 1024 < te) scol[tid + u * 1024] = xc[u];
+    __syncthreads();
+#pragma unroll 8
+    for (int n = 0; n < nn; ++n) v += scol[n * nr + r] * sfull[n * L + k];
+  }
+  if (live) dst[o] = old + v;
+}
+
+template <bool MASK, bool TS>
+__global__ void __launch_bounds__(1024) k_ca_bwd1_lat(const float* __restrict__ pooled, const float* __restrict__ w3,
+                                                     const float* __restrict__ gamma, const float* __restrict__ mask,
+                                                     const float* __restrict__ save, const float* __restrict__ dahat,
+                                                     float* __restrict__ dpool, int cs, int coff, int H, int W,
+                                                     float* __restrict__ dw3, float* __restrict__ dgamma,
+                                                     float* __restrict__ dbeta, int N, int C, const float* __restrict__ tsum,
+                                                     const float* __restrict__ pstat, BnSlices sl,
+                                                     const float* __restrict__ dvbuf, const float* __restrict__ dhbuf,
+                                                     float* __restrict__ dw1, float* __restrict__ db1, float* __restrict__ dw2,
+                                                     float* __restrict__ db2, int nb2, int nb1, int nch) {
+  extern __shared__ __align__(16) float ca_lds[];
+  const int nmain = (C + 31) / 32;
+  if ((int)blockIdx.x >= nmain) {
+    ca_pgrad_block(ca_lds, (int)blockIdx.x - nmain, save, dvbuf, dhbuf, dw1, db1, dw2, db2, N, C, nb2, nb1, nch);
+    return;
+  }
+  double (*rs)[32] = reinterpret_cast<double (*)[32]>(ca_lds);
+  double (*rq)[32] = rs + 32;
+  float (*rw)[32][9] = reinterpret_cast<float (*)[32][9]>(ca_lds + 4096);
+  const float* a = save;
+  const float* smean = save + (int64_t)N * C * 3 + (int64_t)N * (C / 2);
+  const float* sinv = smean + C;
+  const float* gsave = save + (int64_t)N * C * 2 + (int64_t)N * (C / 2);
+  const int cl = threadIdx.x & 31, nl = threadIdx.x >> 5, c = blockIdx.x * 32 + cl;
+  const bool ok = c < C;
+  const int cc = ok ? c : C - 1;
+  float mean = smean[cc], invstd = sinv[cc], gm = gamma[cc];
+  float wt[9], d[CA_NS], av[CA_NS], pv[CA_NS][9], gs[CA_NS], ts0[CA_NS], ts1[CA_NS], ps0[CA_NS][9], ps1[CA_NS][9];
+#pragma unroll
+  for (int t = 0; t < 9; ++t) wt[t] = w3[cc * 9 + t];
+#pragma unroll
+  for (int i = 0; i < CA_NS; ++i) {
+    const int64_t nn = min(nl + 32 * i, N - 1);
+    d[i] = dahat[nn * C + cc];
+    if (MASK) d[i] *= mask[nn * C + cc];
+    av[i] = a[nn * C + cc];
+#pragma unroll
+    for (int t = 0; t < 9; ++t) pv[i][t] = pooled[(nn * 9 + t) * C + cc];
+    if (TS) {
+      gs[i] = gsave[nn * C + cc];
+      ts0[i] = tsum[(nn * 2 + 0) * C + cc];
+      ts1[i] = tsum[(nn * 2 + 1) * C + cc];
+#pragma unroll
+      for (int t = 0; t < 9; ++t) {
+        ps0[i][t] = pstat[((nn * 9 + t) * 2 + 0) * C + cc];
+        ps1[i][t] = pstat[((nn * 9 + t) * 2 + 1) * C + cc];
+      }
+    }
+  }
+  float og = 0.f, ob = 0.f, ow[9];
+  if (nl == 0) {
+    og = dgamma[cc];
+    ob = dbeta[cc];
+#pragma unroll
+    for (int t = 0; t < 9; ++t) ow[t] = dw3[cc * 9 + t];
+  }
+  if (!ok) {
+    mean = invstd = gm = 0.f;
+#pragma unroll
+    for (int t = 0; t < 9; ++t) wt[t] = 0.f;
+  }
+  double sd = 0, sdx = 0;
+  float xh[CA_NS];
+#pragma unroll
+  for (int i = 0; i < CA_NS; ++i) {
+    xh[i] = (av[i] - mean) * invstd;
+    if (ok && nl + 32 * i < N) {
+      sd += d[i];
+      sdx += (double)d[i] * xh[i];
+    }
+  }
+  rs[nl][cl] = sd;
+  rq[nl][cl] = sdx;
+  __syncthreads();
+  sd = 0;
+  sdx = 0;
+  for (int j = 0; j < 32; ++j) {
+    sd += rs[j][cl];
+    sdx += rq[j][cl];
+  }
+  const double NT = (double)N;
+  if (nl == 0 && ok) {
+    dgamma[c] = og + (float)sdx;
+    dbeta[c] = ob + (float)sd;
+  }
+  double bs0 = 0, bs1 = 0;
+  float dwt[9], binv[9];
+#pragma unroll
+  for (int t = 0; t < 9; ++t) {
+    dwt[t] = 0.f;
+    const int bi = t / 3, bj = t % 3;
+    binv[t] = 1.f / (float)((lhn_bin_hi(bi, H) - lhn_bin_lo(bi, H)) * (lhn_bin_hi(bj, W) - lhn_bin_lo(bj, W)));
+  }
+#pragma unroll
+  for (int i = 0; i < CA_NS; ++i) {
+    const int n = nl + 32 * i;
+    if (ok && n < N) {
+      const float da = gm * invstd * (d[i] - (float)(sd / NT) - xh[i] * (float)(sdx / NT));
+      float dseg[9];
+#pragma unroll
+      for (int t = 0; t < 9; ++t) {
+        dwt[t] += da * pv[i][t];
+        dseg[t] = da * wt[t] * binv[t];
+      }
+      lhn_dpool_store(dpool, n, cs, coff + c, dseg);
+      if (TS) {
+        float a0 = gs[i] * ts0[i], a1 = gs[i] * ts1[i];
+#pragma unroll
+        for (int t = 0; t < 9; ++t) {
+          a0 += dseg[t] * ps0[i][t];
+          a1 += dseg[t] * ps1[i][t];
+        }
+        bs0 += a0;
+        bs1 += a1;
+      }
+    }
+  }
+  if (TS) {
+    __syncthreads();
+    rs[nl][cl] = bs0;
+    rq[nl][cl] = bs1;
+  }
+#pragma unroll
+  for (int t = 0; t < 9; ++t) rw[nl][cl][t] = dwt[t];
+  __syncthreads();
+  if (nl == 0 && ok) {
+    if (TS) {
+      double t0 = 0, t1 = 0;
+      for (int j = 0; j < 32; ++j) {
+        t0 += rs[j][cl];
+        t1 += rq[j][cl];
+      }
+      const int cb = coff + c;
+#pragma unroll
+      for (int k = 0; k < 2; ++k)
+        if (k < sl.n && sl.sums[k] && cb >= sl.lo[k] && cb < sl.lo[k] + sl.C[k]) {
+          sl.sums[k][cb - sl.lo[k]] = t0;
+          sl.sums[k][sl.C[k] + cb - sl.lo[k]] = t1;
+        }
+    }
+#pragma unroll
+    for (int t = 0; t < 9; ++t) {
+      float v = 0.f;
+      for (int j = 0; j < 32; ++j) v += rw[j][cl][t];
+      dw3[c * 9 + t] = ow[t] + v;
+    }
+  }
+}
+
 __global__ void __launch_bounds__(256) k_bn_bwd_reduce(lhn_view y, lhn_gradview g, const float* __restrict__ save,
                                                        double* __restrict__ sums, lhn_bnbwdfin fin) {
   __shared__ f4 red[512];
@@ -1370,6 +1820,20 @@
   return 0;
 }
 
+#define CA_MV_LDS_MAX ((128 * 128 + 8 * 128) * 4)
+static bool ca_lat_enabled() {
+  static const bool on = [] {
+    const char* e = getenv("LHN_CA_LAT");
+    return !(e && e[0] == '0');
+  }();
+  return on;
+}
+static inline bool ca_lat_ok(int stage, int N, int C, const float* save) {
+  return ca_lat_enabled() && stage == 0 && N <= 32 * CA_NS && C % 8 == 0 && (reinterpret_cast<uintptr_t>(save) & 15) == 0;
+}
+static inline bool ca_mv_ok(int C, const float* save, const float* w1, const float* w2) {
+  return ca_lat_enabled() && C % 8 == 0 && C <= 128 && ((reinterpret_cast<uintptr_t>(save) | reinterpret_cast<uintptr_t>(w1) | reinterpret_cast<uintptr_t>(w2)) & 15) == 0;
+}
 int lhn_ca_mlp_fwd(const float* pooled, const float* w3, const float* gamma, const float* beta, float* rmean, float* rvar,
                    int64_t* nbt, const float* w1, const float* b1, const float* w2, const float* b2, const float* dropmask,
                    float* gate, int gate_stride, int gate_coff, float* save, int N, int C, float eps, float momentum,
@@ -1379,8 +1843,19 @@
   LHN_CHECK_ARG(C > 0 && C <= 256 && C % 2 == 0 && N > 0, "lhn_ca_mlp_fwd: C=%d (<=256)", C);
   hipStream_t s = (hipStream_t)stream;
   LHN_CHECK_ARG(stage == 0 || (gsum && stage >= 1 && stage <= 2 && count_scale >= 1), "lhn_ca_mlp_fwd: stage %d needs gsum", stage);
-  hipLaunchKernelGGL(k_ca1, dim3((C + 31) / 32), dim3(1024), 0, s, pooled, w3, gamma, beta, rmean, rvar, nbt, dropmask, save, N, C, eps, momentum, training, stage, gsum, stage ? count_scale : 1.0);
-  if (stage != 1) hipLaunchKernelGGL(k_ca2, dim3(N), dim3(128), 0, s, w1, b1, w2, b2, save, gate, gate_stride, gate_coff, N, C);
+  if (ca_lat_ok(stage, N, C, save)) {
+    if (dropmask) hipLaunchKernelGGL(k_ca1_lat<true>, dim3((C + 31) / 32), dim3(1024), 0, s, pooled, w3, gamma, beta, rmean, rvar, nbt, dropmask, save, N, C, eps, momentum, training);
+    else hipLaunchKernelGGL(k_ca1_lat<false>, dim3((C + 31) / 32), dim3(1024), 0, s, pooled, w3, gamma, beta, rmean, rvar, nbt, dropmask, save, N, C, eps, momentum, training);
+  } else {
+    hipLaunchKernelGGL(k_ca1, dim3((C + 31) / 32), dim3(1024), 0, s, pooled, w3, gamma, beta, rmean, rvar, nbt, dropmask, save, N, C, eps, momentum, training, stage, gsum, stage ? count_scale : 1.0);
+  }
+  static LhnKernelCfg cfg2;
+  if (stage != 1) {
+    if (ca_mv_ok(C, save, w1, w2) && lhn_kernel_cfg(cfg2, k_ca2_lat, CA_MV_LDS_MAX, 1, nullptr))
+      hipLaunchKernelGGL(k_ca2_lat, dim3(N), dim3(256), (size_t)(C * C + 8 * C) * 4, s, w1, b1, w2, b2, save, gate, gate_stride, gate_coff, N, C);
+    else
+      hipLaunchKernelGGL(k_ca2, dim3(N), dim3(128), 0, s, w1, b1, w2, b2, save, gate, gate_stride, gate_coff, N, C);
+  }
   LHN_CHECK_LAUNCH("lhn_ca_mlp_fwd");
   return 0;
 }
@@ -1393,6 +1868,10 @@
 }
 int lhn_gate_bwd_reduce3(const lhn_view* y, const float* dz, float* dgate, float* tsum, const lhn_bn_slices* slices, int prezeroed,
                          void* stream) {
+  return lhn_gate_bwd_reduce_tail(y, dz, dgate, tsum, slices, prezeroed, nullptr, stream);
+}
+int lhn_gate_bwd_reduce_tail(const lhn_view* y, const float* dz, float* dgate, float* tsum, const lhn_bn_slices* slices, int prezeroed,
+                             const LhnCaTail* tl, void* stream) {
   LHN_CHECK_ARG(lhn_view_ok(y) && dz && dgate && y->C % 4 == 0 && y->C <= 1024 && lhn_no_pend(y), "lhn_gate_bwd_reduce: bad args");
   LHN_CHECK_ARG(!tsum || (y->coff == 0 && y->C == y->cstride && tsum == dgate + (size_t)y->N * y->C),
                 "lhn_gate_bwd_reduce2: tsum = the 2*N*C floats behind dgate, whole-buffer view");
@@ -1407,7 +1886,15 @@
   if (split < 1) split = 1;
   if (split > 32) split = 32;
   if (lhn_deterministic_mode()) split = 1;
-  hipLaunchKernelGGL(k_gate_bwd_reduce, dim3(y->N, split), dim3(256), 0, s, *y, dz, dgate, tsum, sl);
+  CaTail tail;
+  memset(&tail, 0, sizeof(tail));
+  if (tl) {
+    LHN_CHECK_ARG(tl->tickets && tl->w1 && tl->w2 && tl->save && tl->N == y->N && tl->C == y->C && tl->C <= 256 && tl->C % 2 == 0,
+                  "lhn_gate_bwd_reduce_tail: the attention is not the one of this buffer");
+    float* dahat = const_cast<float*>(tl->save) + (int64_t)tl->N * tl->C * 3 + (int64_t)tl->N * (tl->C / 2) + 2 * tl->C;
+    tail = CaTail{tl->tickets, tl->w1, tl->w2, tl->save, dahat, dahat + (int64_t)tl->N * tl->C, dahat + (int64_t)tl->N * tl->C * 2, tl->N, tl->C};
+  }
+  hipLaunchKernelGGL(k_gate_bwd_reduce, dim3(y->N, split), dim3(256), 0, s, *y, dz, dgate, tsum, sl, tail);
   LHN_CHECK_LAUNCH("lhn_gate_bwd_reduce");
   return 0;
 }
@@ -1424,6 +1911,14 @@
                     int W, float* dw3, float* dgamma, float* dbeta, float* dw1, float* db1, float* dw2, float* db2, int N,
                     int C, int stage, double* gsum, double count_scale, float pgrad_scale, const float* tsum, const float* pstat,
                     const lhn_bn_slices* slices, void* stream) {
+  return lhn_ca_mlp_bwd_part(pooled, w3, gamma, w1, w2, dropmask, save, dgate, dpool, cstride, coff, H, W, dw3, dgamma, dbeta, dw1, db1, dw2,
+                             db2, N, C, stage, gsum, count_scale, pgrad_scale, tsum, pstat, slices, 0, stream);
+}
+int lhn_ca_mlp_bwd_part(const float* pooled, const float* w3, const float* gamma, const float* w1, const float* w2,
+                        const float* dropmask, const float* save, const float* dgate, float* dpool, int cstride, int coff, int H,
+                        int W, float* dw3, float* dgamma, float* dbeta, float* dw1, float* db1, float* dw2, float* db2, int N,
+                        int C, int stage, double* gsum, double count_scale, float pgrad_scale, const float* tsum, const float* pstat,
+                        const lhn_bn_slices* slices, int skip_mlp, void* stream) {
   LHN_CHECK_ARG(!tsum == !pstat && (!tsum || (slices && coff == 0 && C == cstride)), "lhn_ca_mlp_bwd2: tsum, pstat and slices come together (whole buffer)");
   BnSlices sl;
   if (mk_slices(tsum ? slices : nullptr, cstride, &sl, "lhn_ca_mlp_bwd2")) return 1;
@@ -1435,8 +1930,27 @@
   float* dvbuf = dahat + (int64_t)N * C;
   float* dhbuf = dvbuf + (int64_t)N * C;
   LHN_CHECK_ARG(stage == 0 || (gsum && stage >= 1 && stage <= 2 && count_scale >= 1), "lhn_ca_mlp_bwd: stage %d needs gsum", stage);
-  if (stage != 2) hipLaunchKernelGGL(k_ca_bwd2, dim3(N), dim3(256), 0, s, w1, w2, save, dgate, dahat, dvbuf, dhbuf, N, C);
-  hipLaunchKernelGGL(k_ca_bwd1, dim3((C + 31) / 32 + (C * C + C + C / 2 + 1023) / 1024), dim3(1024), 0, s, pooled, w3, gamma, dropmask, save, dahat, dpool, cstride, coff, H, W, dw3, dgamma, dbeta, N, C, 1, stage, gsum, stage ? count_scale : 1.0, stage ? pgrad_scale : 1.f, tsum, pstat, sl, dvbuf, dhbuf, dw1, db1, dw2, db2);
+  static LhnKernelCfg cfg2;
+  if (stage != 2 && !skip_mlp) {
+    if (ca_mv_ok(C, save, w1, w2) && lhn_kernel_cfg(cfg2, k_ca_bwd2_lat, CA_MV_LDS_MAX, 1, nullptr))
+      hipLaunchKernelGGL(k_ca_bwd2_lat, dim3(N), dim3(256), (size_t)(C * C + 2 * C) * 4, s, w1, w2, save, dgate, dahat, dvbuf, dhbuf, N, C);
+    else
+      hipLaunchKernelGGL(k_ca_bwd2, dim3(N), dim3(256), 0, s, w1, w2, save, dgate, dahat, dvbuf, dhbuf, N, C);
+  }
+  if (ca_lat_ok(stage, N, C, save)) {
+    const int nb = (C * (C / 2) + 1023) / 1024, nch = 8192 / C < 32 * CA_NS ? 8192 / C : 32 * CA_NS;
+    const dim3 grid((C + 31) / 32 + 2 * nb + 1);
+#define CA_BWD1_LAT(M, T)                                                                                                          \
+  hipLaunchKernelGGL((k_ca_bwd1_lat<M, T>), grid, dim3(1024), CA_BWD1_LDS, s, pooled, w3, gamma, dropmask, save, dahat, dpool, cstride, \
+                     coff, H, W, dw3, dgamma, dbeta, N, C, tsum, pstat, sl, dvbuf, dhbuf, dw1, db1, dw2, db2, nb, nb, nch)
+    if (dropmask && tsum) CA_BWD1_LAT(true, true);
+    else if (dropmask) CA_BWD1_LAT(true, false);
+    else if (tsum) CA_BWD1_LAT(false, true);
+    else CA_BWD1_LAT(false, false);
+#undef CA_BWD1_LAT
+  } else {
+    hipLaunchKernelGGL(k_ca_bwd1, dim3((C + 31) / 32 + (C * C + C + C / 2 + 1023) / 1024), dim3(1024), 0, s, pooled, w3, gamma, dropmask, save, dahat, dpool, cstride, coff, H, W, dw3, dgamma, dbeta, N, C, 1, stage, gsum, stage ? count_scale : 1.0, stage ? pgrad_scale : 1.f, tsum, pstat, sl, dvbuf, dhbuf, dw1, db1, dw2, db2);
+  }
   LHN_CHECK_LAUNCH("lhn_ca_mlp_bwd");
   return 0;
 }
diff --git a/litehandnet_amd/csrc/lhn_common.h b/litehandnet_amd/csrc/lhn_common.h
--- a/litehandnet_amd/csrc/lhn_common.h
+++ b/litehandnet_amd/csrc/lhn_common.h
@@ -44,6 +44,21 @@
 }
 int lhn_num_cus();
 bool lhn_deterministic_mode();
+
+struct LhnCaTail {
+  unsigned* tickets;
+  const float* w1;
+  const float* w2;
+  const float* save;
+  int N, C;
+};
+extern "C" int lhn_gate_bwd_reduce_tail(const lhn_view* y, const float* dz, float* dgate, float* tsum, const lhn_bn_slices* slices,
+                                        int prezeroed, const LhnCaTail* tail, void* stream);
+extern "C" int lhn_ca_mlp_bwd_part(const float* pooled, const float* w3, const float* gamma, const float* w1, const float* w2,
+                                   const float* dropmask, const float* save, const float* dgate, float* dpool, int cstride, int coff,
+                                   int H, int W, float* dw3, float* dgamma, float* dbeta, float* dw1, float* db1, float* dw2,
+                                   float* db2, int N, int C, int stage, double* gsum, double count_scale, float pgrad_scale,
+                                   const float* tsum, const float* pstat, const lhn_bn_slices* slices, int skip_mlp, void* stream);
 
 #ifdef __HIPCC__
 template <typename F>
diff --git a/litehandnet_amd/csrc/lhn_plan.cpp b/litehandnet_amd/csrc/lhn_plan.cpp
--- a/litehandnet_amd/csrc/lhn_plan.cpp
+++ b/litehandnet_amd/csrc/lhn_plan.cpp
@@ -40,7 +40,17 @@
   std::vector<GraphEntry> graphs;
   uint64_t tick = 0;
   int graph_misses = 0;
+  unsigned* tickets = nullptr;
 };
+#define LHN_TAIL_MAX_N 4096
+static bool ca_tail() {
+  static int v = -1;
+  if (v < 0) {
+    const char* e = getenv("LHN_CA_TAIL");
+    v = (e && e[0] == '1') ? 1 : 0;
+  }
+  return v == 1;
+}
 
 static inline char* at(void* ws, int64_t off) { return off < 0 ? nullptr : static_cast<char*>(ws) + off; }
 
@@ -135,12 +145,22 @@
         return nullptr;
       }
     }
+  if (ca_tail() && !p->bwd.empty()) {
+    if (hipMalloc(reinterpret_cast<void**>(&p->tickets), LHN_TAIL_MAX_N * sizeof(unsigned)) != hipSuccess ||
+        hipMemset(p->tickets, 0, LHN_TAIL_MAX_N * sizeof(unsigned)) != hipSuccess) {
+      lhn_set_error("lhn_plan_create: ticket words");
+      if (p->tickets) (void)hipFree(p->tickets);
+      delete p;
+      return nullptr;
+    }
+  }
   return p;
 }
 
 void lhn_plan_destroy(void* plan) {
   Plan* p = static_cast<Plan*>(plan);
   if (!p) return;
+  if (p->tickets) (void)hipFree(p->tickets);
   for (GraphEntry& g : p->graphs)
     if (g.exec) (void)hipGraphExecDestroy(g.exec);
   delete p;
@@ -155,6 +175,7 @@
   hipStream_t s = static_cast<hipStream_t>(stream);
   int rc = 0;
   const bool whole = (sb == 0 && se >= 2 * ops.size());
+  bool mlp_in_tail = false;
   for (size_t oi = 0; oi < ops.size() && rc == 0; ++oi) {
     const lhn_op& o = ops[oi];
     const bool deferred = false;
@@ -549,8 +570,19 @@
         lhn_view y = mkview(P, ws, o.out_buf, o.out_coff, o.out_C, false);
         float* dg = reinterpret_cast<float*>(at(ws, o.ws[3]));
         const lhn_bn_slices sl = mkslices(ws, &o.i[0], &o.ws[5], nullptr);
-        rc = lhn_gate_bwd_reduce3(&y, reinterpret_cast<const float*>(at(ws, P->bufs[o.out_buf].grad_off)), dg,
-                                  o.ws[4] >= 0 ? dg + (size_t)y.N * y.C : nullptr, &sl, 1, stream);
+        LhnCaTail tl;
+        bool fuse = false;
+        if (P->tickets && oi + 1 < ops.size() && ops[oi + 1].kind == OP_CA_MLP_BWD && ops[oi + 1].out_buf == o.out_buf) {
+          const lhn_op& a = ops[oi + 1];
+          const bool a0 = 2 * (oi + 1) >= sb && 2 * (oi + 1) < se, a1 = 2 * (oi + 1) + 1 >= sb && 2 * (oi + 1) + 1 < se;
+          fuse = a0 && (a.ws[4] < 0 || a1) && a.ws[3] == o.ws[3] && a.out_C == y.C && y.N <= LHN_TAIL_MAX_N && y.C <= 256;
+          if (fuse)
+            tl = LhnCaTail{P->tickets, prm<const float>(params, a.p[2]), prm<const float>(params, a.p[3]),
+                           reinterpret_cast<const float*>(at(ws, a.ws[1])), y.N, y.C};
+        }
+        rc = lhn_gate_bwd_reduce_tail(&y, reinterpret_cast<const float*>(at(ws, P->bufs[o.out_buf].grad_off)), dg,
+                                      o.ws[4] >= 0 ? dg + (size_t)y.N * y.C : nullptr, &sl, 1, fuse ? &tl : nullptr, stream);
+        mlp_in_tail = fuse && rc == 0;
         break;
       }
       case OP_CA_MLP_BWD: {
@@ -558,7 +590,9 @@
         if (o.ws[4] < 0 && !h0) break;
         const lhn_bn_slices sl = mkslices(ws, &o.i[0], &o.ws[6], &o.ws[8]);
         const float* dgp = reinterpret_cast<const float*>(at(ws, o.ws[3]));
-        rc = lhn_ca_mlp_bwd2(reinterpret_cast<const float*>(at(ws, o.ws[0])), prm<const float>(params, o.p[0]),
+        const int skip_mlp = mlp_in_tail;
+        mlp_in_tail = false;
+        rc = lhn_ca_mlp_bwd_part(reinterpret_cast<const float*>(at(ws, o.ws[0])), prm<const float>(params, o.p[0]),
                             prm<const float>(params, o.p[1]), prm<const float>(params, o.p[2]), prm<const float>(params, o.p[3]),
                             o.ws[2] >= 0 ? reinterpret_cast<const float*>(at(ws, o.ws[2])) : nullptr,
                             reinterpret_cast<const float*>(at(ws, o.ws[1])), reinterpret_cast<const float*>(at(ws, o.ws[3])),
@@ -567,7 +601,7 @@
                             prm<float>(grads, o.p[8]), prm<float>(grads, o.p[9]), prm<float>(grads, o.p[10]), b.N, o.out_C,
                             o.ws[4] >= 0 ? stage : 0, o.ws[4] >= 0 ? reinterpret_cast<double*>(at(ws, o.ws[4])) : nullptr, cscale, pscale,
                             o.ws[5] >= 0 ? dgp + (size_t)b.N * b.C : nullptr, o.ws[5] >= 0 ? reinterpret_cast<const float*>(at(ws, o.ws[5])) : nullptr,
-                            &sl, stream);
+                            &sl, skip_mlp, stream);
         break;
       }
       case OP_ATT_MLP_BWD: {
```

Result: faster. 8420 images/s (median of 6 runs) (+2.6%).
